# computational-cell-analytics/micro-sam

Hardware: AMD Instinct MI355X
Metric: 1024^2 tiles/s embed+AMG (vit_b bf16) (higher is better)
Workload: dtype bf16 image encoder (patch embedding + neck, 1.2 % of its flops, on hi+lo operand pairs of that type), fp16 mask decoder (16-bit MFMA operands, fp32 accumulation); 1 GPU; configs[1]: vit_b, 1024x1024 uint8 synthetic tiles, batched embedding precompute + AutomaticMaskGenerator (32x32 grid, multimask, default thresholds); encoder_batch=16, distinct_tiles_per_gpu=256, weights=seeded synthetic checkpoint (synthetic.py variant 'cells'), decode_lanes=3

## Files before the change

### include/msam_hip.h

```cpp
#ifndef MSAM_HIP_H
#define MSAM_HIP_H

#include <stdint.h>

#ifdef __cplusplus
extern "C" {
#endif

#define MSAM_MAX_BLOCKS 32
#define MSAM_F32 1
#define MSAM_BF16 2
#define MSAM_FP8 3
#define MSAM_F16 4
#define MSAM_U8 5
#define MSAM_U16 6
#define MSAM_ACT_NONE 0
#define MSAM_ACT_GELU 1
#define MSAM_ACT_RELU 2
#define MSAM_ACT_SIGMOID 3

const char* msam_last_error(void);
int msam_abi_version(void);


// ... 20 lines not shown
    const float* row_scale; const float* col_scale;
    int32_t split_k;
    const float* ln_add; void* ln_out_a; void* ln_out_b;
} msam_gemm_t;
int msam_gemm_bf16(const msam_gemm_t* p, void* stream);
#define MSAM_GEMM_GROUP_MAX 5
int msam_gemm_group_bf16(const msam_gemm_t* items, int32_t n, void* stream);

typedef struct {
    const void* A; const void* W; int32_t M, N, K;
    const float* bias;
    const float* table; int32_t table_rows, table_cols; int64_t table_ld;
    const void* resid; int32_t resid_rows; int64_t ldr;
    int32_t ln_mode; const float* ln_w; const float* ln_b; float ln_eps;
    void* out; int64_t ldc;
    int32_t kv_split; void* k_out; void* vT_out; int32_t tokens;
    int32_t head_major;
} msam_wsgemm_t;
int msam_wsgemm_bf16(const msam_wsgemm_t* p, void* stream);

typedef struct {
    const void* xin; const void* q_shared;
    const void* wq; const float* bq; const float* peq;
    const void* wo; const float* bo; const float* ln_w; const float* ln_b; float ln_eps;
    const void* ktok; const void* vtok; int32_t Nt;
    void* out; int32_t rows;
} msam_image_layer_t;
int msam_decoder_image_layer(const msam_image_layer_t* p, void* stream);

int64_t msam_t2i_fold_workspace_bytes(int32_t P);
int msam_t2i_fold_attention(const void* keys, int32_t kv_shared, const void* qtok, int32_t P, int32_t Nt, const void* wk,
                            const void* tabk, const void* wv, const float* bv, void* out, void* workspace,
                            int64_t workspace_bytes, void* stream);

int64_t msam_i2t_fold_workspace_bytes(int32_t P);
int msam_i2t_fold_layer(const void* xin, int32_t x_shared, const void* ktok, const void* vtok, int32_t P, int32_t Nt,
                        const void* wq, const void* tabq, const void* wo, const float* bo, const float* ln_w,
                        const float* ln_b, float ln_eps, void* out, void* workspace, int64_t workspace_bytes, void* stream);

int64_t msam_chain_tables_bytes(void);
int msam_chain_prepare_tables(const void* src, const void* q0, const void* tabk, const void* tabq1, void* tables, void* stream);
int64_t msam_i2t_fold_operand_bytes(int32_t P);
int msam_i2t_fold_operands(const void* ktok, const void* vtok, int32_t P, int32_t Nt, const void* wq, const void* wo,
                           const float* bo, int32_t with_kfold, void* operands, void* stream);
int64_t msam_i2t0_t2i_workspace_bytes(int32_t P);
int msam_i2t0_t2i_fused(const void* tables, const void* operands0, const float* ln0_w, const float* ln0_b, float ln_eps,
                        const void* qtok, int32_t P, int32_t Nt, const void* wk, const void* wv, const float* bv, void* out,
                        void* workspace, int64_t workspace_bytes, void* stream);
int64_t msam_chain_tables2_bytes(void);
int msam_chain_prepare_tables2(const void* src, const void* wv, const float* bv, const void* wk, const float* ln0_w,
                               const float* ln0_b, const void* wo0, const float* bo0, void* tables2, void* stream);
int64_t msam_chain_const2_bytes(void);
int msam_chain_prepare_const2(const void* wv, const float* bv, const void* wk, const float* ln0_w, const float* ln0_b,
                              const void* wo0, const float* bo0, void* const2, void* stream);
int msam_chain_prepare_tables2_c(const void* src, const void* const2, void* tables2, void* stream);
int64_t msam_t2i_fold_values_bytes(int32_t P);
int msam_t2i_fold_values(const void* vtok0, int32_t P, int32_t Nt, const void* tables2, void* mf, void* stream);
int msam_i2t_fold_operands_values(const void* ktok, const void* vtok, int32_t P, int32_t Nt, const void* wq, const void* wo,
                                  const float* bo, int32_t with_kfold, const void* tables2, void* operands, void* mf, void* stream);
int64_t msam_i2t0_t2i_v2_workspace_bytes(int32_t P);
int msam_i2t0_t2i_fused_v2(const void* tables, const void* tables2, const void* operands0, const void* mf, const float* ln0_w,
                           float ln_eps, const void* qtok, int32_t P, int32_t Nt, const void* wk, void* out, void* workspace,
                           int64_t workspace_bytes, void* stream);
int msam_i2t01_fused(const void* tables, const void* operands0, const float* ln0_w, const float* ln0_b, const void* operands1,
                     const float* ln1_w, const float* ln1_b, float ln_eps, int32_t P, int32_t Nt, void* out, void* stream);
int64_t msam_chain_handover_bytes(int32_t P);
int msam_i2t0_t2i_fused_v2_handover(const void* tables, const void* tables2, const void* operands0, const void* mf, const float* ln0_w,
                                    float ln_eps, const void* qtok, int32_t P, int32_t Nt, const void* wk, void* out, void* workspace,
                                    int64_t workspace_bytes, void* handover, void* stream);
int msam_i2t01_fused_handover(const void* tables, const void* operands0, const float* ln0_w, const float* ln0_b, const void* operands1,
                              const float* ln1_w, const float* ln1_b, float ln_eps, int32_t P, int32_t Nt, const void* handover,
                              void* out, void* stream);

int msam_upscale_fused(const void* keys, int32_t P, const void* w1, const float* b1, const float* ln_w, const float* ln_b,
                       float ln_eps, const void* w2, const float* b2, const float* hyper, int32_t hyper_ld, int32_t mask0,
                       int32_t nmask, float* low_res, void* stream);
int msam_upscale_fused_layout(const void* keys, int32_t keys_blocked, int32_t P, const void* w1, const float* b1,
                              const float* ln_w, const float* ln_b, float ln_eps, const void* w2, const float* b2,
                              const float* hyper, int32_t hyper_ld, int32_t mask0, int32_t nmask, float* low_res, void* stream);
int msam_upscale_fused_out(const void* keys, int32_t keys_blocked, int32_t P, const void* w1, const float* b1,
                           const float* ln_w, const float* ln_b, float ln_eps, const void* w2, const float* b2,
                           const float* hyper, int32_t hyper_ld, int32_t mask0, int32_t nmask, void* low_res,
                           int32_t low_res_dtype, void* stream);

int msam_upscale_set_prio(int32_t prio);
int msam_fold_attn_set_dma(int32_t on);
int msam_tune_set(const char* key, int32_t value);
int msam_debug_i2t_timing(int32_t enable, uint64_t* host_out);
int msam_gemm256_set_staging(int staging);
int msam_gemm_set_trace(void* device_words);
int msam_profile_enable(int on);
int msam_profile_collect(int32_t* launches, double* total_ms, double* total_flops);
#define MSAM_PROFILE_FAMILIES 8
int msam_profile_collect_family(int32_t* launches, double* ms, double* flops, double* bytes);

int msam_to_image(const void* in, int32_t in_dtype, int32_t H, int32_t W, int32_t C, uint8_t* out, void* workspace, void* stream);

int msam_mask_nms(const uint32_t* bits, const int32_t* order, const float* boxes, const int32_t* area, int32_t K, int32_t H,
                  int32_t W, float thresh, int32_t intersection_over_min, uint64_t* mask_scratch, int32_t* keep_flags,
                  void* stream);

int64_t msam_amg_generate_workspace_bytes(int32_t N, int32_t H, int32_t W);
int msam_amg_generate_labels(const float* iou, const float* stability, const int32_t* boxes, const int32_t* area,
                             const uint32_t* bits, int32_t N, int32_t H, int32_t W, const int32_t* crop_box,
                             float pred_iou_thresh, float stability_score_thresh, float box_nms_thresh,
                             int32_t min_object_size, int32_t with_background, int32_t* labels, int32_t* flag,
                             void* workspace, int64_t workspace_bytes, void* stream);

int64_t msam_labels_from_masks_workspace_bytes(int32_t H, int32_t W);
int msam_labels_from_masks(const uint32_t* bits, const int32_t* order, int32_t K, const int32_t* k_dev, int32_t H, int32_t W,
                           int32_t min_object_size, int32_t with_background, int32_t* labels, int32_t* flag,
                           void* workspace, int64_t workspace_bytes, void* stream);

int msam_layernorm_backward(const float* x, const float* weight, const float* dy, float eps, int64_t rows, int32_t dim,
                            float* dx, float* dweight, float* dbias, void* stream);
int msam_attention_forward(const float* q, const float* k, const float* v, int32_t BH, int32_t Nq, int32_t Nk, int32_t D,
                           float scale, float* out, float* lse, void* stream);
int msam_attention_backward(const float* q, const float* k, const float* v, const float* out, const float* dout,
                            const float* lse, int32_t BH, int32_t Nq, int32_t Nk, int32_t D, float scale, float* dq, float* dk,
                            float* dv, float* delta, void* stream);

int msam_relpos_attention_forward(const float* q, const float* k, const float* v, const float* bias_h, const float* bias_w,
                                  int32_t BH, int32_t Gh, int32_t Gw, int32_t D, float scale, float* out, float* lse,
                                  void* stream);
int msam_relpos_attention_backward(const float* q, const float* k, const float* v, const float* bias_h, const float* bias_w,
                                   const float* out, const float* dout, const float* lse, int32_t BH, int32_t Gh, int32_t Gw,
                                   int32_t D, float scale, float* dq, float* dk, float* dv, float* dbias_h, float* dbias_w,
                                   float* delta, void* stream);

int msam_cast_transpose(const void* x, int32_t x_dtype, int64_t M, int32_t K, int64_t ldx, void* out16, void* outT, float* colsum,
                        void* stream);

int msam_layernorm(const float* x, const float* weight, const float* bias, float eps, int64_t rows, int32_t dim,
                   void* out, int32_t out_dtype, int32_t gelu, int32_t out_nchw_hw, void* stream);

int msam_layernorm_fp8(const float* x, const float* weight, const float* bias, float eps, int64_t rows, int32_t dim,
                       void* out_fp8, float* row_scale, void* stream);
int msam_quant_rows_fp8(const void* x_bf16, int64_t rows, int32_t dim, void* out_fp8, float* row_scale, void* stream);
int msam_patchify(const float* img, int32_t B, void* out_bf16, void* stream);
int msam_patchify16(const float* img, int32_t B, int32_t dtype16, void* out16, void* stream);
int msam_patchify_u8(const uint8_t* img, int32_t B, int32_t h, int32_t w, void* out_bf16, void* stream);
int msam_patchify_u8_16(const uint8_t* img, int32_t B, int32_t h, int32_t w, int32_t dtype16, void* out16, void* stream);
int msam_im2col3x3(const void* x_bf16, int32_t B, int32_t C, void* out_bf16, void* stream);
int msam_cast_f32_to_bf16(const float* x, void* out_bf16, int64_t n, void* stream);
int msam_cast_f32_to_16(const float* x, int32_t dtype16, void* out16, int64_t n, void* stream);
int msam_resample_u8(const uint8_t* in, int32_t B, int32_t H, int32_t W, int32_t C, int32_t axis, int32_t n_out,
                     const int32_t* bounds, const int32_t* coefs, int32_t ksize, uint8_t* out, void* stream);
int msam_patchify_split16(const float* img, int32_t B, int32_t dtype16, void* out16, void* stream);
int msam_patchify_u8_split16(const uint8_t* img, int32_t B, int32_t h, int32_t w, int32_t dtype16, void* out16, void* stream);
int msam_im2col3x3_split16(const float* x_f32, int32_t B, int32_t C, int32_t dtype16, void* out16, void* stream);
int msam_cast_f32_split16(const float* x, int32_t dtype16, void* out16, int64_t rows, int32_t dim, void* stream);

int msam_window_attention(const void* q, const void* k, const void* v, const void* rel_h, const void* rel_w,
                          const float* qkv_bias, int32_t B, int32_t heads, int32_t head_dim, float scale, void* out,
                          void* stream);
int msam_window_attention16(const void* q, const void* k, const void* v, const void* rel_h, const void* rel_w,
                            const float* qkv_bias, int32_t B, int32_t heads, int32_t head_dim, float scale, int32_t dtype16,
                            void* out, void* stream);
int msam_global_attention(const void* q, const void* k, const void* v, const void* rel_h, const void* rel_w,
                          int32_t B, int32_t heads, int32_t head_dim, float scale, void* out, void* stream);
int msam_global_attention16(const void* q, const void* k, const void* v, const void* rel_h, const void* rel_w, int32_t B,
                            int32_t heads, int32_t head_dim, float scale, int32_t dtype16, void* out, void* stream);

typedef struct {
    int32_t embed_dim, depth, heads;
    int32_t is_global[MSAM_MAX_BLOCKS];
    const void* patch_w; const float* patch_b;
    const float* pos_embed;
    const float* ln1_w[MSAM_MAX_BLOCKS]; const float* ln1_b[MSAM_MAX_BLOCKS];
    const void* qkv_w[MSAM_MAX_BLOCKS]; const float* qkv_b[MSAM_MAX_BLOCKS];
    const void* rel_h[MSAM_MAX_BLOCKS]; const void* rel_w[MSAM_MAX_BLOCKS];
    const void* proj_w[MSAM_MAX_BLOCKS]; const float* proj_b[MSAM_MAX_BLOCKS];
    const float* ln2_w[MSAM_MAX_BLOCKS]; const float* ln2_b[MSAM_MAX_BLOCKS];
    const void* lin1_w[MSAM_MAX_BLOCKS]; const float* lin1_b[MSAM_MAX_BLOCKS];
    const void* lin2_w[MSAM_MAX_BLOCKS]; const float* lin2_b[MSAM_MAX_BLOCKS];
    const void* neck0_w;
    const float* neck1_w; const float* neck1_b;
    const void* neck2_w;
    const float* neck3_w; const float* neck3_b;
    int32_t use_glds;
    int32_t head_dim_stored;
    int32_t fp8;
    const void* qkv_w8[MSAM_MAX_BLOCKS]; const float* qkv_cs[MSAM_MAX_BLOCKS];
    const void* proj_w8[MSAM_MAX_BLOCKS]; const float* proj_cs[MSAM_MAX_BLOCKS];
    const void* lin1_w8[MSAM_MAX_BLOCKS]; const float* lin1_cs[MSAM_MAX_BLOCKS];
    const void* lin2_w8[MSAM_MAX_BLOCKS]; const float* lin2_cs[MSAM_MAX_BLOCKS];
    int32_t dtype16;
    int32_t split_io;
    const void* adapter_wd[MSAM_MAX_BLOCKS]; const float* adapter_bd[MSAM_MAX_BLOCKS];
    const void* adapter_wu[MSAM_MAX_BLOCKS]; const float* adapter_bu[MSAM_MAX_BLOCKS];
    const float* adapter_alpha[MSAM_MAX_BLOCKS];
    int32_t adapter_dim;
} msam_encoder_t;

int64_t msam_encoder_workspace_bytes(const msam_encoder_t* enc, int32_t B);
int msam_encoder_forward(const msam_encoder_t* enc, const float* img_f32, const uint8_t* img_u8, int32_t h, int32_t w,
                         int32_t B, float* out, void* workspace, int64_t workspace_bytes,
                         float* tap, int32_t tap_block, void* stream);

int msam_adapter_bf16(const void* y16, int64_t ldy, const void* wd16, const float* bd, const void* wu16, const float* bu,
                      const float* alpha, float* x, int64_t ldx, int32_t R, int32_t D, int32_t P, int32_t dtype16, void* stream);

typedef struct {
    const void* q_w; const float* q_b; const void* k_w; const float* k_b;
    const void* v_w; const float* v_b; const void* o_w; const float* o_b;
} msam_attn_w_t;
typedef struct {
    msam_attn_w_t self_attn, t2i, i2t;
    const float *n1_w, *n1_b, *n2_w, *n2_b, *n3_w, *n3_b, *n4_w, *n4_b;
    const void* mlp1_w; const float* mlp1_b; const void* mlp2_w; const float* mlp2_b;
    const void* mlp1_ws; const void* mlp2_ws;
} msam_twoway_layer_t;
typedef struct {
    const float* pe_gauss;
    const float* point_embed;
    const float* not_a_point;
    const float* no_mask;
    const float* out_tokens;
    msam_twoway_layer_t layer[2];
    msam_attn_w_t final_attn; const float *nf_w, *nf_b;
    const void* up1_w; const float* up1_b;
    const float* up_ln_w; const float* up_ln_b;
    const void* up2_w; const float* up2_b;
    const void* hyp_w[4][3]; const float* hyp_b[4][3];
    const void* iou_w[3]; const float* iou_b[3];
    int32_t use_glds;
    int32_t low_res_dtype;
    int32_t up1_centred;
} msam_decoder_t;

int msam_decoder_dtype(void);
int64_t msam_decoder_const_bytes(void);
int msam_decoder_prepare_const(const msam_decoder_t* dec, void* consts, void* stream);
int64_t msam_decoder_image_bytes(void);
int msam_decoder_prepare_image(const msam_decoder_t* dec, const void* consts, const float* embedding ,
                               void* image_state, void* workspace, int64_t workspace_bytes, void* stream);
int64_t msam_decoder_workspace_bytes(int32_t P);
int msam_decoder_forward(const msam_decoder_t* dec, const void* consts, const void* image_state,
                         const float* points, const int32_t* labels, int32_t Np, const float* boxes, int32_t P,
                         int32_t multimask, float* low_res, float* iou,
                         void* workspace, int64_t workspace_bytes, void* stream);

typedef struct {
    const float *c1_w, *c1_b, *ln1_w, *ln1_b, *c2_w, *c2_b, *ln2_w, *ln2_b, *c3_w, *c3_b;
    int32_t exact_gelu;
} msam_mask_prompt_t;
int msam_decoder_forward_masks(const msam_decoder_t* dec, const msam_mask_prompt_t* mask_w, const void* consts,
                               const void* image_state, const float* points, const int32_t* labels, int32_t Np,
                               const float* boxes, const float* mask_input, int32_t P, int32_t multimask, float* low_res,
                               float* iou, void* workspace, int64_t workspace_bytes, void* stream);

int msam_prompt_encode(const msam_decoder_t* dec, const msam_mask_prompt_t* mask_w, const float* points,
                       const int32_t* labels, int32_t Np, const float* boxes, const float* mask_input, int32_t P,
                       float* sparse, float* dense, void* stream);
int msam_decoder_forward_embeddings(const msam_decoder_t* dec, const void* consts, const void* image_state,
                                    const float* sparse, int32_t Ns, const float* dense, const float* embedding,
                                    int32_t P, int32_t multimask, float* low_res, float* iou, void* workspace,
                                    int64_t workspace_bytes, void* stream);

int msam_postprocess_masks(const float* low_res, int32_t N, int32_t in_h, int32_t in_w, int32_t out_h, int32_t out_w,
                           float thr, float off, int32_t* counts, int32_t* boxes, uint32_t* bits, float* logits,
                           void* stream);
int msam_postprocess_masks16(const void* low_res, int32_t low_res_dtype, int32_t N, int32_t in_h, int32_t in_w, int32_t out_h,
                             int32_t out_w, float thr, float off, int32_t* counts, int32_t* boxes, uint32_t* bits, float* logits,
                             void* stream);
int msam_uncrop_bits(const uint32_t* bits_crop, int32_t N, int32_t crop_h, int32_t crop_w, int32_t x0, int32_t y0,
                     int32_t out_h, int32_t out_w, uint32_t* bits_out, void* stream);

int msam_rle_run_counts(const uint32_t* bits, int32_t N, int32_t out_h, int32_t out_w, int32_t* n_runs, void* stream);
int msam_rle_encode(const uint32_t* bits, int32_t N, int32_t out_h, int32_t out_w, const int64_t* offsets,
                    int32_t* counts_out, void* stream);

int msam_box_nms(const float* boxes_sorted, int32_t K, float iou_threshold, uint64_t* mask_scratch, int32_t* keep_flags,
                 void* stream);

int msam_box_nms_valid(const float* boxes_sorted, const int32_t* valid_sorted, int32_t K, float iou_threshold,
                       uint64_t* mask_scratch, int32_t* keep_flags, void* stream);

int msam_paint_label_image(const uint32_t* bits, const int32_t* order, int32_t K, int32_t H, int32_t W, int32_t* label,
                           void* stream);
int msam_paint_label_image_dev(const uint32_t* bits, const int32_t* order, const int32_t* k_dev, int32_t H, int32_t W,
                               int32_t* label, void* stream);
int msam_label_components(const int32_t* seg, int32_t H, int32_t W, int32_t* roots, int32_t* changed_flag,
                          int32_t max_iters, int32_t* iters_done, void* stream);

int msam_component_sizes(const int32_t* roots, int32_t n, int32_t* sizes, int32_t* bg_count, void* stream);
int msam_label_components_async(const int32_t* seg, int32_t H, int32_t W, int32_t* roots, int32_t* changed_flag,
                                int32_t passes, void* stream);

#define MSAM_MATCH_MAX_THRESHOLDS 16
#define MSAM_MATCH_MAX_BATCH 65535
#define MSAM_MATCH_HEADER 4
#define MSAM_MATCH_ITEM 20
#define MSAM_MATCH_EDGE 6
int64_t msam_label_matching_workspace_bytes(int32_t B, int32_t capacity);
int msam_label_matching(const int32_t* pred, const int32_t* gt, int32_t B, int32_t G, int32_t H, int32_t W,
                        const double* thresholds, int32_t T, void* workspace, int64_t workspace_bytes, int32_t capacity,
                        int32_t* result, int32_t max_edges, void* stream);

int msam_slice_overlaps(const int32_t* labels, int32_t Z, int32_t H, int32_t W, uint64_t* table_keys, int32_t* table_counts,
                        int32_t capacity, int32_t* edges, int32_t max_edges, int32_t* n_edges, void* stream);

int msam_host_seeded_watershed(const float* image, const int32_t* markers, const uint8_t* mask, int32_t H, int32_t W, int32_t* out);

typedef struct {
    const float* A; int64_t lda;
    const float* A2; int64_t lda2; int64_t a2_rows;
    const float* W; int64_t ldw;
    int64_t M; int32_t N, K;
    const float* bias; int32_t act;
    const float* res; int64_t ldr; int64_t res_rows;
    float* out; int64_t ldc;
    const float* col_scale; const float* col_shift;
    int32_t conv_h, conv_w, conv_c;
    int32_t shuffle_h, shuffle_w, shuffle_c;
    int32_t a2_cols;
    int32_t split16;
    float a_scale, w_scale;
    const void* w_pairs;
} msam_sgemm_t;
int msam_strict_gemm(const msam_sgemm_t* p, void* stream);
int msam_strict_layernorm(const float* x, const float* weight, const float* bias, float eps, int64_t rows, int32_t dim, float* out,
                          int32_t gelu, int32_t out_nchw_hw, void* stream);
int msam_strict_relpos_attention(const float* qkv, const float* qkv_bias, const float* rel_h, const float* rel_w, int32_t B, int32_t heads,
                                 int32_t head_dim, int32_t grid, int32_t window, float scale, float* out, void* stream);
int msam_split16_relpos_attention(const float* qkv, const float* qkv_bias, const float* rel_h, const float* rel_w, int32_t B, int32_t heads,
                                  int32_t head_dim, int32_t grid, int32_t window, float scale, float* out, void* stream);
typedef struct msam_si2t {
    const float* keys; int64_t key_batch_stride;
    const float* pos;
    const float* wq; const float* bq;
    const float* tok_k; const float* tok_v; int64_t ld_tok, tok_batch_stride;
    const float* wo; const float* bo;
    const float* ln_weight; const float* ln_bias; float ln_eps; float denom;
    float* out;
    int32_t B, Tk;
    int32_t split16;
    float wq_scale, wo_scale;
    const void* wq_pairs; const void* wo_pairs;
} msam_si2t_t;
int msam_strict_i2t_block(const msam_si2t_t* p, void* stream);
int msam_strict_attention(const float* q, int64_t ldq, int64_t q_batch_stride, const float* k, int64_t ldk, int64_t k_batch_stride,
                          const float* v, int64_t ldv, int64_t v_batch_stride, int32_t B, int32_t H, int32_t Nq, int32_t Nk, int32_t D,
                          float denom, float* out, int64_t ldo, int64_t out_batch_stride, void* stream);
int msam_strict_patchify(const float* img, const uint8_t* img_u8, int32_t B, int32_t h, int32_t w, float* out, void* stream);
int msam_strict_im2col3x3(const float* x, int32_t B, int32_t C, float* out, void* stream);
int msam_strict_source(const float* embedding, const float* dense, int64_t dense_stride, int32_t P, float* src, void* stream);
int msam_strict_hyper_masks(const float* up, const float* hyper, int32_t hyper_ld, int32_t mask0, int32_t nmask, int64_t P, float* low_res,
// ... 107 lines not shown
```

### micro_sam_amd/_lib.py

```python
from __future__ import annotations

import ctypes as C
import os
from typing import Optional

import torch

from . import build as _build

MSAM_MAX_BLOCKS = 32
F32, BF16, FP8, F16, U8, U16 = 1, 2, 3, 4, 5, 6
ACT_NONE, ACT_GELU, ACT_RELU, ACT_SIGMOID = 0, 1, 2, 3

_vp, _i32, _i64, _f32 = C.c_void_p, C.c_int32, C.c_int64, C.c_float
PROFILE_FAMILIES = 8


class GemmParams(C.Structure):
    _fields_ = [
        ("A", _vp), ("lda", _i64), ("W", _vp), ("ldw", _i64), ("M", _i32), ("N", _i32), ("K", _i32),
        ("bias", _vp), ("table", _vp), ("table_rows", _i32), ("table_cols", _i32), ("table_ld", _i64),
        ("resid", _vp), ("resid_dtype", _i32), ("resid_rows", _i32), ("ldr", _i64), ("act", _i32),
        ("out", _vp), ("out_dtype", _i32), ("ldc", _i64), ("out_mode", _i32),
        ("q", _vp), ("k", _vp), ("v", _vp), ("heads", _i32), ("head_dim", _i32), ("tokens", _i32),
        ("use_glds", _i32), ("ln_mode", _i32), ("ln_w", _vp), ("ln_b", _vp), ("ln_eps", _f32),
        ("a_dtype", _i32), ("row_scale", _vp), ("col_scale", _vp), ("split_k", _i32),
        ("ln_add", _vp), ("ln_out_a", _vp), ("ln_out_b", _vp),
    ]


class WsGemmParams(C.Structure):
    _fields_ = [
        ("A", _vp), ("W", _vp), ("M", _i32), ("N", _i32), ("K", _i32), ("bias", _vp),
        ("table", _vp), ("table_rows", _i32), ("table_cols", _i32), ("table_ld", _i64),
        ("resid", _vp), ("resid_rows", _i32), ("ldr", _i64),
        ("ln_mode", _i32), ("ln_w", _vp), ("ln_b", _vp), ("ln_eps", _f32),
        ("out", _vp), ("ldc", _i64), ("kv_split", _i32), ("k_out", _vp), ("vT_out", _vp), ("tokens", _i32),
        ("head_major", _i32),
    ]


class ImageLayerParams(C.Structure):
    _fields_ = [
        ("xin", _vp), ("q_shared", _vp), ("wq", _vp), ("bq", _vp), ("peq", _vp),
        ("wo", _vp), ("bo", _vp), ("ln_w", _vp), ("ln_b", _vp), ("ln_eps", _f32),
        ("ktok", _vp), ("vtok", _vp), ("Nt", _i32), ("out", _vp), ("rows", _i32),
    ]


_blk = _vp * MSAM_MAX_BLOCKS


class EncoderParams(C.Structure):
    _fields_ = [
        ("embed_dim", _i32), ("depth", _i32), ("heads", _i32), ("is_global", _i32 * MSAM_MAX_BLOCKS),
        ("patch_w", _vp), ("patch_b", _vp), ("pos_embed", _vp),
        ("ln1_w", _blk), ("ln1_b", _blk), ("qkv_w", _blk), ("qkv_b", _blk), ("rel_h", _blk), ("rel_w", _blk),
        ("proj_w", _blk), ("proj_b", _blk), ("ln2_w", _blk), ("ln2_b", _blk),
        ("lin1_w", _blk), ("lin1_b", _blk), ("lin2_w", _blk), ("lin2_b", _blk),
        ("neck0_w", _vp), ("neck1_w", _vp), ("neck1_b", _vp), ("neck2_w", _vp), ("neck3_w", _vp), ("neck3_b", _vp),
        ("use_glds", _i32), ("head_dim_stored", _i32), ("fp8", _i32),
        ("qkv_w8", _blk), ("qkv_cs", _blk), ("proj_w8", _blk), ("proj_cs", _blk),
        ("lin1_w8", _blk), ("lin1_cs", _blk), ("lin2_w8", _blk), ("lin2_cs", _blk),
        ("dtype16", _i32), ("split_io", _i32),
        ("adapter_wd", _blk), ("adapter_bd", _blk), ("adapter_wu", _blk), ("adapter_bu", _blk), ("adapter_alpha", _blk),
        ("adapter_dim", _i32),
    ]


class AttnW(C.Structure):
    _fields_ = [("q_w", _vp), ("q_b", _vp), ("k_w", _vp), ("k_b", _vp), ("v_w", _vp), ("v_b", _vp),
                ("o_w", _vp), ("o_b", _vp)]


class TwoWayLayer(C.Structure):
    _fields_ = [("self_attn", AttnW), ("t2i", AttnW), ("i2t", AttnW),
                ("n1_w", _vp), ("n1_b", _vp), ("n2_w", _vp), ("n2_b", _vp), ("n3_w", _vp), ("n3_b", _vp),
                ("n4_w", _vp), ("n4_b", _vp),
                ("mlp1_w", _vp), ("mlp1_b", _vp), ("mlp2_w", _vp), ("mlp2_b", _vp), ("mlp1_ws", _vp), ("mlp2_ws", _vp)]


class DecoderParams(C.Structure):
    _fields_ = [
        ("pe_gauss", _vp), ("point_embed", _vp), ("not_a_point", _vp), ("no_mask", _vp), ("out_tokens", _vp),
        ("layer", TwoWayLayer * 2), ("final_attn", AttnW), ("nf_w", _vp), ("nf_b", _vp),
        ("up1_w", _vp), ("up1_b", _vp), ("up_ln_w", _vp), ("up_ln_b", _vp), ("up2_w", _vp), ("up2_b", _vp),
        ("hyp_w", (_vp * 3) * 4), ("hyp_b", (_vp * 3) * 4), ("iou_w", _vp * 3), ("iou_b", _vp * 3),
        ("use_glds", _i32), ("low_res_dtype", _i32), ("up1_centred", _i32),
    ]


class SGemmParams(C.Structure):
    _fields_ = [("A", _vp), ("lda", _i64), ("A2", _vp), ("lda2", _i64), ("a2_rows", _i64), ("W", _vp), ("ldw", _i64),
                ("M", _i64), ("N", _i32), ("K", _i32), ("bias", _vp), ("act", _i32), ("res", _vp), ("ldr", _i64), ("res_rows", _i64),
                ("out", _vp), ("ldc", _i64), ("col_scale", _vp), ("col_shift", _vp), ("conv_h", _i32), ("conv_w", _i32), ("conv_c", _i32),
                ("shuffle_h", _i32), ("shuffle_w", _i32), ("shuffle_c", _i32), ("a2_cols", _i32), ("split16", _i32), ("a_scale", _f32), ("w_scale", _f32), ("w_pairs", _vp)]


class SI2TParams(C.Structure):
    _fields_ = [("keys", _vp), ("key_batch_stride", _i64), ("pos", _vp), ("wq", _vp), ("bq", _vp), ("tok_k", _vp), ("tok_v", _vp),
                ("ld_tok", _i64), ("tok_batch_stride", _i64), ("wo", _vp), ("bo", _vp), ("ln_weight", _vp), ("ln_bias", _vp),
                ("ln_eps", _f32), ("denom", _f32), ("out", _vp), ("B", _i32), ("Tk", _i32), ("split16", _i32), ("wq_scale", _f32), ("wo_scale", _f32), ("wq_pairs", _vp), ("wo_pairs", _vp)]


class ST2IParams(C.Structure):
    _fields_ = [("keys", _vp), ("key_batch_stride", _i64), ("pos", _vp), ("q", _vp), ("ldq", _i64), ("wk", _vp), ("wv", _vp), ("bv", _vp),
                ("denom", _f32), ("out", _vp), ("ldo", _i64), ("B", _i32), ("Tk", _i32), ("workspace", _vp), ("workspace_bytes", _i64)]


class SUp2Params(C.Structure):
    _fields_ = [("u1", _vp), ("ln_weight", _vp), ("ln_bias", _vp), ("ln_eps", _f32), ("w2", _vp), ("b2", _vp), ("w_scale", _f32),
                ("hyper", _vp), ("hyper_ld", _i32), ("mask0", _i32), ("nmask", _i32), ("low_res", _vp), ("P", _i64)]


class MaskPromptParams(C.Structure):
    _fields_ = [(n, _vp) for n in ("c1_w", "c1_b", "ln1_w", "ln1_b", "c2_w", "c2_b", "ln2_w", "ln2_b", "c3_w", "c3_b")] + [("exact_gelu", _i32)]


_PROTOS = {
    "msam_last_error": (C.c_char_p, []),
    "msam_abi_version": (_i32, []),
    "msam_gemm_bf16": (_i32, [C.POINTER(GemmParams), _vp]),
    "msam_wsgemm_bf16": (_i32, [C.POINTER(WsGemmParams), _vp]),
    "msam_decoder_image_layer": (_i32, [C.POINTER(ImageLayerParams), _vp]),
    "msam_t2i_fold_workspace_bytes": (_i64, [_i32]),
    "msam_t2i_fold_attention": (_i32, [_vp, _i32, _vp, _i32, _i32, _vp, _vp, _vp, _vp, _vp, _vp, _i64, _vp]),
    "msam_upscale_fused": (_i32, [_vp, _i32, _vp, _vp, _vp, _vp, _f32, _vp, _vp, _vp, _i32, _i32, _i32, _vp, _vp]),
    "msam_uncrop_bits": (_i32, [_vp, _i32, _i32, _i32, _i32, _i32, _i32, _i32, _vp, _vp]),
    "msam_decoder_forward_masks": (_i32, [C.POINTER(DecoderParams), C.POINTER(MaskPromptParams), _vp, _vp, _vp, _vp, _i32, _vp, _vp,
                                          _i32, _i32, _vp, _vp, _vp, _i64, _vp]),
    "msam_i2t_fold_workspace_bytes": (_i64, [_i32]),
    "msam_i2t_fold_layer": (_i32, [_vp, _i32, _vp, _vp, _i32, _i32, _vp, _vp, _vp, _vp, _vp, _vp, _f32, _vp, _vp, _i64, _vp]),
    "msam_profile_enable": (_i32, [_i32]),
    "msam_profile_collect": (_i32, [C.POINTER(_i32), C.POINTER(C.c_double), C.POINTER(C.c_double)]),
    "msam_profile_collect_family": (_i32, [_i32 * PROFILE_FAMILIES, C.c_double * PROFILE_FAMILIES, C.c_double * PROFILE_FAMILIES,
                                          C.c_double * PROFILE_FAMILIES]),
    "msam_layernorm": (_i32, [_vp, _vp, _vp, _f32, _i64, _i32, _vp, _i32, _i32, _i32, _vp]),
    "msam_layernorm_backward": (_i32, [_vp, _vp, _vp, _f32, _i64, _i32, _vp, _vp, _vp, _vp]),
    "msam_attention_forward": (_i32, [_vp, _vp, _vp, _i32, _i32, _i32, _i32, _f32, _vp, _vp, _vp]),
    "msam_attention_backward": (_i32, [_vp, _vp, _vp, _vp, _vp, _vp, _i32, _i32, _i32, _i32, _f32, _vp, _vp, _vp, _vp, _vp]),
    "msam_relpos_attention_forward": (_i32, [_vp, _vp, _vp, _vp, _vp, _i32, _i32, _i32, _i32, _f32, _vp, _vp, _vp]),
    "msam_relpos_attention_backward": (_i32, [_vp, _vp, _vp, _vp, _vp, _vp, _vp, _vp, _i32, _i32, _i32, _i32, _f32, _vp, _vp, _vp,
                                              _vp, _vp, _vp, _vp]),
    "msam_amg_generate_workspace_bytes": (_i64, [_i32, _i32, _i32]),
    "msam_amg_generate_labels": (_i32, [_vp, _vp, _vp, _vp, _vp, _i32, _i32, _i32, C.POINTER(_i32), _f32, _f32, _f32, _i32, _i32,
                                        _vp, _vp, _vp, _i64, _vp]),
    "msam_to_image": (_i32, [_vp, _i32, _i32, _i32, _i32, _vp, _vp, _vp]),
    "msam_patchify": (_i32, [_vp, _i32, _vp, _vp]),
    "msam_patchify_u8": (_i32, [_vp, _i32, _i32, _i32, _vp, _vp]),
    "msam_im2col3x3": (_i32, [_vp, _i32, _i32, _vp, _vp]),
    "msam_cast_f32_to_bf16": (_i32, [_vp, _vp, _i64, _vp]),
    "msam_cast_transpose": (_i32, [_vp, _i32, _i64, _i32, _i64, _vp, _vp, _vp, _vp]),
    "msam_gemm256_set_staging": (_i32, [_i32]),
    "msam_gemm_set_trace": (_i32, [_vp]),
    "msam_gemm_group_bf16": (_i32, [_vp, _i32, _vp]),
    "msam_fold_attn_set_dma": (_i32, [_i32]),
    "msam_tune_set": (_i32, [C.c_char_p, _i32]),
    "msam_i2t_fold_operand_bytes": (_i64, [_i32]),
    "msam_i2t_fold_operands": (_i32, [_vp, _vp, _i32, _i32, _vp, _vp, _vp, _i32, _vp, _vp]),
    "msam_i2t0_t2i_workspace_bytes": (_i64, [_i32]),
    "msam_i2t0_t2i_fused": (_i32, [_vp, _vp, _vp, _vp, _f32, _vp, _i32, _i32, _vp, _vp, _vp, _vp, _vp, _i64, _vp]),
    "msam_i2t01_fused": (_i32, [_vp, _vp, _vp, _vp, _vp, _vp, _vp, _f32, _i32, _i32, _vp, _vp]),
    "msam_chain_tables2_bytes": (_i64, []),
    "msam_chain_prepare_tables2": (_i32, [_vp, _vp, _vp, _vp, _vp, _vp, _vp, _vp, _vp, _vp]),
    "msam_chain_const2_bytes": (_i64, []),
    "msam_chain_prepare_const2": (_i32, [_vp, _vp, _vp, _vp, _vp, _vp, _vp, _vp, _vp]),
    "msam_chain_prepare_tables2_c": (_i32, [_vp, _vp, _vp, _vp]),
    "msam_t2i_fold_values_bytes": (_i64, [_i32]),
    "msam_t2i_fold_values": (_i32, [_vp, _i32, _i32, _vp, _vp, _vp]),
    "msam_i2t_fold_operands_values": (_i32, [_vp, _vp, _i32, _i32, _vp, _vp, _vp, _i32, _vp, _vp, _vp, _vp]),
    "msam_i2t0_t2i_v2_workspace_bytes": (_i64, [_i32]),
    "msam_i2t0_t2i_fused_v2": (_i32, [_vp, _vp, _vp, _vp, _vp, _f32, _vp, _i32, _i32, _vp, _vp, _vp, _i64, _vp]),
    "msam_chain_handover_bytes": (_i64, [_i32]),
    "msam_i2t0_t2i_fused_v2_handover": (_i32, [_vp, _vp, _vp, _vp, _vp, _f32, _vp, _i32, _i32, _vp, _vp, _vp, _i64, _vp, _vp]),
    "msam_i2t01_fused_handover": (_i32, [_vp, _vp, _vp, _vp, _vp, _vp, _vp, _f32, _i32, _i32, _vp, _vp, _vp]),
    "msam_chain_tables_bytes": (_i64, []),
    "msam_chain_prepare_tables": (_i32, [_vp, _vp, _vp, _vp, _vp, _vp]),
    "msam_upscale_fused_layout": (_i32, [_vp, _i32, _i32, _vp, _vp, _vp, _vp, _f32, _vp, _vp, _vp, _i32, _i32, _i32, _vp, _vp]),
    "msam_upscale_fused_out": (_i32, [_vp, _i32, _i32, _vp, _vp, _vp, _vp, _f32, _vp, _vp, _vp, _i32, _i32, _i32, _vp, _i32, _vp]),
    "msam_upscale_set_prio": (_i32, [_i32]),
    "msam_layernorm_fp8": (_i32, [_vp, _vp, _vp, _f32, _i64, _i32, _vp, _vp, _vp]),
    "msam_quant_rows_fp8": (_i32, [_vp, _i64, _i32, _vp, _vp, _vp]),
    "msam_debug_i2t_timing": (_i32, [_i32, _vp]),
    "msam_window_attention": (_i32, [_vp, _vp, _vp, _vp, _vp, _vp, _i32, _i32, _i32, C.c_float, _vp, _vp]),
    "msam_global_attention": (_i32, [_vp, _vp, _vp, _vp, _vp, _i32, _i32, _i32, C.c_float, _vp, _vp]),
    "msam_window_attention16": (_i32, [_vp, _vp, _vp, _vp, _vp, _vp, _i32, _i32, _i32, C.c_float, _i32, _vp, _vp]),
    "msam_global_attention16": (_i32, [_vp, _vp, _vp, _vp, _vp, _i32, _i32, _i32, C.c_float, _i32, _vp, _vp]),
    "msam_patchify16": (_i32, [_vp, _i32, _i32, _vp, _vp]),
    "msam_patchify_u8_16": (_i32, [_vp, _i32, _i32, _i32, _i32, _vp, _vp]),
    "msam_cast_f32_to_16": (_i32, [_vp, _i32, _vp, _i64, _vp]),
    "msam_resample_u8": (_i32, [_vp, _i32, _i32, _i32, _i32, _i32, _i32, _vp, _vp, _i32, _vp, _vp]),
    "msam_patchify_split16": (_i32, [_vp, _i32, _i32, _vp, _vp]),
    "msam_patchify_u8_split16": (_i32, [_vp, _i32, _i32, _i32, _i32, _vp, _vp]),
    "msam_im2col3x3_split16": (_i32, [_vp, _i32, _i32, _i32, _vp, _vp]),
    "msam_cast_f32_split16": (_i32, [_vp, _i32, _vp, _i64, _i32, _vp]),
    "msam_encoder_workspace_bytes": (_i64, [C.POINTER(EncoderParams), _i32]),
    "msam_encoder_forward": (_i32, [C.POINTER(EncoderParams), _vp, _vp, _i32, _i32, _i32, _vp, _vp, _i64, _vp, _i32, _vp]),
    "msam_decoder_dtype": (_i32, []),
    "msam_decoder_const_bytes": (_i64, []),
    "msam_decoder_prepare_const": (_i32, [C.POINTER(DecoderParams), _vp, _vp]),
    "msam_decoder_image_bytes": (_i64, []),
    "msam_decoder_prepare_image": (_i32, [C.POINTER(DecoderParams), _vp, _vp, _vp, _vp, _i64, _vp]),
    "msam_decoder_workspace_bytes": (_i64, [_i32]),
    "msam_prompt_encode": (_i32, [C.POINTER(DecoderParams), C.POINTER(MaskPromptParams), _vp, _vp, _i32, _vp, _vp, _i32, _vp, _vp, _vp]),
    "msam_decoder_forward_embeddings": (_i32, [C.POINTER(DecoderParams), _vp, _vp, _vp, _i32, _vp, _vp, _i32, _i32, _vp, _vp, _vp,
                                               _i64, _vp]),
    "msam_decoder_forward": (_i32, [C.POINTER(DecoderParams), _vp, _vp, _vp, _vp, _i32, _vp, _i32, _i32, _vp, _vp, _vp,
                                    _i64, _vp]),
    "msam_postprocess_masks": (_i32, [_vp, _i32, _i32, _i32, _i32, _i32, _f32, _f32, _vp, _vp, _vp, _vp, _vp]),
    "msam_postprocess_masks16": (_i32, [_vp, _i32, _i32, _i32, _i32, _i32, _i32, _f32, _f32, _vp, _vp, _vp, _vp, _vp]),
    "msam_rle_run_counts": (_i32, [_vp, _i32, _i32, _i32, _vp, _vp]),
    "msam_rle_encode": (_i32, [_vp, _i32, _i32, _i32, _vp, _vp, _vp]),
    "msam_mask_nms": (_i32, [_vp, _vp, _vp, _vp, _i32, _i32, _i32, _f32, _i32, _vp, _vp, _vp]),
    "msam_box_nms": (_i32, [_vp, _i32, _f32, _vp, _vp, _vp]),
    "msam_box_nms_valid": (_i32, [_vp, _vp, _i32, _f32, _vp, _vp, _vp]),
    "msam_paint_label_image_dev": (_i32, [_vp, _vp, _vp, _i32, _i32, _vp, _vp]),
    "msam_label_components_async": (_i32, [_vp, _i32, _i32, _vp, _vp, _i32, _vp]),
    "msam_component_sizes": (_i32, [_vp, _i32, _vp, _vp, _vp]),
    "msam_labels_from_masks_workspace_bytes": (_i64, [_i32, _i32]),
    "msam_labels_from_masks": (_i32, [_vp, _vp, _i32, _vp, _i32, _i32, _i32, _i32, _vp, _vp, _vp, _i64, _vp]),
    "msam_host_seeded_watershed": (_i32, [_vp, _vp, _vp, _i32, _i32, _vp]),
    "msam_slice_overlaps": (_i32, [_vp, _i32, _i32, _i32, _vp, _vp, _i32, _vp, _i32, _vp, _vp]),
    "msam_paint_label_image": (_i32, [_vp, _vp, _i32, _i32, _i32, _vp, _vp]),
    "msam_label_components": (_i32, [_vp, _i32, _i32, _vp, _vp, _i32, C.POINTER(_i32), _vp]),
    "msam_strict_gemm": (_i32, [C.POINTER(SGemmParams), _vp]),
    "msam_strict_i2t_block": (_i32, [C.POINTER(SI2TParams), _vp]),
    "msam_strict_layernorm": (_i32, [_vp, _vp, _vp, _f32, _i64, _i32, _vp, _i32, _i32, _vp]),
    "msam_strict_relpos_attention": (_i32, [_vp, _vp, _vp, _vp, _i32, _i32, _i32, _i32, _i32, _f32, _vp, _vp]),
    "msam_split16_relpos_attention": (_i32, [_vp, _vp, _vp, _vp, _i32, _i32, _i32, _i32, _i32, _f32, _vp, _vp]),
    "msam_strict_attention": (_i32, [_vp, _i64, _i64, _vp, _i64, _i64, _vp, _i64, _i64, _i32, _i32, _i32, _i32, _i32, _f32, _vp, _i64,
                                     _i64, _vp]),
    "msam_strict_patchify": (_i32, [_vp, _vp, _i32, _i32, _i32, _vp, _vp]),
    "msam_strict_im2col3x3": (_i32, [_vp, _i32, _i32, _vp, _vp]),
    "msam_strict_source": (_i32, [_vp, _vp, _i64, _i32, _vp, _vp]),
    "msam_strict_hyper_masks": (_i32, [_vp, _vp, _i32, _i32, _i32, _i64, _vp, _vp]),
    "msam_strict_upscale2": (_i32, [C.POINTER(SUp2Params), _vp]),
    "msam_split16_t2i_attention": (_i32, [C.POINTER(ST2IParams), _vp]),
    "msam_split16_prepare_pairs": (_i32, [_vp, _i64, _i32, _f32, _i32, _vp, _vp]),
    "msam_split16_i2t_block": (_i32, [C.POINTER(SI2TParams), _vp, _i64, _vp]),
    "msam_strict_instance_norm": (_i32, [_vp, _i64, _i32, _i64, _i32, _f32, _vp, _vp, _i64, _vp]),
    "msam_strict_resize_bilinear": (_i32, [_vp, _i32, _i32, _i32, _i32, _i32, _i64, _i32, _i32, _i32, _f32, _f32, _i32, _vp, _vp]),
    "msam_objfeat_gather": (_i32, [_vp, _vp, _i32, _i32, _vp, _vp, _i32, _vp, _vp, _vp]),
    "msam_objfeat_accumulate": (_i32, [_vp, _vp, _i32, _vp, _vp, _vp, _vp, _vp, _vp, _vp, _i32, _i32, _i32, _vp, _vp]),
    "msam_objfeat_finish": (_i32, [_vp, _vp, _vp, _i32, _vp, _vp, _i32, _vp, _vp]),
    "msam_objfeat_project": (_i32, [_vp, _i64, _vp, _i32, _vp, _vp]),
    "msam_label_matching_workspace_bytes": (_i64, [_i32, _i32]),
    "msam_label_matching": (_i32, [_vp, _vp, _i32, _i32, _i32, _i32, C.POINTER(C.c_double), _i32, _vp, _i64, _i32, _vp, _i32, _vp]),
    "msam_edt_squared_workspace_bytes": (_i64, [_i32, _i32]),
    "msam_edt_squared": (_i32, [_vp, _i32, _i32, _i32, _vp, _vp, _i64, _vp]),
    "msam_label_props_workspace_bytes": (_i64, [_i32, _i32, _i32]),
    "msam_label_props": (_i32, [_vp, _i32, _i32, _vp, _i32, _vp, _vp, _vp, _vp, _vp, _i64, _vp]),
    "msam_distance_targets_workspace_bytes": (_i64, [_i32, _i32, _i32]),
    "msam_distance_targets": (_i32, [_vp, _i32, _i32, _i32, _i32, _f32, _vp, _vp, _vp, _vp, _vp, _i64, _vp]),
    "msam_mask_pack": (_i32, [_vp, _i32, _i32, _i32, _vp, _vp]),
    "msam_mask_iou_counts": (_i32, [_vp, _vp, _i32, _i32, _i32, C.c_double, _vp, _vp, _vp]),
    "msam_mask_box_prompts": (_i32, [_vp, _i32, _i32, _i32, C.c_double, _i32, _i32, _vp, _vp, _vp]),
    "msam_mask_logits": (_i32, [_vp, _i32, _i32, _i32, _vp, _vp]),
    "msam_paint_max": (_i32, [_vp, _vp, _vp, _i32, _i32, _i32, _vp, _vp]),
    "msam_pca_moments_workspace_bytes": (_i64, [_i32, _i32, _i32]),
    "msam_pca_moments": (_i32, [_vp, _i32, _i32, _i32, _vp, _vp, _vp, _i64, _vp]),
    "msam_pca_project": (_i32, [_vp, _vp, _vp, _i32, _i32, _i32, _i32, _vp, _vp, _vp]),
    "msam_pca_to_rgb": (_i32, [_vp, _vp, _i32, _i32, _vp, _vp]),
    "msam_semantic_loss_workspace_bytes": (_i64, [_i32, _i32, _i32]),
    "msam_semantic_loss_forward": (_i32, [_vp, _vp, _i32, _i32, _i32, _f32, _f32, _i32, C.c_double, _vp, _i64, _vp, _vp, _vp]),
    "msam_semantic_loss_backward": (_i32, [_vp, _vp, _i32, _i32, _i32, _f32, _f32, _i32, C.c_double, _vp, _vp, _vp, _vp]),
    "msam_depth_conv3_bf16": (_i32, [_vp, _i64, _vp, _vp, _vp, _i64, _i32, _i32, _i32, _i32, _i32, _vp]),
    "msam_conv3d_k3_bf16": (_i32, [_vp, _i64, _vp, _vp, _vp, _i64, _i32, _i32, _i32, _i32, _i32, _i32, _vp]),
    "msam_conv3d_k3_wgrad_workspace_bytes": (_i64, [_i32, _i32, _i32, _i32, _i32, _i32]),
    "msam_conv3d_k3_wgrad_bf16": (_i32, [_vp, _i64, _vp, _i64, _vp, _vp, _i64, _i32, _i32, _i32, _i32, _i32, _i32, _vp]),
    "msam_instance_norm_workspace_bytes": (_i64, [_i32, _i64, _i32]),
    "msam_instance_norm_stats": (_i32, [_vp, _i64, _i32, _i64, _i32, _vp, _vp, _i64, _vp]),
    "msam_instance_norm_apply": (_i32, [_vp, _i64, _vp, _vp, _i64, _vp, _i32, _i64, _i32, _f32, _f32, _i32, _vp, _i64, _vp, _i64, _vp]),
    "msam_instance_norm_backward": (_i32, [_vp, _i64, _vp, _i64, _vp, _vp, _i64, _vp, _i32, _i64, _i32, _f32, _f32, _i32, _vp, _i64, _vp, _i64,
                                           _vp, _vp, _i64, _vp]),
    "msam_column_sums_f32": (_i32, [_vp, _i64, _i64, _i32, _vp, _vp, _i64, _vp]),
    "msam_adapter_bf16": (_i32, [_vp, _i64, _vp, _vp, _vp, _vp, _vp, _vp, _i64, _i32, _i32, _i32, _i32, _vp]),
}
OPTIONAL = set()

_lib: Optional[C.CDLL] = None


def lib_path() -> str:
    return _build.variant_path(os.environ.get("MSAM_LIB_VARIANT", ""))


def load() -> C.CDLL:
    global _lib
    if _lib is not None:
        return _lib
    path = lib_path()
    if not os.path.exists(path):
        raise RuntimeError(
            f"micro_sam_amd: {path} is missing. Build it with `python -m micro_sam_amd.build` "
            "(hipcc --offload-arch=gfx950). There is no CPU / PyTorch fallback."
        )
    lib = C.CDLL(path)
    for name, (res, args) in _PROTOS.items():
        if not hasattr(lib, name):
            if name in OPTIONAL:
                continue
            raise RuntimeError(f"micro_sam_amd: {path} does not export {name}")
        fn = getattr(lib, name)
        fn.restype, fn.argtypes = res, args
    _lib = lib
    for item in filter(None, os.environ.get("MSAM_TUNE", "").split(",")):
        key, _, val = item.partition("=")
        if lib.msam_tune_set(key.strip().encode(), int(val)) != 0:
            raise RuntimeError(f"micro_sam_amd: MSAM_TUNE: unknown knob {key!r}")
    return lib


def decoder_dtype() -> torch.dtype:
    return torch.float16 if load().msam_decoder_dtype() == F16 else torch.bfloat16


def exported_symbols():
    return [n for n in _PROTOS if n not in OPTIONAL]


def check(status: int, what: str = "") -> None:
    if status == 0:
        return
    msg = load().msam_last_error().decode("utf-8", "replace")
    if status == 1:
        raise ValueError(f"{what}: {msg}")
    raise RuntimeError(f"{what}: {msg}")


def require_gpu(device=None) -> torch.device:
    if not torch.cuda.is_available():
        raise RuntimeError("micro_sam_amd needs an AMD GPU (gfx950); torch.cuda.is_available() is False. "
                           "There is no CPU fallback.")
    return torch.device("cuda", torch.cuda.current_device()) if device is None else torch.device(device)


def stream_ptr() -> int:
    return torch.cuda.current_stream().cuda_stream


def ptr(t: Optional[torch.Tensor]) -> Optional[int]:
    if t is None:
        return None
    assert t.is_cuda, "device tensor expected"
    return t.data_ptr()
```

### micro_sam_amd/csrc/decfold.hip

```cpp
#include "common.h"
#include "../../include/msam_hip.h"
#include <string>

void msam_set_error(const char* msg);
int msam_check_launch(const char* what);
void msam_profile_mark2(void* stream, int begin, double flops, double bytes, int family);

namespace {

constexpr int T = 4096, C = 256, CI = 128, TK = 32, NTHR = 256;
constexpr int SUBT = 1024 + 32;
constexpr int KEYS_BYTES = 16 * SUBT, TAB_BYTES = TK * CI * 2, BUF_BYTES = KEYS_BYTES + TAB_BYTES;
constexpr float NEG_BIG = -1.0e30f;
#ifndef FOLD_ATTN_DMA_DEFAULT
#define FOLD_ATTN_DMA_DEFAULT 0
#endif

typedef short s16x4_t __attribute__((ext_vector_type(4)));

MSAM_DEVINL uint2 lds_tr16(const unsigned char* p) {
    s16x4_t v = __builtin_amdgcn_ds_read_tr16_b64_v4i16((s16x4_t __attribute__((address_space(3)))*)p);
    return __builtin_bit_cast(uint2, v);
}

// ... 596 lines not shown
    if (g_fold_attn_dma && !a.blocked) {
        const int grid3 = a.nitems < 3 * cus ? a.nitems : 3 * cus;
        hipLaunchKernelGGL(fold_attn_kernel<true>, dim3(grid3), dim3(NTHR), 0, s, a);
    } else {
        hipLaunchKernelGGL(fold_attn_kernel<false>, dim3(grid), dim3(NTHR), 0, s, a);
    }
    msam_profile_mark2(stream, 0, flops, bytes, 3);
    if (int e = msam_check_launch("fold_attn")) return e;
    if (KS == 1) return 0;
    hipLaunchKernelGGL(fold_finish_kernel, dim3(P * 8), dim3(128), 0, s, opart, stats, KS, Nt, (const u16*)wv, bv, (u16*)out);
    return msam_check_launch("fold_finish");
}

int64_t msam_i2t_tok_workspace_bytes(int32_t P);
int msam_i2t_tok_layer(const void* xin, int32_t x_shared, const void* ktok, const void* vtok, int32_t P, int32_t Nt,
                       const void* wq, const void* tabq, const void* wo, const float* bo, const float* ln_w,
                       const float* ln_b, float ln_eps, void* out, void* workspace, int KS, void* stream);
extern int g_tune_i2t_variant;

extern "C" int64_t msam_i2t_fold_workspace_bytes(int32_t P) {
    const int64_t a = (int64_t)P * 64 * C * 2 * 2, b = msam_i2t_tok_workspace_bytes(P);
    return a > b ? a : b;
}

extern "C" int msam_i2t_fold_layer(const void* xin, int32_t x_shared, const void* ktok, const void* vtok, int32_t P,
                                   int32_t Nt, const void* wq, const void* tabq, const void* wo, const float* bo,
                                   const float* ln_w, const float* ln_b, float ln_eps, void* out, void* workspace,
                                   int64_t workspace_bytes, void* stream) {
    if (!xin || !ktok || !vtok || !wq || !tabq || !wo || !bo || !ln_w || !ln_b || !out || !workspace || P <= 0) {
        msam_set_error("msam_i2t_fold_layer: null argument");
        return 1;
    }
    if (Nt < 1 || Nt > 8) { msam_set_error("msam_i2t_fold_layer: 1 <= Nt <= 8 tokens per prompt"); return 1; }
    if (workspace_bytes < msam_i2t_fold_workspace_bytes(P)) { msam_set_error("msam_i2t_fold_layer: workspace too small"); return 1; }
    if (g_tune_i2t_variant == 1)
        return msam_i2t_tok_layer(xin, x_shared, ktok, vtok, P, Nt, wq, tabq, wo, bo, ln_w, ln_b, ln_eps, out, workspace,
                                  key_splits(P), stream);
    hipStream_t s = (hipStream_t)stream;
    u16* kfold = (u16*)workspace;
    u16* vfoldT = kfold + (long)P * 64 * C;
    hipLaunchKernelGGL(fold_q_kernel, dim3(P * 8), dim3(256), 0, s, (const u16*)ktok, (const u16*)wq, Nt, kfold);
    if (int e = msam_check_launch("fold_k")) return e;
    hipLaunchKernelGGL(fold_v_kernel, dim3(P), dim3(256), 0, s, (const u16*)vtok, (const u16*)wo, Nt, vfoldT);
    if (int e = msam_check_launch("fold_v")) return e;
    I2tArgs a{};
    a.xin = (const u16*)xin; a.x_shared = x_shared; a.kfold = kfold; a.vfoldT = vfoldT; a.ktok = (const u16*)ktok; a.Nt = Nt;
    a.tabq = (const u16*)tabq; a.bo = bo; a.ln_w = ln_w; a.ln_b = ln_b; a.eps = ln_eps;
    a.KS = key_splits(P); a.nitems = P * a.KS; a.out = (u16*)out;
    int dev = 0, cus = 256;
    (void)hipGetDevice(&dev);
    (void)hipDeviceGetAttribute(&cus, hipDeviceAttributeMultiprocessorCount, dev);
    const int grid = a.nitems < 2 * cus ? a.nitems : 2 * cus;
    const double flops = (double)P * T * (2.0 * 64 * C * 2 + 2.0 * 64 * 32);
    const double bytes = (double)(x_shared ? 1 : P) * T * C * 2 + (double)P * T * C * 2;
    msam_profile_mark2(stream, 1, flops, bytes, 2);
    if (g_i2t_timing) hipLaunchKernelGGL(fold_i2t_kernel<true>, dim3(grid), dim3(NTHR), 0, s, a);
    else hipLaunchKernelGGL(fold_i2t_kernel<false>, dim3(grid), dim3(NTHR), 0, s, a);
    msam_profile_mark2(stream, 0, flops, bytes, 2);
    return msam_check_launch("fold_i2t");
}

extern "C" int msam_debug_i2t_timing(int32_t enable, uint64_t* host_out) {
    g_i2t_timing = enable;
    if (host_out) {
        if (hipDeviceSynchronize() != hipSuccess ||
            hipMemcpyFromSymbol(host_out, HIP_SYMBOL(g_i2t_stamps), sizeof(unsigned long long) * 64 * 12) != hipSuccess) {
            msam_set_error("msam_debug_i2t_timing: copy failed");
            return 2;
        }
    }
    return 0;
}

extern "C" int msam_fold_attn_set_dma(int32_t on) { g_fold_attn_dma = on; return 0; }

extern int g_tune_i2t_wg_per_cu, g_tune_chain_variant, g_tune_chain_tmask, g_tune_up_gelu16, g_tune_up_ln_two_pass, g_tune_up_centred;
void msam_gemm_set_dbg(int v);
void msam_gemm_set_gw(int delay, int cls);
void msam_gemm_set_g3(int delay);
void msam_gemm_set_g3_epi(int v);
extern int g_tune_tok_fuse;
extern int g_tune_chain_handover, g_tune_chain_handover_ring;
extern int g_tune_mlp_split_fused;
extern int g_tune_sgemm_bufs, g_tune_srel_mfma, g_tune_sgemm_small_below, g_tune_si2t_dbg, g_tune_si2t_late_us, g_tune_sattn_allh;
int g_tune_dec_chain = 1, g_tune_dec_chain_min_p = 128;
extern "C" int msam_tune_set(const char* key, int32_t value) {
    const std::string k = key ? key : "";
    if (k == "i2t_variant") g_tune_i2t_variant = value;
    else if (k == "i2t_wg_per_cu") g_tune_i2t_wg_per_cu = value;
    else if (k == "dec_chain") g_tune_dec_chain = value;
    else if (k == "chain_variant") g_tune_chain_variant = value;
    else if (k == "chain_tmask") g_tune_chain_tmask = value;
    else if (k == "chain_handover") g_tune_chain_handover = value;
    else if (k == "chain_handover_ring") g_tune_chain_handover_ring = value;
    else if (k == "up_gelu16") g_tune_up_gelu16 = value;
    else if (k == "up_ln_two_pass") g_tune_up_ln_two_pass = value;
    else if (k == "up_centred") g_tune_up_centred = value;
    else if (k == "gemm_dbg") msam_gemm_set_dbg(value);
    else if (k == "gw_delay") msam_gemm_set_gw(value, -1);
    else if (k == "gw_class") msam_gemm_set_gw(-2, value);
    else if (k == "g3_delay") msam_gemm_set_g3(value);
    else if (k == "g3_epi") msam_gemm_set_g3_epi(value);
    else if (k == "tok_fuse") g_tune_tok_fuse = value;
    else if (k == "mlp_split_fused") g_tune_mlp_split_fused = value;
    else if (k == "dec_chain_min_p") g_tune_dec_chain_min_p = value;
    else if (k == "sgemm_bufs") g_tune_sgemm_bufs = value;
    else if (k == "srel_mfma") g_tune_srel_mfma = value;
    else if (k == "sattn_allh") g_tune_sattn_allh = value;
    else if (k == "sgemm_small_below") g_tune_sgemm_small_below = value;
    else if (k == "si2t_dbg") g_tune_si2t_dbg = value;
    else if (k == "si2t_late_us") g_tune_si2t_late_us = value;
    else { msam_set_error("msam_tune_set: unknown key"); return 1; }
    return 0;
}
```

### micro_sam_amd/csrc/decoder.hip

```cpp
#include <stdlib.h>
#include "common.h"
#include "../../include/msam_hip.h"

void msam_set_error(const char* msg);
int msam_check_launch(const char* what);

namespace {

constexpr int T = 4096;
constexpr int C = 256;
constexpr int CI = 128;
constexpr float NEG_BIG = -1.0e30f;
constexpr float TWO_PI = 6.283185307179586f;


MSAM_DEVINL void pe_encode(const float* __restrict__ G, float cx, float cy, int j, float& s, float& c) {
    const float x = 2.f * cx - 1.f, y = 2.f * cy - 1.f;
    const float v = TWO_PI * (x * G[j] + y * G[128 + j]);
    s = sinf(v); c = cosf(v);
}

__global__ __launch_bounds__(256) void dense_pe_kernel(const float* __restrict__ G, float* __restrict__ pos_f32,
                                                       u16* __restrict__ pos_bf16) {
    const int idx = blockIdx.x * 256 + threadIdx.x;
// ... 800 lines not shown
                CHECK(msam_cast_f32_split16(h32, MSAM_D16, h3, M, 2048, cx.s));
            }
            mlp_h = h3; mlp2_w = L.mlp2_ws; mlp2_k = 3 * 2048;
        } else {
        CHECK(gemm(cx, w.a, C, L.mlp1_w, M, 2048, C, L.mlp1_b, w.mlp_h, MSAM_D16, 2048, MSAM_ACT_RELU));
        }
        if (fuse_tok) {
            CHECK(gemm_ln_tok(cx, mlp_h, mlp2_k, mlp2_w, M, mlp2_k, L.mlp2_b, w.queries, L.n3_w, L.n3_b, w.queries, w.qpe, w.a, w.b));
        } else {
        CHECK(gemm(cx, mlp_h, mlp2_k, mlp2_w, M, C, mlp2_k, L.mlp2_b, w.tmp, MSAM_F32, C, 0, w.queries, MSAM_F32, C));
        LN(w.tmp, L.n3_w, L.n3_b, M, w.queries, MSAM_F32);
        ADD_CAST2(w.queries, w.qpe, w.a, w.b);
        }
        {
            const msam_gemm_t kv[2] = {mk_gemm(w.a, C, L.i2t.k_w, M, CI, C, L.i2t.k_b, w.ks, MSAM_D16, CI),
                                       mk_gemm(w.b, C, L.i2t.v_w, M, CI, C, L.i2t.v_b, w.vs, MSAM_D16, CI)};
            CHECK(msam_gemm_group_bf16(kv, 2, cx.s));
        }
        if (chain) {
            if (li == 0 && chain2)
                CHECK(msam_i2t_fold_operands_values(w.ks, w.vs, P, Nt, L.i2t.q_w, L.i2t.o_w, L.i2t.o_b, 0, tables2, oper0, mfrag, cx.s));
            else
                CHECK(msam_i2t_fold_operands(w.ks, w.vs, P, Nt, L.i2t.q_w, L.i2t.o_w, L.i2t.o_b, li, li == 0 ? oper0 : oper1, cx.s));
            if (li == 1) {
                const msam_twoway_layer_t& L0 = dec->layer[0];
                if (handover)
                    CHECK(msam_i2t01_fused_handover(tables, oper0, L0.n4_w, L0.n4_b, oper1, L.n4_w, L.n4_b, 1e-5f, P, Nt, w.hand, w.keys, cx.s));
                else
                    CHECK(msam_i2t01_fused(tables, oper0, L0.n4_w, L0.n4_b, oper1, L.n4_w, L.n4_b, 1e-5f, P, Nt, w.keys, cx.s));
            }
        } else if (Nt <= 8) {
            const bool shared = li == 0 && !own_src;
            CHECK(msam_i2t_fold_layer(shared ? (const void*)im.src_bf16 : (const void*)w.keys, shared, w.ks, w.vs, P, Nt,
                                      L.i2t.q_w, c.tab_q[li], L.i2t.o_w, L.i2t.o_b, L.n4_w, L.n4_b, 1e-5f, w.keys, w.qimg,
                                      (int64_t)((char*)w.up1 - (char*)w.qimg), cx.s));
        } else {
            msam_image_layer_t g{};
            g.wo = L.i2t.o_w; g.bo = L.i2t.o_b; g.ln_w = L.n4_w; g.ln_b = L.n4_b; g.ln_eps = 1e-5f;
            g.ktok = w.ks; g.vtok = w.vs; g.Nt = Nt; g.out = w.keys; g.rows = (int)R;
            if (li == 0 && !own_src) { g.xin = im.src_bf16; g.q_shared = im.q0; }
            else { g.xin = w.keys; g.wq = L.i2t.q_w; g.bq = L.i2t.q_b; g.peq = c.pe_q[li]; }
            CHECK(msam_decoder_image_layer(&g, cx.s));
        }
    }
    if (dbg) return 0;
    if (!fuse_tok) ADD_CAST(w.queries, w.qpe, w.a);
    CHECK(gemm(cx, w.a, C, dec->final_attn.q_w, M, CI, C, dec->final_attn.q_b, w.qs, MSAM_D16, CI));
    CHECK(t2i_stream(cx, w, c, 2, dec->final_attn, P, Nt, chain));
    if (fuse_tok) {
        CHECK(gemm_ln_tok(cx, w.attn_tok, CI, dec->final_attn.o_w, M, CI, dec->final_attn.o_b, w.queries, dec->nf_w, dec->nf_b, w.queries,
                          nullptr, w.a, nullptr));
    } else {
    CHECK(gemm(cx, w.attn_tok, CI, dec->final_attn.o_w, M, C, CI, dec->final_attn.o_b, w.tmp, MSAM_F32, C, 0, w.queries,
               MSAM_F32, C));
    LN(w.tmp, dec->nf_w, dec->nf_b, M, w.queries, MSAM_F32);

    ADD_CAST(w.queries, nullptr, w.a);
    }
    {
        msam_gemm_t h[5];
        const long PC = (long)P * C;
        for (int i = 0; i < 5; ++i) {
            const void* wt = i == 0 ? dec->iou_w[0] : dec->hyp_w[i - 1][0];
            const float* bs = i == 0 ? dec->iou_b[0] : dec->hyp_b[i - 1][0];
            h[i] = mk_gemm(w.a + (long)i * C, (long)Nt * C, wt, P, C, C, bs, w.hh0 + i * PC, MSAM_D16, C, MSAM_ACT_RELU);
        }
        CHECK(msam_gemm_group_bf16(h, 5, cx.s));
        for (int i = 0; i < 5; ++i) {
            const void* wt = i == 0 ? dec->iou_w[1] : dec->hyp_w[i - 1][1];
            const float* bs = i == 0 ? dec->iou_b[1] : dec->hyp_b[i - 1][1];
            h[i] = mk_gemm(w.hh0 + i * PC, C, wt, P, C, C, bs, w.hh1 + i * PC, MSAM_D16, C, MSAM_ACT_RELU);
        }
        CHECK(msam_gemm_group_bf16(h, 5, cx.s));
        h[0] = mk_gemm(w.hh1, C, dec->iou_w[2], P, 128, C, dec->iou_b[2], w.iou_full, MSAM_F32, 128);
        for (int i = 1; i < 5; ++i)
            h[i] = mk_gemm(w.hh1 + i * PC, C, dec->hyp_w[i - 1][2], P, 128, C, dec->hyp_b[i - 1][2], w.hyper + (long)(i - 1) * 128,
                           MSAM_F32, 4 * 128);
        CHECK(msam_gemm_group_bf16(h, 5, cx.s));
    }
    const int mask0 = multimask ? 1 : 0, nmask = multimask ? 3 : 1;
    hipLaunchKernelGGL(gather_iou_kernel, dim3((P * nmask + 255) / 256), dim3(256), 0, cx.s, w.iou_full, P, mask0, nmask, iou);
    CHECK(msam_check_launch("gather_iou"));

    CHECK(msam_upscale_fused_out(w.keys, (chain ? 1 : 0) | (dec->up1_centred ? 2 : 0), P, dec->up1_w, dec->up1_b, dec->up_ln_w, dec->up_ln_b, 1e-6f, dec->up2_w,
                                 dec->up2_b, w.hyper, 128, mask0, nmask, low_res, dec->low_res_dtype == MSAM_F16 ? MSAM_F16 : MSAM_F32,
                                 cx.s));
#undef CHECK
#undef ADD_CAST
#undef ADD_CAST2
#undef LN
    return 0;
}
}
```

### micro_sam_amd/csrc/postprocess.hip

```cpp
#include "common.h"
#include "../../include/msam_hip.h"

void msam_set_error(const char* msg);
int msam_check_launch(const char* what);

namespace {

struct Axis { int i0, i1; float w0, w1; };
struct lowh_t { unsigned short bits; };
MSAM_DEVINL float lowf(float v) { return v; }
MSAM_DEVINL float lowf(lowh_t v) { return h2f(v.bits); }

MSAM_DEVINL Axis axis_weights(int dst, float scale, int in_size) {
    float src = __fsub_rn(__fmul_rn(scale, __fadd_rn((float)dst, 0.5f)), 0.5f);
    if (src < 0.f) src = 0.f;
    Axis a;
    a.i0 = (int)src;
    a.i1 = a.i0 + (a.i0 < in_size - 1 ? 1 : 0);
    a.w1 = __fsub_rn(src, (float)a.i0);
    a.w0 = __fsub_rn(1.0f, a.w1);
    return a;
}

MSAM_DEVINL float lerp_torch(float w0, float p0, float w1, float p1) { return __fmaf_rn(w0, p0, __fmul_rn(w1, p1)); }

template <typename TL>
MSAM_DEVINL float stage1(const TL* __restrict__ low, int Y, int X) {
    const Axis ay = axis_weights(Y, 0.25f, 256), ax = axis_weights(X, 0.25f, 256);
    const TL* r0 = low + ay.i0 * 256; const TL* r1 = low + ay.i1 * 256;
    const float t0 = lerp_torch(ax.w0, lowf(r0[ax.i0]), ax.w1, lowf(r0[ax.i1]));
    const float t1 = lerp_torch(ax.w0, lowf(r1[ax.i0]), ax.w1, lowf(r1[ax.i1]));
    return lerp_torch(ay.w0, t0, ay.w1, t1);
}

__global__ void init_stats_kernel(int* __restrict__ counts, int* __restrict__ boxes, int N) {
    const int n = blockIdx.x * 256 + threadIdx.x;
    if (n >= N) return;
    counts[n * 3] = 0; counts[n * 3 + 1] = 0; counts[n * 3 + 2] = 0;
    boxes[n * 4] = 0x7fffffff; boxes[n * 4 + 1] = 0x7fffffff; boxes[n * 4 + 2] = -1; boxes[n * 4 + 3] = -1;
}

__global__ void finalize_boxes_kernel(int* __restrict__ boxes, int N) {
    const int n = blockIdx.x * 256 + threadIdx.x;
    if (n >= N) return;
    if (boxes[n * 4 + 2] < boxes[n * 4] || boxes[n * 4 + 3] < boxes[n * 4 + 1]) {
        boxes[n * 4] = 0; boxes[n * 4 + 1] = 0; boxes[n * 4 + 2] = 0; boxes[n * 4 + 3] = 0;
    }
}

template <bool TWO_STAGE, bool LOGITS, typename TL>
__global__ __launch_bounds__(256) void postprocess_kernel(const TL* __restrict__ low_res, int in_h, int in_w, int out_h,
                                                          int out_w, float thr, float off, int* __restrict__ counts,
                                                          int* __restrict__ boxes, uint32_t* __restrict__ bits,
                                                          float* __restrict__ logits) {
    __shared__ int red[4][7];
    __shared__ float tile[2][10 * 66];
    const int x = blockIdx.x * 256 + threadIdx.x, n = blockIdx.y;
    const int wpc = (out_h + 31) >> 5;
    const TL* low = low_res + (long)n * 65536;
    const float hi_t = thr + off, lo_t = thr - off;
    int c_hi = 0, c_lo = 0, c_m = 0, ymin = 0x7fffffff, ymax = -1;
    bool any = false;
    if (!TWO_STAGE) {
        const int cbase = max((int)blockIdx.x * 64 - 1, 0);
        int sr[3], sc[3];
#pragma unroll
        for (int k = 0; k < 3; ++k) {
            const int idx = threadIdx.x + k * 256;
            sr[k] = idx / 66; sc[k] = min(cbase + idx % 66, 255);
        }
        float nx[3] = {0.f, 0.f, 0.f};
#define PP_LOAD(yw_)                                                                               \
        _Pragma("unroll") for (int k = 0; k < 3; ++k)                                              \
            if (threadIdx.x + k * 256 < 660) nx[k] = lowf(low[min(max((yw_) * 8 - 1 + sr[k], 0), 255) * 256 + sc[k]]);
#define PP_STORE(buf_)                                                                             \
        _Pragma("unroll") for (int k = 0; k < 3; ++k)                                              \
            if (threadIdx.x + k * 256 < 660) tile[buf_][threadIdx.x + k * 256] = nx[k];
        PP_LOAD(0);
        PP_STORE(0);
        __syncthreads();
        const Axis ax = axis_weights(min(x, out_w - 1), 0.25f, 256);
        const int l0 = ax.i0 - cbase, l1 = ax.i1 - cbase;
        const float W1[4] = {0.625f, 0.875f, 0.125f, 0.375f};
        for (int yw = 0; yw < wpc; ++yw) {
            if (yw + 1 < wpc) { PP_LOAD(yw + 1); }
            const float* tl = tile[yw & 1];
            if (x < out_w) {
                float t[10];
#pragma unroll
                for (int k = 0; k < 10; ++k) t[k] = lerp_torch(ax.w0, tl[k * 66 + l0], ax.w1, tl[k * 66 + l1]);
                const int nb = min(32, out_h - yw * 32);
                uint32_t wm = 0, wh = 0, wl = 0;
                uint32_t word;
                if (nb == 32) {
                    int s_hi = 0, s_lo = 0;
                    bool decided = false;
                    if (!LOGITS) {
                        const float tmin = fminf(fminf(fminf(t[0], t[1]), fminf(t[2], t[3])), fminf(fminf(t[4], t[5]), fminf(fminf(t[6], t[7]), fminf(t[8], t[9]))));
                        const float tmax = fmaxf(fmaxf(fmaxf(t[0], t[1]), fmaxf(t[2], t[3])), fmaxf(fmaxf(t[4], t[5]), fmaxf(fmaxf(t[6], t[7]), fmaxf(t[8], t[9]))));
                        const bool one = tmin > hi_t + 0.01f && tmax < 8192.f, zero = tmax < lo_t - 0.01f && tmin > -8192.f;
                        if (__ballot(!(one || zero)) == 0) {
                            decided = true;
                            word = one ? 0xffffffffu : 0u;
                            s_hi = s_lo = 32 * __popcll(__ballot(one));
                        }
                    }
                    if (!decided) {
#pragma unroll
                        for (int b = 0; b < 32; ++b) {
                            float w1 = W1[b & 3];
                            if (b < 2 && yw == 0) w1 = 0.0f;
                            const float v = lerp_torch(1.0f - w1, t[(b + 2) / 4], w1, t[(b + 2) / 4 + 1]);
                            if (LOGITS) logits[((long)n * out_h + yw * 32 + b) * out_w + x] = v;
                            wm = __builtin_amdgcn_alignbit(wm, __float_as_uint(__fsub_rn(thr, v)), 31);
                            s_hi += __popcll(__ballot(v > hi_t));
                            s_lo += __popcll(__ballot(v > lo_t));
                        }
                        word = __brev(wm);
                    }
                    if ((threadIdx.x & 63) == __ffsll((long long)__ballot(1)) - 1) { c_hi += s_hi; c_lo += s_lo; }
                } else {
#pragma unroll
                    for (int b = 0; b < 32; ++b) {
                        float w1 = W1[b & 3];
                        if (b < 2 && yw == 0) w1 = 0.0f;
                        const float v = lerp_torch(1.0f - w1, t[(b + 2) / 4], w1, t[(b + 2) / 4 + 1]);
                        if (LOGITS) { if (b < nb) logits[((long)n * out_h + yw * 32 + b) * out_w + x] = v; }
                        wm = __builtin_amdgcn_alignbit(wm, __float_as_uint(__fsub_rn(thr, v)), 31);
                        wh = __builtin_amdgcn_alignbit(wh, __float_as_uint(__fsub_rn(hi_t, v)), 31);
                        wl = __builtin_amdgcn_alignbit(wl, __float_as_uint(__fsub_rn(lo_t, v)), 31);
                    }
                    const uint32_t valid = (1u << nb) - 1u;
                    word = __brev(wm) & valid;
                    c_hi += __popc(__brev(wh) & valid); c_lo += __popc(__brev(wl) & valid);
                }
                if (word) {
                    c_m += __popc(word); any = true;
                    ymin = min(ymin, yw * 32 + __ffs(word) - 1); ymax = yw * 32 + 31 - __clz(word);
                }
                bits[((long)n * wpc + yw) * out_w + x] = word;
            }
            if (yw + 1 < wpc) { PP_STORE((yw + 1) & 1); }
            __syncthreads();
        }
#undef PP_LOAD
#undef PP_STORE
    } else {
        const bool live = x < out_w;
        const int x = min((int)(blockIdx.x * 256 + threadIdx.x), out_w - 1);
        const float sx = (float)in_w / (float)out_w, sy = (float)in_h / (float)out_h;
        const Axis ax2 = axis_weights(x, sx, in_w);
        const Axis axa = axis_weights(ax2.i0, 0.25f, 256), axb = axis_weights(ax2.i1, 0.25f, 256);
        int lr[2] = {-1, -1};
        float la[2] = {0.f, 0.f}, lb[2] = {0.f, 0.f};
        int lnext = 0;
        auto low_row = [&](int r, float& va, float& vb) {
            if (r == lr[0]) { va = la[0]; vb = lb[0]; return; }
            if (r == lr[1]) { va = la[1]; vb = lb[1]; return; }
            const TL* row = low + r * 256;
            va = lerp_torch(axa.w0, lowf(row[axa.i0]), axa.w1, lowf(row[axa.i1]));
            vb = lerp_torch(axb.w0, lowf(row[axb.i0]), axb.w1, lowf(row[axb.i1]));
            lr[lnext] = r; la[lnext] = va; lb[lnext] = vb; lnext ^= 1;
        };
        int ir[2] = {-1, -1};
        float ia[2] = {0.f, 0.f}, ib[2] = {0.f, 0.f};
        int inext = 0;
        auto inter_row = [&](int Y, float& va, float& vb) {
            if (Y == ir[0]) { va = ia[0]; vb = ib[0]; return; }
            if (Y == ir[1]) { va = ia[1]; vb = ib[1]; return; }
            const Axis ay = axis_weights(Y, 0.25f, 256);
            float a0, b0, a1, b1;
            low_row(ay.i0, a0, b0);
            low_row(ay.i1, a1, b1);
            va = lerp_torch(ay.w0, a0, ay.w1, a1);
            vb = lerp_torch(ay.w0, b0, ay.w1, b1);
            ir[inext] = Y; ia[inext] = va; ib[inext] = vb; inext ^= 1;
        };
        int gclo, gchi;
        {
            const int xf = min((int)blockIdx.x * 256, out_w - 1), xl = min((int)blockIdx.x * 256 + 255, out_w - 1);
            const Axis f2 = axis_weights(xf, sx, in_w), l2 = axis_weights(xl, sx, in_w);
            gclo = axis_weights(f2.i0, 0.25f, 256).i0; gchi = axis_weights(l2.i1, 0.25f, 256).i1;
        }
        for (int yw = 0; yw < wpc; ++yw) {
            uint32_t word = 0;
            if (!LOGITS) {
                const int y0 = yw * 32, nb = min(32, out_h - y0);
                const int Ylo = axis_weights(y0, sy, in_h).i0, Yhi = axis_weights(y0 + nb - 1, sy, in_h).i1;
                const int rlo = axis_weights(Ylo, 0.25f, 256).i0, rhi = axis_weights(Yhi, 0.25f, 256).i1;
                float* cm = &tile[yw & 1][0];
                if ((int)threadIdx.x <= gchi - gclo) {
                    const int c = gclo + threadIdx.x;
                    float a = 3.0e38f, b = -3.0e38f;
                    for (int r = rlo; r <= rhi; ++r) { const float v = lowf(low[r * 256 + c]); a = fminf(a, v); b = fmaxf(b, v); }
                    cm[threadIdx.x] = a; cm[256 + threadIdx.x] = b;
                }
                __syncthreads();
                const int clo = min(axa.i0, axb.i0), chi = max(axa.i1, axb.i1);
                float mn = 3.0e38f, mx = -3.0e38f;
                for (int c = clo; c <= chi; ++c) { mn = fminf(mn, cm[c - gclo]); mx = fmaxf(mx, cm[256 + c - gclo]); }
                const bool one = mn > hi_t + 0.01f && mx < 8192.f, zero = mx < lo_t - 0.01f && mn > -8192.f;
                if (__ballot(!(one || zero)) == 0) {
                    if (!live) continue;
                    if (one) {
                        word = nb == 32 ? 0xffffffffu : (1u << nb) - 1u;
                        c_hi += nb; c_lo += nb; c_m += nb; any = true;
                        ymin = min(ymin, y0); ymax = y0 + nb - 1;
                    }
                    bits[((long)n * wpc + yw) * out_w + x] = word;
                    continue;
                }
            }
            for (int b = 0; b < 32; ++b) {
                const int y = yw * 32 + b;
                if (y >= out_h) break;
                const Axis ay2 = axis_weights(y, sy, in_h);
                float p00, p01, p10, p11;
                inter_row(ay2.i0, p00, p01);
                inter_row(ay2.i1, p10, p11);
                const float t0 = lerp_torch(ax2.w0, p00, ax2.w1, p01);
                const float t1 = lerp_torch(ax2.w0, p10, ax2.w1, p11);
                const float v = lerp_torch(ay2.w0, t0, ay2.w1, t1);
                if (!live) continue;
                if (LOGITS) logits[((long)n * out_h + y) * out_w + x] = v;
                c_hi += v > hi_t; c_lo += v > lo_t;
                if (v > thr) { word |= 1u << b; ++c_m; any = true; ymin = min(ymin, y); ymax = y; }
            }
            if (live) bits[((long)n * wpc + yw) * out_w + x] = word;
        }
    }
    int xmin = any ? x : 0x7fffffff, xmax = any ? x : -1;
#pragma unroll
    for (int s = 1; s < 64; s <<= 1) {
        c_hi += __shfl_xor(c_hi, s); c_lo += __shfl_xor(c_lo, s); c_m += __shfl_xor(c_m, s);
        ymin = min(ymin, __shfl_xor(ymin, s)); ymax = max(ymax, __shfl_xor(ymax, s));
        xmin = min(xmin, __shfl_xor(xmin, s)); xmax = max(xmax, __shfl_xor(xmax, s));
    }
    const int wave = threadIdx.x >> 6;
    if ((threadIdx.x & 63) == 0) {
        red[wave][0] = c_hi; red[wave][1] = c_lo; red[wave][2] = c_m; red[wave][3] = xmin; red[wave][4] = ymin;
        red[wave][5] = xmax; red[wave][6] = ymax;
    }
    __syncthreads();
    if (threadIdx.x == 0) {
        int hi = 0, lo = 0, m = 0, x0 = 0x7fffffff, y0 = 0x7fffffff, x1 = -1, y1 = -1;
        for (int w = 0; w < 4; ++w) {
            hi += red[w][0]; lo += red[w][1]; m += red[w][2];
            x0 = min(x0, red[w][3]); y0 = min(y0, red[w][4]); x1 = max(x1, red[w][5]); y1 = max(y1, red[w][6]);
        }
        if (hi) atomicAdd(&counts[n * 3], hi);
        if (lo) atomicAdd(&counts[n * 3 + 1], lo);
        if (m) {
            atomicAdd(&counts[n * 3 + 2], m);
            atomicMin(&boxes[n * 4], x0); atomicMin(&boxes[n * 4 + 1], y0);
            atomicMax(&boxes[n * 4 + 2], x1); atomicMax(&boxes[n * 4 + 3], y1);
        }
    }
}


MSAM_DEVINL uint32_t col_prev_bit(const uint32_t* __restrict__ bm, int wpc, int out_w, int out_h, int x) {
    if (x == 0) return 0u;
    const int y = out_h - 1;
    return (bm[(long)(y >> 5) * out_w + (x - 1)] >> (y & 31)) & 1u;
}

MSAM_DEVINL int col_transitions(const uint32_t* __restrict__ bm, int wpc, int out_w, int out_h, int x, uint32_t prev) {
    int cnt = 0;
    for (int yw = 0; yw < wpc; ++yw) {
        uint32_t w = bm[(long)yw * out_w + x];
        const int nb = min(32, out_h - yw * 32);
        uint32_t shifted = (w << 1) | prev;
        uint32_t diff = w ^ shifted;
        if (nb < 32) diff &= (1u << nb) - 1u;
        cnt += __popc(diff);
        prev = (w >> (nb - 1)) & 1u;
    }
    return cnt;
}

__global__ __launch_bounds__(256) void rle_count_kernel(const uint32_t* __restrict__ bits, int out_h, int out_w,
                                                        int* __restrict__ n_runs) {
    __shared__ int red[4];
    const int n = blockIdx.x, wpc = (out_h + 31) >> 5;
    const uint32_t* bm = bits + (long)n * wpc * out_w;
    int cnt = 0;
    for (int x = threadIdx.x; x < out_w; x += 256) cnt += col_transitions(bm, wpc, out_w, out_h, x, col_prev_bit(bm, wpc, out_w, out_h, x));
#pragma unroll
    for (int s = 1; s < 64; s <<= 1) cnt += __shfl_xor(cnt, s);
    if ((threadIdx.x & 63) == 0) red[threadIdx.x >> 6] = cnt;
    __syncthreads();
    if (threadIdx.x == 0) n_runs[n] = red[0] + red[1] + red[2] + red[3] + 1;
}

__global__ __launch_bounds__(256) void rle_encode_kernel(const uint32_t* __restrict__ bits, int out_h, int out_w,
                                                         const long* __restrict__ offsets, int* __restrict__ out) {
    __shared__ int scan[256];
    __shared__ int carry;
    const int n = blockIdx.x, wpc = (out_h + 31) >> 5, tid = threadIdx.x;
    const uint32_t* bm = bits + (long)n * wpc * out_w;
    int* dst = out + offsets[n];
    if (tid == 0) carry = 0;
    __syncthreads();
    for (int x0 = 0; x0 < out_w; x0 += 256) {
        const int x = x0 + tid;
        uint32_t prev = 0; int cnt = 0;
        if (x < out_w) { prev = col_prev_bit(bm, wpc, out_w, out_h, x); cnt = col_transitions(bm, wpc, out_w, out_h, x, prev); }
        scan[tid] = cnt;
        __syncthreads();
        for (int s = 1; s < 256; s <<= 1) {
            int v = tid >= s ? scan[tid - s] : 0;
            __syncthreads();
            scan[tid] += v;
            __syncthreads();
        }
        int k = carry + scan[tid] - cnt;
        if (x < out_w) {
            for (int yw = 0; yw < wpc; ++yw) {
                uint32_t w = bm[(long)yw * out_w + x];
                const int nb = min(32, out_h - yw * 32);
                uint32_t diff = w ^ ((w << 1) | prev);
                if (nb < 32) diff &= (1u << nb) - 1u;
                while (diff) {
                    const int b = __ffs(diff) - 1;
                    diff &= diff - 1;
                    dst[k++] = x * out_h + yw * 32 + b;
                }
                prev = (w >> (nb - 1)) & 1u;
            }
        }
        __syncthreads();
        if (tid == 255) carry += scan[255];
        __syncthreads();
    }
    const int ntrans = carry;
    const int L = out_w * out_h;
    const int nchunks = (ntrans + 1 + 255) / 256;
    for (int ch = nchunks - 1; ch >= 0; --ch) {
        const int k = ch * 256 + tid;
        int val = 0; bool ok = k <= ntrans;
        if (ok) {
            const int cur = k < ntrans ? dst[k] : L;
            const int prv = k > 0 ? dst[k - 1] : 0;
            val = cur - prv;
        }
        __syncthreads();
        if (ok) dst[k] = val;
        __syncthreads();
    }
}

}

extern "C" int msam_postprocess_masks16(const void* low_res, int32_t low_res_dtype, int32_t N, int32_t in_h, int32_t in_w, int32_t out_h,
                                        int32_t out_w, float thr, float off, int32_t* counts, int32_t* boxes, uint32_t* bits,
                                        float* logits, void* stream) {
    if (!low_res || !counts || !boxes || !bits || N <= 0) { msam_set_error("msam_postprocess_masks: null argument"); return 1; }
    if (low_res_dtype != MSAM_F32 && low_res_dtype != MSAM_F16) { msam_set_error("msam_postprocess_masks16: low_res_dtype is MSAM_F32 or MSAM_F16"); return 1; }
    if (in_h <= 0 || in_w <= 0 || in_h > 1024 || in_w > 1024 || out_h <= 0 || out_w <= 0) {
        msam_set_error("msam_postprocess_masks: bad sizes");
        return 1;
    }
    if (N > 65535) { msam_set_error("msam_postprocess_masks: at most 65535 masks per call"); return 1; }
    hipStream_t s = (hipStream_t)stream;
    hipLaunchKernelGGL(init_stats_kernel, dim3((N + 255) / 256), dim3(256), 0, s, counts, boxes, N);
    dim3 grid((out_w + 255) / 256, N);
#define PP_LAUNCH(TS_, LG_)                                                                                                              \
    do {                                                                                                                                 \
        if (low_res_dtype == MSAM_F16)                                                                                                   \
            hipLaunchKernelGGL((postprocess_kernel<TS_, LG_, lowh_t>), grid, dim3(256), 0, s, (const lowh_t*)low_res, in_h, in_w,        \
                               out_h, out_w, thr, off, counts, boxes, bits, logits);                                                     \
        else                                                                                                                             \
            hipLaunchKernelGGL((postprocess_kernel<TS_, LG_, float>), grid, dim3(256), 0, s, (const float*)low_res, in_h, in_w, out_h,   \
                               out_w, thr, off, counts, boxes, bits, logits);                                                            \
    } while (0)
    const bool direct = in_h == out_h && in_w == out_w;
    if (direct && !logits) PP_LAUNCH(false, false);
    else if (direct) PP_LAUNCH(false, true);
    else if (!logits) PP_LAUNCH(true, false);
    else PP_LAUNCH(true, true);
#undef PP_LAUNCH
    hipLaunchKernelGGL(finalize_boxes_kernel, dim3((N + 255) / 256), dim3(256), 0, s, boxes, N);
    return msam_check_launch("msam_postprocess_masks");
}

extern "C" int msam_postprocess_masks(const float* low_res, int32_t N, int32_t in_h, int32_t in_w, int32_t out_h,
                                      int32_t out_w, float thr, float off, int32_t* counts, int32_t* boxes, uint32_t* bits,
                                      float* logits, void* stream) {
    return msam_postprocess_masks16(low_res, MSAM_F32, N, in_h, in_w, out_h, out_w, thr, off, counts, boxes, bits, logits, stream);
}

__global__ __launch_bounds__(256) void uncrop_bits_kernel(const uint32_t* __restrict__ in, int ch, int cw, int x0, int y0,
                                                          int H, int W, uint32_t* __restrict__ out) {
    const int x = blockIdx.x * 256 + threadIdx.x, yw = blockIdx.y, n = blockIdx.z;
    if (x >= W) return;
    const int wpc_in = (ch + 31) >> 5, wpc_out = (H + 31) >> 5;
    uint32_t word = 0u;
    const int xs = x - x0;
    if (xs >= 0 && xs < cw) {
        const int base = yw * 32 - y0;
        const uint32_t* src = in + (long)n * wpc_in * cw + xs;
        if (base >= 0) {
            const int wl = base >> 5, sh = base & 31;
            if (wl < wpc_in) word = src[(long)wl * cw] >> sh;
            if (sh && wl + 1 < wpc_in) word |= src[(long)(wl + 1) * cw] << (32 - sh);
        } else if (base > -32) {
            word = src[0] << (-base);
        }
        const int rows = min(32, H - yw * 32);
        if (rows < 32) word &= (1u << rows) - 1u;
    }
    out[((long)n * wpc_out + yw) * W + x] = word;
}

extern "C" int msam_uncrop_bits(const uint32_t* bits_crop, int32_t N, int32_t crop_h, int32_t crop_w, int32_t x0, int32_t y0,
                                int32_t out_h, int32_t out_w, uint32_t* bits_out, void* stream) {
    if (!bits_crop || !bits_out || N <= 0 || crop_h <= 0 || crop_w <= 0 || out_h <= 0 || out_w <= 0 || x0 < 0 || y0 < 0 ||
        x0 + crop_w > out_w || y0 + crop_h > out_h) {
        msam_set_error("msam_uncrop_bits: bad arguments (the crop must lie inside the output image)");
        return 1;
    }
    if (N > 65535) { msam_set_error("msam_uncrop_bits: at most 65535 masks per call"); return 1; }
    dim3 grid((out_w + 255) / 256, (out_h + 31) / 32, N);
    hipLaunchKernelGGL(uncrop_bits_kernel, grid, dim3(256), 0, (hipStream_t)stream, bits_crop, crop_h, crop_w, x0, y0, out_h,
                       out_w, bits_out);
    return msam_check_launch("msam_uncrop_bits");
}

extern "C" int msam_rle_run_counts(const uint32_t* bits, int32_t N, int32_t out_h, int32_t out_w, int32_t* n_runs,
                                   void* stream) {
    if (!bits || !n_runs || N <= 0 || out_h <= 0 || out_w <= 0) { msam_set_error("msam_rle_run_counts: bad arguments"); return 1; }
    hipLaunchKernelGGL(rle_count_kernel, dim3(N), dim3(256), 0, (hipStream_t)stream, bits, out_h, out_w, n_runs);
    return msam_check_launch("msam_rle_run_counts");
}

extern "C" int msam_rle_encode(const uint32_t* bits, int32_t N, int32_t out_h, int32_t out_w, const int64_t* offsets,
                               int32_t* counts_out, void* stream) {
    if (!bits || !offsets || !counts_out || N <= 0) { msam_set_error("msam_rle_encode: bad arguments"); return 1; }
    hipLaunchKernelGGL(rle_encode_kernel, dim3(N), dim3(256), 0, (hipStream_t)stream, bits, out_h, out_w,
                       (const long*)offsets, counts_out);
    return msam_check_launch("msam_rle_encode");
}
```

### micro_sam_amd/csrc/upfused.hip

```cpp
#include "common.h"
#include "../../include/msam_hip.h"

void msam_set_error(const char* msg);
int msam_check_launch(const char* what);
void msam_profile_mark2(void* stream, int begin, double flops, double bytes, int family);

namespace {

constexpr int T = 4096, C = 256, TK = 16, NTHR = 256;
int g_uf_prio = 1;
}
int g_tune_up_gelu16 = 1;
int g_tune_up_centred = 1;
int g_tune_up_ln_two_pass = 0;
namespace {
constexpr int SUB_BYTES = TK * 64 + 64, XT_BYTES = 8 * SUB_BYTES;
constexpr int W2_BYTES = 128 * 128;
constexpr int PATCH = 3 * 4 * 64;

struct UpArgs {
    const u16* keys;
    const u16* w1; const float* b1;
    const float* lnw; const float* lnb; float eps;
    const u16* w2; const float* b2;
    const float* hyper; int hyper_ld, mask0, nmask;
    int nitems, KS;
    void* out;
    int out16;
    int blocked;
    int centred;
};

MSAM_DEVINL float wave_rows_sum(float v) {
    const auto a = __builtin_amdgcn_permlane16_swap(__float_as_uint(v), __float_as_uint(v), false, false);
    const float t = __uint_as_float(a[0]) + __uint_as_float(a[1]);
    const auto b = __builtin_amdgcn_permlane32_swap(__float_as_uint(t), __float_as_uint(t), false, false);
    return __uint_as_float(b[0]) + __uint_as_float(b[1]);
}
typedef _Float16 h16x2_t __attribute__((ext_vector_type(2)));
typedef unsigned short u16x2_t __attribute__((ext_vector_type(2)));
template <int EXPM>
MSAM_DEVINL uint32_t gelu_pk_h(float x0, float x1) {
    const f32x2_t xf = {x0, x1};
    const h16x2_t x = __builtin_convertvector(xf, h16x2_t);
    const h16x2_t zero = {(_Float16)0.f, (_Float16)0.f};
    const h16x2_t r = __builtin_elementwise_max(x, zero);
    const h16x2_t t = r * (_Float16)2.f - x;
    h16x2_t q = t * (_Float16)-0.0248758f + (_Float16)-0.49884797f;
    q = q * t + (_Float16)-1.12922424f;
    q = q * t + (_Float16)-1.00353579f;
    h16x2_t e;
    if constexpr (EXPM == 2) {
        e = q;
    } else if constexpr (EXPM == 3) {
        const h16x2_t lim = {(_Float16)-13.f, (_Float16)-13.f};
        const h16x2_t qc = __builtin_elementwise_max(q, lim);
        const h16x2_t sm = qc + (_Float16)1536.f;
        const h16x2_t rr = sm - (_Float16)1536.f;
        const h16x2_t f = qc - rr;
        h16x2_t pz = f * (_Float16)0.0555041f + (_Float16)0.2402265f;
        pz = pz * f + (_Float16)0.6931472f;
        pz = pz * f + (_Float16)1.0f;
        const u16x2_t sh = __builtin_bit_cast(u16x2_t, sm) << (unsigned short)10;
        e = __builtin_bit_cast(h16x2_t, (u16x2_t)(__builtin_bit_cast(u16x2_t, pz) + sh));
    } else {
        uint32_t ew_;
        asm("v_exp_f16_sdwa %0, %1 dst_sel:WORD_0 dst_unused:UNUSED_PRESERVE src0_sel:WORD_0\n\ts_nop 0\n\t"
            "v_exp_f16_sdwa %0, %1 dst_sel:WORD_1 dst_unused:UNUSED_PRESERVE src0_sel:WORD_1\n\ts_nop 0"
            : "=&v"(ew_) : "v"(__builtin_bit_cast(uint32_t, q)));
        e = __builtin_bit_cast(h16x2_t, ew_);
    }
    const h16x2_t g = r - t * e;
    return __builtin_bit_cast(uint32_t, g);
}

template <int EXPM>
MSAM_DEVINL void gelu_pk_h2(float x0, float x1, float x2, float x3, uint32_t& g01, uint32_t& g23) {
    if constexpr (EXPM != 1) {
        g01 = gelu_pk_h<EXPM == 0 ? 1 : EXPM>(x0, x1); g23 = gelu_pk_h<EXPM == 0 ? 1 : EXPM>(x2, x3);
        return;
    }
    const h16x2_t zero = {(_Float16)0.f, (_Float16)0.f};
    const h16x2_t xa = __builtin_convertvector(f32x2_t{x0, x1}, h16x2_t), xb = __builtin_convertvector(f32x2_t{x2, x3}, h16x2_t);
    const h16x2_t ra = __builtin_elementwise_max(xa, zero), rb = __builtin_elementwise_max(xb, zero);
    const h16x2_t ta = ra * (_Float16)2.f - xa, tb = rb * (_Float16)2.f - xb;
    h16x2_t qa = ta * (_Float16)-0.0248758f + (_Float16)-0.49884797f, qb = tb * (_Float16)-0.0248758f + (_Float16)-0.49884797f;
    qa = qa * ta + (_Float16)-1.12922424f; qb = qb * tb + (_Float16)-1.12922424f;
    qa = qa * ta + (_Float16)-1.00353579f; qb = qb * tb + (_Float16)-1.00353579f;
    uint32_t ea_, eb_;
    asm("v_exp_f16_sdwa %0, %2 dst_sel:WORD_0 dst_unused:UNUSED_PRESERVE src0_sel:WORD_0\n\t"
        "v_exp_f16_sdwa %1, %3 dst_sel:WORD_0 dst_unused:UNUSED_PRESERVE src0_sel:WORD_0\n\t"
        "v_exp_f16_sdwa %0, %2 dst_sel:WORD_1 dst_unused:UNUSED_PRESERVE src0_sel:WORD_1\n\t"
        "v_exp_f16_sdwa %1, %3 dst_sel:WORD_1 dst_unused:UNUSED_PRESERVE src0_sel:WORD_1\n\ts_nop 0"
        : "=&v"(ea_), "=&v"(eb_) : "v"(__builtin_bit_cast(uint32_t, qa)), "v"(__builtin_bit_cast(uint32_t, qb)));
    g01 = __builtin_bit_cast(uint32_t, (h16x2_t)(ra - ta * __builtin_bit_cast(h16x2_t, ea_)));
    g23 = __builtin_bit_cast(uint32_t, (h16x2_t)(rb - tb * __builtin_bit_cast(h16x2_t, eb_)));
}

template <int UF_PRIO, int G16, int LN2P = 0, int CEN = 0>
__global__ __launch_bounds__(NTHR, 2) void up_fused_kernel(UpArgs a) {
#define UF_LDS_AHEAD 1
#if defined(__HIP_DEVICE_COMPILE__) && UF_LDS_AHEAD
#define UF_R16(dst_, base_, imm_) asm volatile("ds_read_b128 %0, %1 offset:%2" : "=v"(dst_) : "v"(base_), "n"(imm_))
#define UF_LDS_ADDR(ptr_) ((uint32_t)(size_t)(ptr_))
#define UF_ARRIVED2(n_, x0_, tok_) asm volatile("s_waitcnt lgkmcnt(" #n_ ")" : "+v"(x0_), "+v"(tok_))
#define UF_ARRIVED4(n_, x0_, x1_, x2_, tok_) asm volatile("s_waitcnt lgkmcnt(" #n_ ")" : "+v"(x0_), "+v"(x1_), "+v"(x2_), "+v"(tok_))
#define UF_ARRIVED6(n_, x0_, x1_, x2_, x3_, x4_, tok_) asm volatile("s_waitcnt lgkmcnt(" #n_ ")" : "+v"(x0_), "+v"(x1_), "+v"(x2_), "+v"(x3_), "+v"(x4_), "+v"(tok_))
#else
#define UF_R16(dst_, base_, imm_) dst_ = *(const f32x4_t*)((base_) + (imm_))
#define UF_LDS_ADDR(ptr_) ((const unsigned char*)(ptr_))
#define UF_ARRIVED2(n_, x0_, tok_) (void)0
#define UF_ARRIVED4(n_, x0_, x1_, x2_, tok_) (void)0
#define UF_ARRIVED6(n_, x0_, x1_, x2_, x3_, x4_, tok_) (void)0
#endif
    __shared__ __attribute__((aligned(16))) unsigned char lds[2 * XT_BYTES + W2_BYTES];
    __shared__ __attribute__((aligned(16))) float patch[2][PATCH + 4 * 64];
    __shared__ __attribute__((aligned(16))) float prm[256 + 64 + 64 + 32];
#if UF_LDS_AHEAD
    __shared__ __attribute__((aligned(16))) uint4 hyp[4][2][64];
#endif
    unsigned char* const W2L = lds + 2 * XT_BYTES;
    const int tid = threadIdx.x, lane = tid & 63, w = __builtin_amdgcn_readfirstlane(tid >> 6), fr = lane & 15, fg = lane >> 4;
    const int sub = w;
    const int ks_sh = __builtin_ctz(a.KS), tpi_sh = 8 - ks_sh, TPI = 1 << tpi_sh;
    const int my_items = (a.nitems - (int)blockIdx.x + (int)gridDim.x - 1) / (int)gridDim.x;
    const int nq = my_items * TPI;
    if (nq <= 0) return;

    for (int i = tid; i < 416; i += NTHR) prm[i] = i < 256 ? a.b1[i] : i < 320 ? a.lnw[i - 256] : i < 384 ? a.lnb[i - 320] : a.b2[i - 384];
#pragma unroll
    for (int j = 0; j < 4; ++j) {
        const int id = j * NTHR + tid, row = id >> 3, ch = id & 7, kk = ch >> 2, g = ch & 3;
        const uint2 lo = *(const uint2*)(a.w2 + row * 64 + kk * 32 + g * 4);
        const uint2 hi = *(const uint2*)(a.w2 + row * 64 + kk * 32 + 16 + g * 4);
        *(uint4*)(W2L + row * 128 + ((ch ^ ((row >> 1) & 7)) << 4)) = make_uint4(lo.x, lo.y, hi.x, hi.y);
    }
    uint4 w1f[4][8];
#pragma unroll
    for (int rt = 0; rt < 4; ++rt)
#pragma unroll
        for (int ks = 0; ks < 8; ++ks)
            w1f[rt][ks] = *(const uint4*)(a.w1 + (long)(sub * 64 + rt * 16 + fr) * C + ks * 32 + fg * 8);
    wait_vmem_all();

    uint4 ra0, ra1, rb0, rb1;
    int kdst[2];
#pragma unroll
    for (int i = 0; i < 2; ++i) {
        const int id = i * NTHR + tid;
        const int row = a.blocked ? id & 15 : id >> 5, c = a.blocked ? (id >> 6) * 4 + ((id >> 4) & 3) : id & 31;
        kdst[i] = (c >> 2) * SUB_BYTES + row * 64 + (((c & 3) ^ ((row >> 2) & 3)) << 4);
    }
    auto tile_pos = [&](int q, int& p, int& key0) {
        const int item = (int)blockIdx.x + (q >> tpi_sh) * (int)gridDim.x;
        p = __builtin_amdgcn_readfirstlane(item >> ks_sh);
        key0 = __builtin_amdgcn_readfirstlane((item & (a.KS - 1)) * (T >> ks_sh) + (q & (TPI - 1)) * TK);
    };
    const int voff = tid * 16;
    int lq = 0, lsoff;
    const u16* lbase;
    {
        int p_, k0_;
        tile_pos(0, p_, k0_);
        lbase = a.keys + (long)p_ * T * C; lsoff = k0_ * C * 2;
    }
    auto load_advance = [&]() {
        if (lq < nq - 1) {
            ++lq;
            if ((lq & (TPI - 1)) == 0) {
                int p_, k0_;
                tile_pos(lq, p_, k0_);
                lbase = a.keys + (long)p_ * T * C; lsoff = k0_ * C * 2;
            } else {
                lsoff += TK * C * 2;
            }
        }
    };
#define UF_LOAD(r0_, r1_)                                                                          \
    do {                                                                                           \
        const rsrc_t rx_ = make_rsrc(lbase, T * C * 2);                                            \
        r0_ = buf_load16(rx_, voff, lsoff); r1_ = buf_load16(rx_, voff, lsoff + NTHR * 16);        \
        load_advance();                                                                            \
    } while (0)
#define UF_STORE(r0_, r1_, buf_)                                                                   \
    do {                                                                                           \
        unsigned char* b_ = lds + (buf_) * XT_BYTES;                                               \
        *(uint4*)(b_ + kdst[0]) = r0_; *(uint4*)(b_ + kdst[1]) = r1_;                              \
    } while (0)

    const int boff = fr * 64 + ((fg ^ ((fr >> 2) & 3)) << 4);
    const int w2off = fr * 128;
    const int w2sw = (fr >> 1) & 7;
    const float* const b1p = prm + sub * 64 + fg * 4;
#if !UF_LDS_AHEAD
    uint4 hh = make_uint4(0, 0, 0, 0), hl = hh;
    f32x4_t b2a, b2b;
    {
        const float4 ba = *(const float4*)(a.b2 + fg * 4), bb = *(const float4*)(a.b2 + 16 + fg * 4);
        b2a = f32x4_t{ba.x, ba.y, ba.z, ba.w}; b2b = f32x4_t{bb.x, bb.y, bb.z, bb.w};
    }
#endif
    wait_vmem_all();

    auto stage1 = [&](const unsigned char* B, f32x4_t (&u)[4]) {
#pragma unroll
        for (int rt = 0; rt < 4; ++rt) u[rt] = *(const f32x4_t*)(b1p + rt * 16);
#pragma unroll
        for (int ks = 0; ks < 8; ++ks) {
            const uint4 kf = *(const uint4*)(B + boff + ks * SUB_BYTES);
#pragma unroll
            for (int rt = 0; rt < 4; ++rt) u[rt] = mfma16d(w1f[rt][ks], kf, u[rt]);
        }
    };

    f32x4_t ua[4], ub[4];
    UF_LOAD(ra0, ra1);
    UF_LOAD(rb0, rb1);
    __syncthreads();
    UF_STORE(ra0, ra1, 0);
    UF_STORE(rb0, rb1, 1);
    UF_LOAD(ra0, ra1);
    __syncthreads();
    stage1(lds, ua);
    __syncthreads();
#if UF_LDS_AHEAD
    f32x4_t kfa, kfb;
#define UF_NEXT_TILE(B_, u_)                                                                       \
    do {                                                                                           \
        UF_R16(u_[0], b1a, 0); UF_R16(u_[1], b1a, 64); UF_R16(u_[2], b1a, 128); UF_R16(u_[3], b1a, 192); \
        const auto bn_ = UF_LDS_ADDR((B_) + boff);                                                 \
        UF_R16(kfa, bn_, 0); UF_R16(kfb, bn_, SUB_BYTES);                                          \
    } while (0)
    const auto b1a = UF_LDS_ADDR(b1p), prma = UF_LDS_ADDR(&prm[256 + fg * 4]);
    UF_NEXT_TILE(lds + XT_BYTES, ub);
#endif

    if ((int)blockIdx.x >= ((int)gridDim.x >> 1)) __builtin_amdgcn_s_sleep(11);
    const int oesz = a.out16 ? 1 : 2;
    const int ptoff = ((lane >> 4) * 4 + w) * 64 + (lane & 15) * 4;
    const int ovoff = ((((lane >> 4) * 256 + w) * 256) + (lane & 15) * 4) << oesz;
    float4 o4c = make_float4(0.f, 0.f, 0.f, 0.f);
    const char* obase_c = (const char*)a.out;
    uint32_t orange_c = 0;
    int osoff_c = 0;
    auto store_previous = [&]() {
        const int oso = __builtin_amdgcn_readfirstlane(osoff_c);
        const unsigned long long ob_ = (unsigned long long)obase_c;
        const char* obu = (const char*)(((unsigned long long)(uint32_t)__builtin_amdgcn_readfirstlane((int)(ob_ >> 32)) << 32) |
                                        (uint32_t)__builtin_amdgcn_readfirstlane((int)(uint32_t)ob_));
        const rsrc_t ro = make_rsrc(obu, (uint32_t)__builtin_amdgcn_readfirstlane((int)orange_c));
        if (__builtin_amdgcn_readfirstlane(oesz) == 1) buf_store8(make_uint2(pack2h(o4c.x, o4c.y), pack2h(o4c.z, o4c.w)), ro, ovoff, oso);
        else buf_store16(make_uint4(__float_as_uint(o4c.x), __float_as_uint(o4c.y), __float_as_uint(o4c.z), __float_as_uint(o4c.w)), ro, ovoff, oso);
    };
    int q = 0, p = 0, key0 = 0;
    const char* obase = (const char*)a.out;
    auto iteration = [&](uint4& p0, uint4& p1, uint4& f0, uint4& f1, f32x4_t (&uc)[4], f32x4_t (&un)[4]) {
        UF_LOAD(f0, f1);
        if ((q & (TPI - 1)) != 0) {
            key0 += TK;
        } else {
            tile_pos(q, p, key0);
            obase = (const char*)a.out + (((long)p * a.nmask) << (16 + oesz));
            float h8[8] = {0.f, 0.f, 0.f, 0.f, 0.f, 0.f, 0.f, 0.f};
            if (fr < a.nmask) {
                const float* hp = a.hyper + ((long)p * 4 + a.mask0 + fr) * a.hyper_ld;
                const float4 x0 = *(const float4*)(hp + fg * 4), x1 = *(const float4*)(hp + 16 + fg * 4);
                h8[0] = x0.x; h8[1] = x0.y; h8[2] = x0.z; h8[3] = x0.w; h8[4] = x1.x; h8[5] = x1.y; h8[6] = x1.z; h8[7] = x1.w;
            }
            wait_vmem_all();
#if UF_LDS_AHEAD
            uint4 hh, hl;
#endif
            hh = make_uint4(pack2h(h8[0], h8[1]), pack2h(h8[2], h8[3]), pack2h(h8[4], h8[5]), pack2h(h8[6], h8[7]));
            const uint32_t hw_[4] = {hh.x, hh.y, hh.z, hh.w};
            float l8[8];
#pragma unroll
            for (int i = 0; i < 4; ++i) { l8[2 * i] = h8[2 * i] - h2f(hw_[i] & 0xffff); l8[2 * i + 1] = h8[2 * i + 1] - h2f(hw_[i] >> 16); }
            hl = make_uint4(pack2h(l8[0], l8[1]), pack2h(l8[2], l8[3]), pack2h(l8[4], l8[5]), pack2h(l8[6], l8[7]));
#if UF_LDS_AHEAD
            hyp[w][0][lane] = hh; hyp[w][1][lane] = hl;
#endif
        }
        const unsigned char* Bn = lds + ((q + 1) & 1) * XT_BYTES;
#if UF_LDS_AHEAD
        const auto bna = UF_LDS_ADDR(Bn + boff);
#endif
#if !UF_LDS_AHEAD
#pragma unroll
        for (int rt = 0; rt < 4; ++rt) un[rt] = *(const f32x4_t*)(b1p + rt * 16);
#endif
#if UF_LDS_AHEAD
#define UF_MF_(ks_, between_)                                                                      \
        do {                                                                                       \
            f32x4_t& kf_ = ((ks_) & 1) ? kfb : kfa;                                                \
            const uint4 kw_ = make_uint4(__float_as_uint(kf_[0]), __float_as_uint(kf_[1]), __float_as_uint(kf_[2]), __float_as_uint(kf_[3])); \
            _Pragma("unroll") for (int rt_ = 0; rt_ < 4; ++rt_) un[rt_] = mfma16d(w1f[rt_][ks_], kw_, un[rt_]); \
            between_;                                                                              \
            if ((ks_) + 2 < 8) UF_R16(kf_, bna, (((ks_) + 2) & 7) * SUB_BYTES);                    \
        } while (0)
#define UF_MF(ks_) UF_MF_(ks_, (void)0)
#define UF_S1(ks_, tok_, n_)                                                                       \
        do {                                                                                       \
            if ((ks_) & 1) UF_ARRIVED2(n_, kfb, tok_); else UF_ARRIVED2(n_, kfa, tok_);            \
            UF_MF(ks_);                                                                            \
        } while (0)
#else
#define UF_MF(ks_) (void)0
#define UF_S1(ks_, tok_, n_) UF_S1_(ks_, tok_)
#define UF_S1_(ks_, tok_)                                                                          \
        do {                                                                                       \
            uint4 kf_ = *(const uint4*)(Bn + boff + (ks_) * SUB_BYTES);                            \
            asm volatile("" : "+v"(kf_.x), "+v"(tok_));                                            \
            _Pragma("unroll") for (int rt_ = 0; rt_ < 4; ++rt_) un[rt_] = mfma16d(w1f[rt_][ks_], kf_, un[rt_]); \
        } while (0)
#endif
#if UF_LDS_AHEAD
        { int first_ = 0; UF_ARRIVED6(1, un[0], un[1], un[2], un[3], kfa, first_); }
        UF_MF_(0, store_previous());
        f32x4_t gq[2], bq[2];
        UF_R16(gq[0], prma, 0); UF_R16(bq[0], prma, 256);
#else
        { int first_ = 0; UF_S1(0, first_, 0); }
        store_previous();
#endif
        float s = 0.f, ss = 0.f;
#pragma unroll
        for (int rt = 0; rt < 4; ++rt) {
            if constexpr (!CEN) s += (uc[rt][0] + uc[rt][1]) + (uc[rt][2] + uc[rt][3]);
#pragma unroll
            for (int r = 0; r < 4; ++r) ss += uc[rt][r] * uc[rt][r];
        }
        if constexpr (!CEN) s = wave_rows_sum(s);
        ss = wave_rows_sum(ss);
        float mean = s * (1.f / 64.f);
        __builtin_amdgcn_sched_barrier(0);
        if constexpr (CEN) UF_S1(1, ss, 3); else UF_S1(1, mean, 3);
        if constexpr (!CEN) {
#pragma unroll
            for (int rt = 0; rt < 4; ++rt)
#pragma unroll
                for (int r = 0; r < 4; ++r) uc[rt][r] -= mean;
        }
        __builtin_amdgcn_sched_barrier(0);
        if constexpr (LN2P) {
            float s2 = 0.f;
#pragma unroll
            for (int rt = 0; rt < 4; ++rt)
#pragma unroll
                for (int r = 0; r < 4; ++r) s2 += uc[rt][r] * uc[rt][r];
            ss = wave_rows_sum(s2);
        }
        UF_S1(2, ss, 3);
        float rstd = (LN2P || CEN) ? rsqrtf(ss * (1.f / 64.f) + a.eps) : rsqrtf(fmaxf(ss * (1.f / 64.f) - mean * mean, 0.f) + a.eps);
        __builtin_amdgcn_sched_barrier(0);
        uint32_t g1w[4][2];
#pragma unroll
        for (int rt = 0; rt < 4; ++rt) {
#if UF_LDS_AHEAD
            f32x4_t& kfr = (rt & 1) ? kfa : kfb;
            if (rt == 0) UF_ARRIVED4(1, gq[0], bq[0], kfr, rstd); else UF_ARRIVED4(1, gq[rt & 1], bq[rt & 1], kfr, g1w[rt - 1][1]);
            const float4 g4 = make_float4(gq[rt & 1][0], gq[rt & 1][1], gq[rt & 1][2], gq[rt & 1][3]);
            const float4 b4 = make_float4(bq[rt & 1][0], bq[rt & 1][1], bq[rt & 1][2], bq[rt & 1][3]);
            if (rt < 3) { UF_R16(gq[(rt + 1) & 1], prma, ((rt + 1) & 3) * 64); UF_R16(bq[(rt + 1) & 1], prma, 256 + ((rt + 1) & 3) * 64); }
            UF_MF(3 + rt);
#else
            if (rt == 0) UF_S1(3, rstd, 0); else UF_S1(3 + rt, g1w[rt - 1][1], 0);
            const float4 g4 = *(const float4*)&prm[256 + rt * 16 + fg * 4], b4 = *(const float4*)&prm[320 + rt * 16 + fg * 4];
#endif
            if (G16) {
                gelu_pk_h2<G16>(uc[rt][0] * rstd * g4.x + b4.x, uc[rt][1] * rstd * g4.y + b4.y, uc[rt][2] * rstd * g4.z + b4.z,
                                uc[rt][3] * rstd * g4.w + b4.w, g1w[rt][0], g1w[rt][1]);
            } else {
                const f32x2_t g01 = gelu_erf2(f32x2_t{uc[rt][0] * rstd * g4.x + b4.x, uc[rt][1] * rstd * g4.y + b4.y});
                const f32x2_t g23 = gelu_erf2(f32x2_t{uc[rt][2] * rstd * g4.z + b4.z, uc[rt][3] * rstd * g4.w + b4.w});
                g1w[rt][0] = pack2d(g01.x, g01.y); g1w[rt][1] = pack2d(g23.x, g23.y);
            }
            __builtin_amdgcn_sched_barrier(0);
        }
        UF_S1(7, g1w[3][1], 0);
#undef UF_S1
#undef UF_MF
        uint4 g1[2];
#pragma unroll
        for (int kk = 0; kk < 2; ++kk) g1[kk] = make_uint4(g1w[2 * kk][0], g1w[2 * kk][1], g1w[2 * kk + 1][0], g1w[2 * kk + 1][1]);
        float* pt = patch[q & 1];
        f32x4_t ya[4], yb[4], ov[4];
        uint4 gh[4];
#if UF_LDS_AHEAD
        const f32x4_t b2a = *(const f32x4_t*)&prm[384 + fg * 4], b2b = *(const f32x4_t*)&prm[400 + fg * 4];
        const uint4 hh = hyp[w][0][lane], hl = hyp[w][1][lane];
#endif
        auto stage2 = [&](int s2) {
            f32x4_t xa = b2a, xb = b2b;
#pragma unroll
            for (int kk = 0; kk < 2; ++kk) {
                const uint4 wa = *(const uint4*)(W2L + (s2 * 2) * 2048 + w2off + (((kk * 4 + fg) ^ w2sw) << 4));
                const uint4 wb = *(const uint4*)(W2L + (s2 * 2 + 1) * 2048 + w2off + (((kk * 4 + fg) ^ w2sw) << 4));
                xa = mfma16d(wa, g1[kk], xa);
                xb = mfma16d(wb, g1[kk], xb);
            }
            ya[s2] = xa; yb[s2] = xb;
        };
        auto act2 = [&](int s2) {
            if (G16) {
                gelu_pk_h2<G16>(ya[s2][0], ya[s2][1], ya[s2][2], ya[s2][3], gh[s2].x, gh[s2].y);
                gelu_pk_h2<G16>(yb[s2][0], yb[s2][1], yb[s2][2], yb[s2][3], gh[s2].z, gh[s2].w);
                return;
            }
            const f32x2_t a01 = gelu_erf2(f32x2_t{ya[s2][0], ya[s2][1]}), a23 = gelu_erf2(f32x2_t{ya[s2][2], ya[s2][3]});
            const f32x2_t b01 = gelu_erf2(f32x2_t{yb[s2][0], yb[s2][1]}), b23 = gelu_erf2(f32x2_t{yb[s2][2], yb[s2][3]});
            gh[s2] = make_uint4(pack2h(a01.x, a01.y), pack2h(a23.x, a23.y), pack2h(b01.x, b01.y), pack2h(b23.x, b23.y));
        };
        auto stage3 = [&](int s2) {
            f32x4_t o = {0.f, 0.f, 0.f, 0.f};
            o = mfma16h(hh, gh[s2], o);
            o = mfma16h(hl, gh[s2], o);
            ov[s2] = o;
        };
        stage2(0); stage2(1);
        act2(0);
        stage2(2);
        act2(1);
        stage3(0); stage2(3);
        act2(2);
        stage3(1);
        act2(3);
        stage3(2); stage3(3);
        if (fg == 0) {
#pragma unroll
            for (int sub2 = 0; sub2 < 4; ++sub2) {
                const int yl = (sub >> 1) * 2 + (sub2 >> 1), xl = fr * 4 + (sub & 1) * 2 + (sub2 & 1);
                pt[(0 * 4 + yl) * 64 + xl] = ov[sub2][0];
                pt[(1 * 4 + yl) * 64 + xl] = ov[sub2][1];
                pt[(2 * 4 + yl) * 64 + xl] = ov[sub2][2];
            }
        }
        UF_STORE(p0, p1, q & 1);
        __syncthreads();
#if UF_LDS_AHEAD
        UF_NEXT_TILE(lds + (q & 1) * XT_BYTES, uc);
#endif
        o4c = *(const float4*)&pt[ptoff];
        obase_c = obase; orange_c = (uint32_t)a.nmask << (16 + oesz);
        osoff_c = (((key0 >> 6) << 10) + ((key0 & 63) << 2)) << oesz;
    };
    while (true) {
        iteration(ra0, ra1, rb0, rb1, ua, ub);
        if (++q >= nq) break;
        iteration(rb0, rb1, ra0, ra1, ub, ua);
        if (++q >= nq) break;
    }
    store_previous();
#undef UF_LOAD
#undef UF_STORE
}

}

extern "C" int msam_upscale_fused_out(const void* keys, int32_t keys_blocked, int32_t P, const void* w1, const float* b1,
                                      const float* ln_w, const float* ln_b, float ln_eps, const void* w2, const float* b2,
                                      const float* hyper, int32_t hyper_ld, int32_t mask0, int32_t nmask, void* low_res,
                                      int32_t low_res_dtype, void* stream);
extern "C" int msam_upscale_fused_layout(const void* keys, int32_t keys_blocked, int32_t P, const void* w1, const float* b1,
                                         const float* ln_w, const float* ln_b, float ln_eps, const void* w2, const float* b2,
                                         const float* hyper, int32_t hyper_ld, int32_t mask0, int32_t nmask, float* low_res,
                                         void* stream) {
    return msam_upscale_fused_out(keys, keys_blocked, P, w1, b1, ln_w, ln_b, ln_eps, w2, b2, hyper, hyper_ld, mask0, nmask, low_res,
                                  MSAM_F32, stream);
}
extern "C" int msam_upscale_fused(const void* keys, int32_t P, const void* w1, const float* b1, const float* ln_w,
                                  const float* ln_b, float ln_eps, const void* w2, const float* b2, const float* hyper,
                                  int32_t hyper_ld, int32_t mask0, int32_t nmask, float* low_res, void* stream) {
    return msam_upscale_fused_layout(keys, 0, P, w1, b1, ln_w, ln_b, ln_eps, w2, b2, hyper, hyper_ld, mask0, nmask, low_res, stream);
}

extern "C" int msam_upscale_fused_out(const void* keys, int32_t keys_blocked, int32_t P, const void* w1, const float* b1,
                                      const float* ln_w, const float* ln_b, float ln_eps, const void* w2, const float* b2,
                                      const float* hyper, int32_t hyper_ld, int32_t mask0, int32_t nmask, void* low_res,
                                      int32_t low_res_dtype, void* stream) {
    if (low_res_dtype != MSAM_F32 && low_res_dtype != MSAM_F16) {
        msam_set_error("msam_upscale_fused_out: low_res_dtype is MSAM_F32 or MSAM_F16");
        return 1;
    }
    if (!keys || !w1 || !b1 || !ln_w || !ln_b || !w2 || !b2 || !hyper || !low_res || P <= 0) {
        msam_set_error("msam_upscale_fused: null argument");
        return 1;
    }
    if (nmask < 1 || nmask > 3 || mask0 < 0 || mask0 + nmask > 4 || hyper_ld < 32 || hyper_ld % 4) {
        msam_set_error("msam_upscale_fused: 1 <= nmask <= 3 masks out of 4, hyper_ld >= 32 and a multiple of 4");
        return 1;
    }
    UpArgs a{};
    a.keys = (const u16*)keys; a.w1 = (const u16*)w1; a.b1 = b1; a.lnw = ln_w; a.lnb = ln_b; a.eps = ln_eps;
    a.w2 = (const u16*)w2; a.b2 = b2; a.hyper = hyper; a.hyper_ld = hyper_ld; a.mask0 = mask0; a.nmask = nmask;
    int dev = 0, cus = 256;
    (void)hipGetDevice(&dev);
    (void)hipDeviceGetAttribute(&cus, hipDeviceAttributeMultiprocessorCount, dev);
    int ks = 1;
    while (P * ks < 2 * cus && ks < 16) ks *= 2;
    a.KS = ks; a.nitems = P * ks; a.out = low_res; a.out16 = low_res_dtype == MSAM_F16; a.blocked = keys_blocked & 1; a.centred = (keys_blocked >> 1) & 1;
    const int grid = a.nitems < 2 * cus ? a.nitems : 2 * cus;
    const double rows = (double)P * T;
    const double flops = rows * (2.0 * 256 * 256 + 4 * 2.0 * 128 * 64 + 16 * 3 * 2.0 * 16 * 32);
    const double bytes = rows * C * 2 + (double)P * nmask * 256 * 256 * (low_res_dtype == MSAM_F16 ? 2 : 4);
    msam_profile_mark2(stream, 1, flops, bytes, 4);
#if MSAM_DEC_F16
    if (g_tune_up_gelu16 == 2) hipLaunchKernelGGL((up_fused_kernel<1, 2>), dim3(grid), dim3(NTHR), 0, (hipStream_t)stream, a);
    else if (g_tune_up_gelu16 == 3) hipLaunchKernelGGL((up_fused_kernel<1, 3>), dim3(grid), dim3(NTHR), 0, (hipStream_t)stream, a);
    else if (g_tune_up_gelu16) {
        if (g_tune_up_ln_two_pass) hipLaunchKernelGGL((up_fused_kernel<1, 1, 1>), dim3(grid), dim3(NTHR), 0, (hipStream_t)stream, a);
        else if (g_uf_prio && a.centred && g_tune_up_centred) hipLaunchKernelGGL((up_fused_kernel<1, 1, 0, 1>), dim3(grid), dim3(NTHR), 0, (hipStream_t)stream, a);
        else if (g_uf_prio) hipLaunchKernelGGL((up_fused_kernel<1, 1>), dim3(grid), dim3(NTHR), 0, (hipStream_t)stream, a);
        else hipLaunchKernelGGL((up_fused_kernel<0, 1>), dim3(grid), dim3(NTHR), 0, (hipStream_t)stream, a);
    } else
#endif
    if (g_tune_up_ln_two_pass) hipLaunchKernelGGL((up_fused_kernel<1, 0, 1>), dim3(grid), dim3(NTHR), 0, (hipStream_t)stream, a);
    else if (g_uf_prio && a.centred && g_tune_up_centred) hipLaunchKernelGGL((up_fused_kernel<1, 0, 0, 1>), dim3(grid), dim3(NTHR), 0, (hipStream_t)stream, a);
    else if (g_uf_prio) hipLaunchKernelGGL((up_fused_kernel<1, 0>), dim3(grid), dim3(NTHR), 0, (hipStream_t)stream, a);
    else hipLaunchKernelGGL((up_fused_kernel<0, 0>), dim3(grid), dim3(NTHR), 0, (hipStream_t)stream, a);
    msam_profile_mark2(stream, 0, flops, bytes, 4);
    return msam_check_launch("up_fused");
}

extern "C" int msam_upscale_set_prio(int32_t prio) { g_uf_prio = prio; return 0; }
```

### micro_sam_amd/modeling.py

```python
from __future__ import annotations

import ctypes as C
import os
from typing import List, Optional, Tuple

import torch
import torch.nn as nn
import torch.nn.functional as F

from . import _lib

VIT_CONFIGS = {
    "vit_b": dict(embed_dim=768, depth=12, num_heads=12, global_attn_indexes=(2, 5, 8, 11)),
    "vit_l": dict(embed_dim=1024, depth=24, num_heads=16, global_attn_indexes=(5, 11, 17, 23)),
    "vit_h": dict(embed_dim=1280, depth=32, num_heads=16, global_attn_indexes=(7, 15, 23, 31)),
}
IMG_SIZE, PATCH, GRID, WINDOW, PROMPT_DIM = 1024, 16, 64, 14, 256


def _bf16(t: torch.Tensor) -> torch.Tensor:
    return t.detach().to(torch.bfloat16).contiguous()


def _d16(t: torch.Tensor) -> torch.Tensor:
    return t.detach().to(_lib.decoder_dtype()).contiguous()


class _ParamWatch:

    def __init__(self, *modules) -> None:
        self._modules = modules
        self._slots = None

    def reset(self) -> None:
        self._slots = None

    def key(self) -> int:
        if self._slots is None:
            self._slots = [(m._parameters, name) for root in self._modules for m in root.modules() for name in m._parameters]
        acc = []
        for d, name in self._slots:
            q = d.get(name)
            if q is not None:
                acc.append((id(q), q._version, q.data_ptr(), q.device.index))
        return hash(tuple(acc))


def _split16(w: torch.Tensor) -> torch.Tensor:
    w = w.detach().to(torch.float32)
    hi = w.to(_lib.decoder_dtype())
    lo = (w - hi.to(torch.float32)).to(_lib.decoder_dtype())
    return torch.cat([hi, hi, lo], dim=1).contiguous()


def _f32(t: torch.Tensor) -> torch.Tensor:
    return t.detach().to(torch.float32).contiguous()


class LayerNorm2d(nn.Module):
    def __init__(self, num_channels: int, eps: float = 1e-6) -> None:
        super().__init__()
        self.weight = nn.Parameter(torch.ones(num_channels))
        self.bias = nn.Parameter(torch.zeros(num_channels))
        self.eps = eps


class MLPBlock(nn.Module):
    def __init__(self, dim: int, mlp_dim: int, act=nn.GELU) -> None:
        super().__init__()
        self.lin1 = nn.Linear(dim, mlp_dim)
        self.lin2 = nn.Linear(mlp_dim, dim)
        self.act = act()


class _ViTAttention(nn.Module):
    def __init__(self, dim: int, num_heads: int, input_size: int) -> None:
        super().__init__()
        self.num_heads = num_heads
        head_dim = dim // num_heads
        self.scale = head_dim ** -0.5
        self.qkv = nn.Linear(dim, dim * 3, bias=True)
        self.proj = nn.Linear(dim, dim)
        self.use_rel_pos = True
        self.rel_pos_h = nn.Parameter(torch.zeros(2 * input_size - 1, head_dim))
        self.rel_pos_w = nn.Parameter(torch.zeros(2 * input_size - 1, head_dim))


# ... 514 lines not shown
        state = torch.empty(lib.msam_decoder_image_bytes(), dtype=torch.uint8, device=self.device)
        _lib.check(lib.msam_decoder_prepare_image(C.byref(p), consts.data_ptr(), feats.data_ptr(), state.data_ptr(),
                                                  None, 0, _lib.stream_ptr()), "msam_decoder_prepare_image")
        self._img_state = (key, state, feats, features)
        return state

    def _workspace(self, P: int) -> torch.Tensor:
        need = _lib.load().msam_decoder_workspace_bytes(P)
        if self._dec_ws is None or self._dec_ws.numel() < need or self._dec_ws.device != self.device:
            self._dec_ws = None
            self._dec_ws = torch.empty(need, dtype=torch.uint8, device=self.device)
        return self._dec_ws

    @torch.no_grad()
    def _prompt_encode(self, points, boxes, masks):
        p, _, _ = self._prepare_decoder()
        dev = self.device
        pts = lbl = bx = msk = None
        if points is not None:
            pts = points[0].to(device=dev, dtype=torch.float32).contiguous()
            lbl = points[1].to(device=dev, dtype=torch.int32).contiguous()
            B, Np = pts.shape[0], pts.shape[1]
        else:
            Np = 0
            B = boxes.shape[0] if boxes is not None else (masks.shape[0] if masks is not None else 1)
        if boxes is not None:
            bx = boxes.to(device=dev, dtype=torch.float32).reshape(-1, 4).contiguous()
        if masks is not None:
            msk = masks.to(device=dev, dtype=torch.float32).reshape(-1, 4 * GRID, 4 * GRID).contiguous()
            if msk.shape[0] != B:
                raise ValueError(f"masks holds {msk.shape[0]} masks for {B} prompts")
        Ns = Np + (2 if boxes is not None else (1 if Np > 0 else 0))
        sparse = torch.empty((B, Ns, PROMPT_DIM), dtype=torch.float32, device=dev)
        dense = torch.empty((B, PROMPT_DIM, GRID, GRID), dtype=torch.float32, device=dev) if msk is not None else None
        if Ns > 0 or msk is not None:
            self._mask_params.exact_gelu = 1 if self.reference_formulation else 0
            _lib.check(_lib.load().msam_prompt_encode(
                C.byref(p), C.byref(self._mask_params), _lib.ptr(pts), _lib.ptr(lbl), Np, _lib.ptr(bx), _lib.ptr(msk), B,
                _lib.ptr(sparse) if Ns > 0 else None, _lib.ptr(dense), _lib.stream_ptr()), "msam_prompt_encode")
        if dense is None:
            dense = self.prompt_encoder.no_mask_embed.weight.detach().to(dev).reshape(1, -1, 1, 1).expand(B, -1, GRID, GRID)
        return sparse, dense

    @torch.no_grad()
    def _decode_embeddings(self, image_embeddings, image_pe, sparse, dense, multimask_output: bool):
        if image_embeddings.numel() != PROMPT_DIM * GRID * GRID:
            raise NotImplementedError("micro_sam_amd: mask_decoder takes ONE image embedding [1,256,64,64] per call "
                                      f"(got {tuple(image_embeddings.shape)})")
        p, _, consts = self._prepare_decoder()
        dev = self.device
        if self.reference_formulation:
            nm = self.prompt_encoder.no_mask_embed.weight.detach().to(dev).reshape(1, -1, 1, 1)
            dn = dense.to(device=dev, dtype=torch.float32)
            no_mask = (dn.stride(-1) == 0 and dn.stride(-2) == 0 and torch.equal(dn[:, :, :1, :1], nm.expand(dn.shape[0], -1, 1, 1))) \
                or bool(torch.equal(dn, nm.expand_as(dn)))
            return self._decode_strict(image_embeddings, sparse.to(device=dev, dtype=torch.float32), None if no_mask else dn,
                                       multimask_output)
        own_pe = self._dense_pe()
        if image_pe is not None and (tuple(image_pe.shape) != tuple(own_pe.shape) or
                                     not torch.allclose(image_pe.to(device=dev, dtype=torch.float32), own_pe, atol=1e-5)):
            raise NotImplementedError("micro_sam_amd: mask_decoder needs image_pe == prompt_encoder.get_dense_pe() "
                                      "(the positional projections are precomputed tables)")
        state = self._image_state(image_embeddings)
        sp = sparse.to(device=dev, dtype=torch.float32).contiguous()
        P, Ns = sp.shape[0], sp.shape[1]
        if Ns > 11:
            raise ValueError(f"at most 11 sparse prompt tokens per prompt, got {Ns}")
        nm = self.prompt_encoder.no_mask_embed.weight.detach().to(dev).reshape(1, -1, 1, 1)
        dn = dense.to(device=dev, dtype=torch.float32)
        is_no_mask = (dn.stride(-1) == 0 and dn.stride(-2) == 0 and torch.equal(dn[:, :, :1, :1], nm.expand(dn.shape[0], -1, 1, 1))) \
            or bool(torch.equal(dn, nm.expand_as(dn)))
        dptr = eptr = None
        if not is_no_mask:
            if dn.shape[0] != P:
                raise ValueError(f"dense_prompt_embeddings holds {dn.shape[0]} entries for {P} prompts")
            dn = dn.contiguous()
            emb = image_embeddings.to(device=dev, dtype=torch.float32).reshape(PROMPT_DIM, GRID * GRID).contiguous()
            dptr, eptr = dn.data_ptr(), emb.data_ptr()
        nc = 3 if multimask_output else 1
        low = torch.empty((P, nc, 256, 256), dtype=torch.float32, device=dev)
        iou = torch.empty((P, nc), dtype=torch.float32, device=dev)
        ws = self._workspace(P)
        p.low_res_dtype = _lib.F32
        _lib.check(_lib.load().msam_decoder_forward_embeddings(
            C.byref(p), consts.data_ptr(), state.data_ptr(), sp.data_ptr() if Ns > 0 else None, Ns, dptr, eptr, P,
            1 if multimask_output else 0, low.data_ptr(), iou.data_ptr(), ws.data_ptr(), ws.numel(), _lib.stream_ptr()),
            "msam_decoder_forward_embeddings")
        return low, iou

    @torch.no_grad()
    def decode(self, features: torch.Tensor, point_coords: Optional[torch.Tensor], point_labels: Optional[torch.Tensor],
               boxes: Optional[torch.Tensor] = None, mask_input: Optional[torch.Tensor] = None,
               multimask_output: bool = True, low_res_dtype: torch.dtype = torch.float32) -> Tuple[torch.Tensor, torch.Tensor]:
        if low_res_dtype not in (torch.float32, torch.float16):
            raise ValueError("low_res_dtype is torch.float32 or torch.float16")
        if features.numel() != PROMPT_DIM * GRID * GRID:
            raise ValueError(f"expected one image embedding [1,256,64,64], got {tuple(features.shape)}")
        if self.reference_formulation:
            if point_coords is None and boxes is None and mask_input is None:
                raise ValueError("micro_sam_amd: a prompt needs points, a box and / or a mask input")
            pts = None if point_coords is None else (point_coords, point_labels)
            msk = None if mask_input is None else mask_input.reshape(-1, 1, 4 * GRID, 4 * GRID)
            sparse, dense = self._prompt_encode(pts, None if boxes is None else boxes.reshape(-1, 4), msk)
            low, iou = self._decode_strict(features, sparse, dense if mask_input is not None else None, multimask_output)
            return (low if low_res_dtype == torch.float32 else low.to(low_res_dtype)), iou
        prepared = self._prepare_decoder()
        p, _, consts = prepared
        state = self._image_state(features, prepared)
        lib = _lib.load()
        dev = self.device
        if point_coords is not None:
            pts = point_coords.to(device=dev, dtype=torch.float32).contiguous()
            lbl = point_labels.to(device=dev, dtype=torch.int32).contiguous()
            P, Np = pts.shape[0], pts.shape[1]
        else:
            if boxes is None and mask_input is None:
                raise ValueError("micro_sam_amd: a prompt needs points, a box and / or a mask input")
            pts = lbl = None
            P, Np = (boxes.shape[0] if boxes is not None else mask_input.reshape(-1, 4 * GRID, 4 * GRID).shape[0]), 0
        bx = None if boxes is None else boxes.to(device=dev, dtype=torch.float32).reshape(-1, 4).contiguous()
        nc = 3 if multimask_output else 1
        low = torch.empty((P, nc, 256, 256), dtype=low_res_dtype, device=dev)
        iou = torch.empty((P, nc), dtype=torch.float32, device=dev)
        p.low_res_dtype = _lib.F16 if low_res_dtype == torch.float16 else _lib.F32
        need = lib.msam_decoder_workspace_bytes(P)
        if self._dec_ws is None or self._dec_ws.numel() < need or self._dec_ws.device != dev:
            self._dec_ws = None
            self._dec_ws = torch.empty(need, dtype=torch.uint8, device=dev)
        msk = None
        if mask_input is not None:
            msk = mask_input.to(device=dev, dtype=torch.float32).reshape(-1, 4 * GRID, 4 * GRID).contiguous()
            if msk.shape[0] != P:
                raise ValueError(f"mask_input holds {msk.shape[0]} masks for {P} prompts")
        _lib.check(lib.msam_decoder_forward_masks(
            C.byref(p), C.byref(self._mask_params), consts.data_ptr(), state.data_ptr(), _lib.ptr(pts), _lib.ptr(lbl), Np,
            _lib.ptr(bx), _lib.ptr(msk), P, 1 if multimask_output else 0, low.data_ptr(), iou.data_ptr(),
            self._dec_ws.data_ptr(), self._dec_ws.numel(), _lib.stream_ptr()), "msam_decoder_forward")
        return low, iou


def build_sam(model_type: str = "vit_b", num_multimask_outputs: int = 3) -> Sam:
    key = model_type[:5]
    if key == "vit_t":
        from .models.tiny_vit import TinyViT
        sam = Sam(TinyViT(), PromptEncoder(), MaskDecoder(num_multimask_outputs))
        sam.eval()
        return sam
    if key not in VIT_CONFIGS:
        raise ValueError(f"Invalid model_type: {model_type}. Expect one of {tuple(VIT_CONFIGS) + ('vit_t',)}")
    cfg = VIT_CONFIGS[key]
    sam = Sam(ImageEncoderViT(cfg["embed_dim"], cfg["depth"], cfg["num_heads"], cfg["global_attn_indexes"]),
              PromptEncoder(), MaskDecoder(num_multimask_outputs))
    sam.eval()
    return sam


sam_model_registry = {
    "vit_b": lambda **kw: build_sam("vit_b", **kw),
    "vit_l": lambda **kw: build_sam("vit_l", **kw),
    "vit_h": lambda **kw: build_sam("vit_h", **kw),
    "vit_t": lambda **kw: build_sam("vit_t", **kw),
}
```

### micro_sam_amd/ops.py

```python
from __future__ import annotations

import ctypes as C
from typing import Any, Dict, List, Optional, Tuple

import numpy as np
import torch

from . import _lib
from ._lib import ACT_GELU, ACT_NONE, ACT_RELU, BF16, F16, F32


_CODE16 = {torch.float32: F32, torch.bfloat16: BF16, torch.float16: F16}
_F32, _I32, _I64, _U8 = torch.float32, torch.int32, torch.int64, torch.uint8
_BITS = (torch.int32, torch.uint32)


def _code(name: str, dtype: torch.dtype) -> int:
    try:
        return _CODE16[dtype]
    except KeyError:
        raise TypeError(f"micro_sam_amd: {name} must be float32, bfloat16 or float16, got {dtype}") from None


def _home(name: str, t) -> torch.device:
# ... 253 lines not shown
        out = torch.empty((B, H, neww, Cc), dtype=torch.uint8, device=x.device)
        _lib.check(lib.msam_resample_u8(x.data_ptr(), B, H, W, Cc, 1, neww, b.data_ptr(), c.data_ptr(), int(c.shape[1]), out.data_ptr(),
                                        _lib.stream_ptr()), "msam_resample_u8")
        x, W = out, neww
    if newh != H:
        b, c = tables(H, newh)
        out = torch.empty((B, newh, W, Cc), dtype=torch.uint8, device=x.device)
        _lib.check(lib.msam_resample_u8(x.data_ptr(), B, H, W, Cc, 0, newh, b.data_ptr(), c.data_ptr(), int(c.shape[1]), out.data_ptr(),
                                        _lib.stream_ptr()), "msam_resample_u8")
        x = out
    return x


def patchify(img: torch.Tensor) -> torch.Tensor:
    _t("img", img, _F32, (None, 3, 1024, 1024), _home("img", img))
    B = img.shape[0]
    out = torch.empty((B * 4096, 768), dtype=torch.bfloat16, device=img.device)
    _lib.check(_lib.load().msam_patchify(img.data_ptr(), B, out.data_ptr(), _lib.stream_ptr()), "msam_patchify")
    return out


def patchify_u8(img: torch.Tensor) -> torch.Tensor:
    _t("img", img, _U8, (None, None, None, 3), _home("img", img))
    B, h, w = img.shape[:3]
    _need(1 <= h <= 1024 and 1 <= w <= 1024, f"img must be [B, h <= 1024, w <= 1024, 3], got {list(img.shape)}")
    out = torch.empty((B * 4096, 768), dtype=torch.bfloat16, device=img.device)
    _lib.check(_lib.load().msam_patchify_u8(img.data_ptr(), B, h, w, out.data_ptr(), _lib.stream_ptr()), "msam_patchify_u8")
    return out


def im2col3x3(x: torch.Tensor) -> torch.Tensor:
    _t("x", x, torch.bfloat16, (None, 64, 64, None), _home("x", x))
    B, _, _, Cc = x.shape
    _need(Cc % 8 == 0, f"x must have C % 8 == 0 channels, got {list(x.shape)}")
    out = torch.empty((B * 4096, 9 * Cc), dtype=torch.bfloat16, device=x.device)
    _lib.check(_lib.load().msam_im2col3x3(x.data_ptr(), B, Cc, out.data_ptr(), _lib.stream_ptr()), "msam_im2col3x3")
    return out


def _enc16(*tensors) -> int:
    dts = {t.dtype for t in tensors}
    if dts == {torch.bfloat16}:
        return _lib.BF16
    if dts == {torch.float16}:
        return _lib.F16
    raise ValueError(f"expected all-bfloat16 or all-float16 operands, got {sorted(str(d) for d in dts)}")


def _attention_operands(q, k, v, rel_h, rel_w, rel_rows: int) -> int:
    dev = _home("q", q)
    _t("q", q, (torch.bfloat16, torch.float16), (None, None, 4096, None), dev)
    _need(q.shape[3] in (64, 96), f"q must have a stored head_dim of 64 or 96, got {list(q.shape)}")
    for name, t in (("k", k), ("v", v)):
        _t(name, t, q.dtype, tuple(q.shape), dev)
    for name, t in (("rel_h", rel_h), ("rel_w", rel_w)):
        _t(name, t, q.dtype, (rel_rows, q.shape[3]), dev)
    return _enc16(q, k, v, rel_h, rel_w)


def window_attention(q, k, v, rel_h, rel_w, qkv_bias, scale: Optional[float] = None) -> torch.Tensor:
    dt = _attention_operands(q, k, v, rel_h, rel_w, 27)
    B, heads, _, hd = q.shape
    _t("qkv_bias", qkv_bias, _F32, (3 * heads * hd,), q.device)
    out = torch.empty((B * 4096, heads * hd), dtype=q.dtype, device=q.device)
    _lib.check(_lib.load().msam_window_attention16(q.data_ptr(), k.data_ptr(), v.data_ptr(), rel_h.data_ptr(), rel_w.data_ptr(),
                                                   qkv_bias.data_ptr(), B, heads, hd, float(hd ** -0.5 if scale is None else scale),
                                                   dt, out.data_ptr(), _lib.stream_ptr()),
               "msam_window_attention")
    return out


def global_attention(q, k, v, rel_h, rel_w, scale: Optional[float] = None) -> torch.Tensor:
    dt = _attention_operands(q, k, v, rel_h, rel_w, 127)
    B, heads, _, hd = q.shape
    out = torch.empty((B * 4096, heads * hd), dtype=q.dtype, device=q.device)
    _lib.check(_lib.load().msam_global_attention16(q.data_ptr(), k.data_ptr(), v.data_ptr(), rel_h.data_ptr(), rel_w.data_ptr(),
                                                   B, heads, hd, float(hd ** -0.5 if scale is None else scale), dt, out.data_ptr(),
                                                   _lib.stream_ptr()), "msam_global_attention")
    return out


def postprocess_masks(low_res: torch.Tensor, input_size: Tuple[int, int], original_size: Tuple[int, int],
                      mask_threshold: float = 0.0, stability_offset: float = 1.0,
                      want_logits: bool = False) -> Dict[str, torch.Tensor]:
    _home("low_res", low_res)
    _need(low_res.dim() == 3 and tuple(low_res.shape[1:]) == (256, 256), f"low_res must be [N,256,256], got {list(low_res.shape)}")
    low_res = low_res.contiguous() if low_res.dtype == torch.float16 else low_res.to(torch.float32).contiguous()
    low_dt = _lib.F16 if low_res.dtype == torch.float16 else _lib.F32
    N = low_res.shape[0]
    H, W = int(original_size[0]), int(original_size[1])
    dev = low_res.device
    counts = torch.empty((N, 3), dtype=torch.int32, device=dev)
    boxes = torch.empty((N, 4), dtype=torch.int32, device=dev)
    bits = torch.empty((N, (H + 31) // 32, W), dtype=torch.int32, device=dev)
    logits = torch.empty((N, H, W), dtype=torch.float32, device=dev) if want_logits else None
    lib = _lib.load()
    step = 65535
    for s in range(0, N, step):
        n = min(step, N - s)
        _lib.check(lib.msam_postprocess_masks16(
            low_res[s:].data_ptr(), low_dt, n, int(input_size[0]), int(input_size[1]), H, W, float(mask_threshold),
            float(stability_offset), counts[s:].data_ptr(), boxes[s:].data_ptr(), bits[s:].data_ptr(),
            None if logits is None else logits[s:].data_ptr(), _lib.stream_ptr()), "msam_postprocess_masks")
    out = {"counts": counts, "boxes": boxes, "bits": bits}
    if want_logits:
        out["logits"] = logits
    return out


def rle_encode(bits: torch.Tensor, height: int, width: int) -> Tuple[torch.Tensor, torch.Tensor]:
    _t("bits", bits, _BITS, (None, (height + 31) // 32, width), _home("bits", bits))
    N = bits.shape[0]
    lib = _lib.load()
    n_runs = torch.empty((N,), dtype=torch.int32, device=bits.device)
    _lib.check(lib.msam_rle_run_counts(bits.data_ptr(), N, height, width, n_runs.data_ptr(), _lib.stream_ptr()),
               "msam_rle_run_counts")
    offsets = torch.zeros((N + 1,), dtype=torch.int64, device=bits.device)
    torch.cumsum(n_runs, 0, out=offsets[1:])
    total = int(offsets[-1].item())
    counts = torch.empty((total,), dtype=torch.int32, device=bits.device)
    _lib.check(lib.msam_rle_encode(bits.data_ptr(), N, height, width, offsets.data_ptr(), counts.data_ptr(),
                                   _lib.stream_ptr()), "msam_rle_encode")
    return counts, offsets


def rles_to_list(counts: torch.Tensor, offsets: torch.Tensor, height: int, width: int,
                 as_list: bool = True) -> List[Dict[str, Any]]:
    c = counts.cpu().numpy()
    o = offsets.cpu().numpy()
    if as_list:
        return [{"size": [height, width], "counts": c[o[i]:o[i + 1]].tolist()} for i in range(len(o) - 1)]
    return [{"size": [height, width], "counts": c[o[i]:o[i + 1]]} for i in range(len(o) - 1)]


def unpack_bits(bits: torch.Tensor, height: int) -> torch.Tensor:
    N, wpc, W = bits.shape
    sh = torch.arange(32, device=bits.device, dtype=torch.int32).view(1, 1, 32, 1)
    m = ((bits.unsqueeze(2) >> sh) & 1).to(torch.bool).reshape(N, wpc * 32, W)
    return m[:, :height]


def paint_label_image(bits: torch.Tensor, order: torch.Tensor, height: int, width: int) -> torch.Tensor:
    _t("bits", bits, _BITS, (None, (height + 31) // 32, width), _home("bits", bits))
    _need(isinstance(order, torch.Tensor) and order.dim() == 1, "order must be a 1-d tensor of mask indices")
    label = torch.empty((height, width), dtype=torch.int32, device=bits.device)
    order = order.to(device=bits.device, dtype=torch.int32).contiguous()
    _lib.check(_lib.load().msam_paint_label_image(bits.data_ptr() if order.numel() else None,
                                                  order.data_ptr() if order.numel() else None, order.numel(), height, width,
                                                  label.data_ptr(), _lib.stream_ptr()), "msam_paint_label_image")
    return label


def _seg2d(seg) -> torch.Tensor:
    _home("seg", seg)
    if seg.dtype != torch.int32:
        raise TypeError(f"micro_sam_amd: seg must be int32, got {seg.dtype}")
    _need(seg.dim() == 2, f"seg must be [H,W], got {list(seg.shape)}")
    return seg.contiguous()


def label_components(seg: torch.Tensor) -> torch.Tensor:
    seg = _seg2d(seg)
    h, w = seg.shape
    roots = torch.empty((h * w,), dtype=torch.int32, device=seg.device)
    flag = torch.zeros((1,), dtype=torch.int32, device=seg.device)
    iters = C.c_int32(0)
    _lib.check(_lib.load().msam_label_components(seg.data_ptr(), h, w, roots.data_ptr(), flag.data_ptr(), 16, C.byref(iters),
                                                 _lib.stream_ptr()), "msam_label_components")
    return roots


def _boxes_scores(boxes, scores, valid=None) -> None:
    dev = _home("boxes", boxes)
    _need(boxes.dim() == 2 and boxes.shape[1] == 4, f"boxes must be [K,4], got {list(boxes.shape)}")
    k = boxes.shape[0]
    _need(isinstance(scores, torch.Tensor) and tuple(scores.shape) == (k,), f"scores must be [{k}] like boxes")
    _need(scores.device == dev, f"scores lives on {scores.device}, boxes on {dev}")
    if valid is not None:
        _need(isinstance(valid, torch.Tensor) and tuple(valid.shape) == (k,), f"valid must be [{k}] like boxes")
        if valid.dtype != torch.bool:
            raise TypeError(f"micro_sam_amd: valid must be bool, got {valid.dtype}")
        _need(valid.device == dev, f"valid lives on {valid.device}, boxes on {dev}")
# ... 644 lines not shown
```

### micro_sam_amd/predictor.py

```python
from __future__ import annotations

from typing import Optional, Tuple

import numpy as np
import torch

from .modeling import Sam
from .transforms import ResizeLongestSide


class SamPredictor:
    def __init__(self, sam_model: Sam) -> None:
        self.model = sam_model
        self.transform = ResizeLongestSide(sam_model.image_encoder.img_size)
        self.reset_image()

    @property
    def device(self) -> torch.device:
        return self.model.device

    def set_precision(self, mode: str) -> None:
        self.model.set_precision(mode)

    def reset_image(self) -> None:
        self.model._img_state = None
        self.is_image_set = False
        self.features = None
        self.orig_h = self.orig_w = self.input_h = self.input_w = None
        self.original_size = None
        self.input_size = None

    def set_image(self, image: np.ndarray, image_format: str = "RGB") -> None:
        assert image_format in ["RGB", "BGR"], f"image_format must be in ['RGB', 'BGR'], is {image_format}."
        if image_format != self.model.image_format:
            image = image[..., ::-1]
        input_image = self.transform.apply_image(image)
        self.reset_image()
        self.original_size = tuple(image.shape[:2])
        self.input_size = tuple(input_image.shape[:2])
        u8 = torch.as_tensor(np.ascontiguousarray(input_image), device=self.device)[None]
        self.features = self.model.image_encoder.forward_u8(u8)
        self.is_image_set = True

    @torch.no_grad()
    def set_torch_image(self, transformed_image: torch.Tensor, original_image_size: Tuple[int, ...]) -> None:
        assert (len(transformed_image.shape) == 4 and transformed_image.shape[1] == 3
                and max(*transformed_image.shape[2:]) == self.model.image_encoder.img_size), \
            f"set_torch_image input must be BCHW with long side {self.model.image_encoder.img_size}."
        self.reset_image()
        self.original_size = tuple(original_image_size)
        self.input_size = tuple(transformed_image.shape[-2:])
        input_image = self.model.preprocess(transformed_image.to(self.device).float())
        self.features = self.model.image_encoder(input_image)
        self.is_image_set = True

    def get_image_embedding(self) -> torch.Tensor:
        if not self.is_image_set:
            raise RuntimeError("An image must be set with .set_image(...) to generate an embedding.")
        assert self.features is not None, "Features must exist if an image has been set."
        return self.features

    def predict(self, point_coords: Optional[np.ndarray] = None, point_labels: Optional[np.ndarray] = None,
                box: Optional[np.ndarray] = None, mask_input: Optional[np.ndarray] = None,
                multimask_output: bool = True, return_logits: bool = False):
        if not self.is_image_set:
            raise RuntimeError("An image must be set with .set_image(...) before mask prediction.")
        coords_torch = labels_torch = box_torch = mask_input_torch = None
        if point_coords is not None:
            assert point_labels is not None, "point_labels must be supplied if point_coords is supplied."
            point_coords = self.transform.apply_coords(point_coords, self.original_size)
            coords_torch = torch.as_tensor(point_coords, dtype=torch.float, device=self.device)[None, :, :]
            labels_torch = torch.as_tensor(point_labels, dtype=torch.int, device=self.device)[None, :]
        if box is not None:
            box = self.transform.apply_boxes(box, self.original_size)
            box_torch = torch.as_tensor(box, dtype=torch.float, device=self.device)[None, :]
        if mask_input is not None:
            mask_input_torch = torch.as_tensor(mask_input, dtype=torch.float, device=self.device)[None, :, :, :]
        masks, iou, low = self.predict_torch(coords_torch, labels_torch, box_torch, mask_input_torch, multimask_output,
                                             return_logits=return_logits)
        return masks[0].detach().cpu().numpy(), iou[0].detach().cpu().numpy(), low[0].detach().cpu().numpy()

    @torch.no_grad()
    def predict_torch(self, point_coords: Optional[torch.Tensor], point_labels: Optional[torch.Tensor],
                      boxes: Optional[torch.Tensor] = None, mask_input: Optional[torch.Tensor] = None,
                      multimask_output: bool = True, return_logits: bool = False):
        if not self.is_image_set:
            raise RuntimeError("An image must be set with .set_image(...) before mask prediction.")
        low, iou = self.model.decode(self.features, point_coords, point_labels, boxes, mask_input, multimask_output)
        from .ops import postprocess_masks, unpack_bits
        b, c = low.shape[:2]
        res = postprocess_masks(low.reshape(b * c, 256, 256), self.input_size, self.original_size,
                                self.model.mask_threshold, 1.0, want_logits=return_logits)
        if return_logits:
            masks = res["logits"].reshape(b, c, *self.original_size)
        else:
            masks = unpack_bits(res["bits"], self.original_size[0]).reshape(b, c, *self.original_size)
        return masks, iou, low

    @torch.no_grad()
    def predict_masks_device(self, point_coords, point_labels, boxes=None, multimask_output: bool = True,
                             stability_score_offset: float = 1.0):
        if not self.is_image_set:
            raise RuntimeError("An image must be set with .set_image(...) before mask prediction.")
        low, iou = self.model.decode(self.features, point_coords, point_labels, boxes, None, multimask_output,
                                     low_res_dtype=self.model.amg_low_res_dtype)
        from .ops import postprocess_masks
        b, c = low.shape[:2]
        res = postprocess_masks(low.reshape(b * c, 256, 256), self.input_size, self.original_size,
                                self.model.mask_threshold, stability_score_offset, want_logits=False)
        return iou, res
```

Before: 180.8 tiles/s.

## Emit per-band logit range map from upscale kernel to shortcut AMG postprocess

Adds a range-emitting variant of the fused upscale kernel. It writes min/max logits per column band of each low-res mask into a small [N,256,4,2] map. A new postprocess entry point reads this map so it can decide whole 32-row bit words as all-ones or all-zeros without running the per-pixel interpolation and threshold work. The path is only used for float32 low-res output at 1024x1024 and is gated by a tune key. The cost is extra global writes for the map and a second kernel template instantiation. It also shares the x4 bit-word logic between the old and new postprocess kernels through helper functions.

New measurement: 185.4 tiles/s, median of 6. 1.03x the previous value.

```diff
diff --git a/include/msam_hip.h b/include/msam_hip.h
--- a/include/msam_hip.h
+++ b/include/msam_hip.h
@@ -126,10 +126,15 @@
                            const float* ln_w, const float* ln_b, float ln_eps, const void* w2, const float* b2,
                            const float* hyper, int32_t hyper_ld, int32_t mask0, int32_t nmask, void* low_res,
                            int32_t low_res_dtype, void* stream);
+int msam_upscale_fused_range(const void* keys, int32_t keys_blocked, int32_t P, const void* w1, const float* b1,
+                             const float* ln_w, const float* ln_b, float ln_eps, const void* w2, const float* b2,
+                             const float* hyper, int32_t hyper_ld, int32_t mask0, int32_t nmask, void* low_res,
+                             int32_t low_res_dtype, float* range, void* stream);
 
 int msam_upscale_set_prio(int32_t prio);
 int msam_fold_attn_set_dma(int32_t on);
 int msam_tune_set(const char* key, int32_t value);
+int msam_tune_get(const char* key, int32_t* value);
 int msam_debug_i2t_timing(int32_t enable, uint64_t* host_out);
 int msam_gemm256_set_staging(int staging);
 int msam_gemm_set_trace(void* device_words);
@@ -271,6 +276,7 @@
     int32_t use_glds;
     int32_t low_res_dtype;
     int32_t up1_centred;
+    float* low_res_range;
 } msam_decoder_t;
 
 int msam_decoder_dtype(void);
@@ -308,6 +314,9 @@
 int msam_postprocess_masks16(const void* low_res, int32_t low_res_dtype, int32_t N, int32_t in_h, int32_t in_w, int32_t out_h,
                              int32_t out_w, float thr, float off, int32_t* counts, int32_t* boxes, uint32_t* bits, float* logits,
                              void* stream);
+int msam_postprocess_masks_range(const float* low_res, const float* range, int32_t N, int32_t in_h, int32_t in_w, int32_t out_h,
+                                 int32_t out_w, float thr, float off, int32_t* counts, int32_t* boxes, uint32_t* bits,
+                                 void* stream);
 int msam_uncrop_bits(const uint32_t* bits_crop, int32_t N, int32_t crop_h, int32_t crop_w, int32_t x0, int32_t y0,
                      int32_t out_h, int32_t out_w, uint32_t* bits_out, void* stream);
 
diff --git a/micro_sam_amd/_lib.py b/micro_sam_amd/_lib.py
--- a/micro_sam_amd/_lib.py
+++ b/micro_sam_amd/_lib.py
@@ -86,7 +86,7 @@
         ("layer", TwoWayLayer * 2), ("final_attn", AttnW), ("nf_w", _vp), ("nf_b", _vp),
         ("up1_w", _vp), ("up1_b", _vp), ("up_ln_w", _vp), ("up_ln_b", _vp), ("up2_w", _vp), ("up2_b", _vp),
         ("hyp_w", (_vp * 3) * 4), ("hyp_b", (_vp * 3) * 4), ("iou_w", _vp * 3), ("iou_b", _vp * 3),
-        ("use_glds", _i32), ("low_res_dtype", _i32), ("up1_centred", _i32),
+        ("use_glds", _i32), ("low_res_dtype", _i32), ("up1_centred", _i32), ("low_res_range", _vp),
     ]
 
 
@@ -156,6 +156,7 @@
     "msam_gemm_group_bf16": (_i32, [_vp, _i32, _vp]),
     "msam_fold_attn_set_dma": (_i32, [_i32]),
     "msam_tune_set": (_i32, [C.c_char_p, _i32]),
+    "msam_tune_get": (_i32, [C.c_char_p, C.POINTER(_i32)]),
     "msam_i2t_fold_operand_bytes": (_i64, [_i32]),
     "msam_i2t_fold_operands": (_i32, [_vp, _vp, _i32, _i32, _vp, _vp, _vp, _i32, _vp, _vp]),
     "msam_i2t0_t2i_workspace_bytes": (_i64, [_i32]),
@@ -178,6 +179,7 @@
     "msam_chain_prepare_tables": (_i32, [_vp, _vp, _vp, _vp, _vp, _vp]),
     "msam_upscale_fused_layout": (_i32, [_vp, _i32, _i32, _vp, _vp, _vp, _vp, _f32, _vp, _vp, _vp, _i32, _i32, _i32, _vp, _vp]),
     "msam_upscale_fused_out": (_i32, [_vp, _i32, _i32, _vp, _vp, _vp, _vp, _f32, _vp, _vp, _vp, _i32, _i32, _i32, _vp, _i32, _vp]),
+    "msam_upscale_fused_range": (_i32, [_vp, _i32, _i32, _vp, _vp, _vp, _vp, _f32, _vp, _vp, _vp, _i32, _i32, _i32, _vp, _i32, _vp, _vp]),
     "msam_upscale_set_prio": (_i32, [_i32]),
     "msam_layernorm_fp8": (_i32, [_vp, _vp, _vp, _f32, _i64, _i32, _vp, _vp, _vp]),
     "msam_quant_rows_fp8": (_i32, [_vp, _i64, _i32, _vp, _vp, _vp]),
@@ -209,6 +211,7 @@
                                     _i64, _vp]),
     "msam_postprocess_masks": (_i32, [_vp, _i32, _i32, _i32, _i32, _i32, _f32, _f32, _vp, _vp, _vp, _vp, _vp]),
     "msam_postprocess_masks16": (_i32, [_vp, _i32, _i32, _i32, _i32, _i32, _i32, _f32, _f32, _vp, _vp, _vp, _vp, _vp]),
+    "msam_postprocess_masks_range": (_i32, [_vp, _vp, _i32, _i32, _i32, _i32, _i32, _f32, _f32, _vp, _vp, _vp, _vp]),
     "msam_rle_run_counts": (_i32, [_vp, _i32, _i32, _i32, _vp, _vp]),
     "msam_rle_encode": (_i32, [_vp, _i32, _i32, _i32, _vp, _vp, _vp]),
     "msam_mask_nms": (_i32, [_vp, _vp, _vp, _vp, _i32, _i32, _i32, _f32, _i32, _vp, _vp, _vp]),
@@ -311,6 +314,12 @@
     return lib
 
 
+def tune_get(key: str) -> int:
+    v = _i32(0)
+    check(load().msam_tune_get(key.encode(), C.byref(v)), "msam_tune_get")
+    return int(v.value)
+
+
 def decoder_dtype() -> torch.dtype:
     return torch.float16 if load().msam_decoder_dtype() == F16 else torch.bfloat16
 
diff --git a/micro_sam_amd/csrc/decfold.hip b/micro_sam_amd/csrc/decfold.hip
--- a/micro_sam_amd/csrc/decfold.hip
+++ b/micro_sam_amd/csrc/decfold.hip
@@ -702,6 +702,7 @@
 extern int g_tune_tok_fuse;
 extern int g_tune_chain_handover, g_tune_chain_handover_ring;
 extern int g_tune_mlp_split_fused;
+extern int g_tune_amg_range_map;
 extern int g_tune_sgemm_bufs, g_tune_srel_mfma, g_tune_sgemm_small_below, g_tune_si2t_dbg, g_tune_si2t_late_us, g_tune_sattn_allh;
 int g_tune_dec_chain = 1, g_tune_dec_chain_min_p = 128;
 extern "C" int msam_tune_set(const char* key, int32_t value) {
@@ -716,6 +717,7 @@
     else if (k == "up_gelu16") g_tune_up_gelu16 = value;
     else if (k == "up_ln_two_pass") g_tune_up_ln_two_pass = value;
     else if (k == "up_centred") g_tune_up_centred = value;
+    else if (k == "amg_range_map") g_tune_amg_range_map = value;
     else if (k == "gemm_dbg") msam_gemm_set_dbg(value);
     else if (k == "gw_delay") msam_gemm_set_gw(value, -1);
     else if (k == "gw_class") msam_gemm_set_gw(-2, value);
@@ -733,3 +735,9 @@
     else { msam_set_error("msam_tune_set: unknown key"); return 1; }
     return 0;
 }
+extern "C" int msam_tune_get(const char* key, int32_t* value) {
+    const std::string k = key ? key : "";
+    if (!value || k != "amg_range_map") { msam_set_error("msam_tune_get: unknown key"); return 1; }
+    *value = g_tune_amg_range_map;
+    return 0;
+}
diff --git a/micro_sam_amd/csrc/decoder.hip b/micro_sam_amd/csrc/decoder.hip
--- a/micro_sam_amd/csrc/decoder.hip
+++ b/micro_sam_amd/csrc/decoder.hip
@@ -906,9 +906,9 @@
     hipLaunchKernelGGL(gather_iou_kernel, dim3((P * nmask + 255) / 256), dim3(256), 0, cx.s, w.iou_full, P, mask0, nmask, iou);
     CHECK(msam_check_launch("gather_iou"));
 
-    CHECK(msam_upscale_fused_out(w.keys, (chain ? 1 : 0) | (dec->up1_centred ? 2 : 0), P, dec->up1_w, dec->up1_b, dec->up_ln_w, dec->up_ln_b, 1e-6f, dec->up2_w,
-                                 dec->up2_b, w.hyper, 128, mask0, nmask, low_res, dec->low_res_dtype == MSAM_F16 ? MSAM_F16 : MSAM_F32,
-                                 cx.s));
+    CHECK(msam_upscale_fused_range(w.keys, (chain ? 1 : 0) | (dec->up1_centred ? 2 : 0), P, dec->up1_w, dec->up1_b, dec->up_ln_w, dec->up_ln_b, 1e-6f, dec->up2_w,
+                                   dec->up2_b, w.hyper, 128, mask0, nmask, low_res, dec->low_res_dtype == MSAM_F16 ? MSAM_F16 : MSAM_F32,
+                                   dec->low_res_range, cx.s));
 #undef CHECK
 #undef ADD_CAST
 #undef ADD_CAST2
diff --git a/micro_sam_amd/csrc/postprocess.hip b/micro_sam_amd/csrc/postprocess.hip
--- a/micro_sam_amd/csrc/postprocess.hip
+++ b/micro_sam_amd/csrc/postprocess.hip
@@ -45,6 +45,118 @@
     if (n >= N) return;
     if (boxes[n * 4 + 2] < boxes[n * 4] || boxes[n * 4 + 3] < boxes[n * 4 + 1]) {
         boxes[n * 4] = 0; boxes[n * 4 + 1] = 0; boxes[n * 4 + 2] = 0; boxes[n * 4 + 3] = 0;
+    }
+}
+
+struct X4Stage { int sr[3], sc[3]; float nx[3]; };
+MSAM_DEVINL void x4_stage_init(X4Stage& st, int cbase) {
+#pragma unroll
+    for (int k = 0; k < 3; ++k) {
+        const int idx = threadIdx.x + k * 256;
+        st.sr[k] = idx / 66; st.sc[k] = min(cbase + idx % 66, 255);
+        st.nx[k] = 0.f;
+    }
+}
+template <typename TL>
+MSAM_DEVINL void x4_patch_load(X4Stage& st, const TL* __restrict__ low, int yw) {
+#pragma unroll
+    for (int k = 0; k < 3; ++k)
+        if (threadIdx.x + k * 256 < 660) st.nx[k] = lowf(low[min(max(yw * 8 - 1 + st.sr[k], 0), 255) * 256 + st.sc[k]]);
+}
+MSAM_DEVINL void x4_patch_store(const X4Stage& st, float* tile) {
+#pragma unroll
+    for (int k = 0; k < 3; ++k)
+        if (threadIdx.x + k * 256 < 660) tile[threadIdx.x + k * 256] = st.nx[k];
+}
+struct X4Acc { int c_hi, c_lo, c_m, ymin, ymax; bool any; };
+
+template <bool LOGITS>
+MSAM_DEVINL void x4_word(const float* tl, const Axis& ax, int l0, int l1, int n, int x, int yw, int wpc, int out_h, int out_w, float thr, float hi_t,
+                         float lo_t, uint32_t* __restrict__ bits, float* __restrict__ logits, X4Acc& acc) {
+    const float W1[4] = {0.625f, 0.875f, 0.125f, 0.375f};
+    float t[10];
+#pragma unroll
+    for (int k = 0; k < 10; ++k) t[k] = lerp_torch(ax.w0, tl[k * 66 + l0], ax.w1, tl[k * 66 + l1]);
+    const int nb = min(32, out_h - yw * 32);
+    uint32_t wm = 0, wh = 0, wl = 0;
+    uint32_t word;
+    if (nb == 32) {
+        int s_hi = 0, s_lo = 0;
+        bool decided = false;
+        if (!LOGITS) {
+            const float tmin = fminf(fminf(fminf(t[0], t[1]), fminf(t[2], t[3])), fminf(fminf(t[4], t[5]), fminf(fminf(t[6], t[7]), fminf(t[8], t[9]))));
+            const float tmax = fmaxf(fmaxf(fmaxf(t[0], t[1]), fmaxf(t[2], t[3])), fmaxf(fmaxf(t[4], t[5]), fmaxf(fmaxf(t[6], t[7]), fmaxf(t[8], t[9]))));
+            const bool one = tmin > hi_t + 0.01f && tmax < 8192.f, zero = tmax < lo_t - 0.01f && tmin > -8192.f;
+            if (__ballot(!(one || zero)) == 0) {
+                decided = true;
+                word = one ? 0xffffffffu : 0u;
+                s_hi = s_lo = 32 * __popcll(__ballot(one));
+            }
+        }
+        if (!decided) {
+#pragma unroll
+            for (int b = 0; b < 32; ++b) {
+                float w1 = W1[b & 3];
+                if (b < 2 && yw == 0) w1 = 0.0f;
+                const float v = lerp_torch(1.0f - w1, t[(b + 2) / 4], w1, t[(b + 2) / 4 + 1]);
+                if (LOGITS) logits[((long)n * out_h + yw * 32 + b) * out_w + x] = v;
+                wm = __builtin_amdgcn_alignbit(wm, __float_as_uint(__fsub_rn(thr, v)), 31);
+                s_hi += __popcll(__ballot(v > hi_t));
+                s_lo += __popcll(__ballot(v > lo_t));
+            }
+            word = __brev(wm);
+        }
+        if ((threadIdx.x & 63) == __ffsll((long long)__ballot(1)) - 1) { acc.c_hi += s_hi; acc.c_lo += s_lo; }
+    } else {
+#pragma unroll
+        for (int b = 0; b < 32; ++b) {
+            float w1 = W1[b & 3];
+            if (b < 2 && yw == 0) w1 = 0.0f;
+            const float v = lerp_torch(1.0f - w1, t[(b + 2) / 4], w1, t[(b + 2) / 4 + 1]);
+            if (LOGITS) { if (b < nb) logits[((long)n * out_h + yw * 32 + b) * out_w + x] = v; }
+            wm = __builtin_amdgcn_alignbit(wm, __float_as_uint(__fsub_rn(thr, v)), 31);
+            wh = __builtin_amdgcn_alignbit(wh, __float_as_uint(__fsub_rn(hi_t, v)), 31);
+            wl = __builtin_amdgcn_alignbit(wl, __float_as_uint(__fsub_rn(lo_t, v)), 31);
+        }
+        const uint32_t valid = (1u << nb) - 1u;
+        word = __brev(wm) & valid;
+        acc.c_hi += __popc(__brev(wh) & valid); acc.c_lo += __popc(__brev(wl) & valid);
+    }
+    if (word) {
+        acc.c_m += __popc(word); acc.any = true;
+        acc.ymin = min(acc.ymin, yw * 32 + __ffs(word) - 1); acc.ymax = yw * 32 + 31 - __clz(word);
+    }
+    bits[((long)n * wpc + yw) * out_w + x] = word;
+}
+
+MSAM_DEVINL void stats_reduce(int (*red)[7], int n, int x, int c_hi, int c_lo, int c_m, int ymin, int ymax, bool any, int* __restrict__ counts,
+                              int* __restrict__ boxes) {
+    int xmin = any ? x : 0x7fffffff, xmax = any ? x : -1;
+#pragma unroll
+    for (int s = 1; s < 64; s <<= 1) {
+        c_hi += __shfl_xor(c_hi, s); c_lo += __shfl_xor(c_lo, s); c_m += __shfl_xor(c_m, s);
+        ymin = min(ymin, __shfl_xor(ymin, s)); ymax = max(ymax, __shfl_xor(ymax, s));
+        xmin = min(xmin, __shfl_xor(xmin, s)); xmax = max(xmax, __shfl_xor(xmax, s));
+    }
+    const int wave = threadIdx.x >> 6;
+    if ((threadIdx.x & 63) == 0) {
+        red[wave][0] = c_hi; red[wave][1] = c_lo; red[wave][2] = c_m; red[wave][3] = xmin; red[wave][4] = ymin;
+        red[wave][5] = xmax; red[wave][6] = ymax;
+    }
+    __syncthreads();
+    if (threadIdx.x == 0) {
+        int hi = 0, lo = 0, m = 0, x0 = 0x7fffffff, y0 = 0x7fffffff, x1 = -1, y1 = -1;
+        for (int w = 0; w < 4; ++w) {
+            hi += red[w][0]; lo += red[w][1]; m += red[w][2];
+            x0 = min(x0, red[w][3]); y0 = min(y0, red[w][4]); x1 = max(x1, red[w][5]); y1 = max(y1, red[w][6]);
+        }
+        if (hi) atomicAdd(&counts[n * 3], hi);
+        if (lo) atomicAdd(&counts[n * 3 + 1], lo);
+        if (m) {
+            atomicAdd(&counts[n * 3 + 2], m);
+            atomicMin(&boxes[n * 4], x0); atomicMin(&boxes[n * 4 + 1], y0);
+            atomicMax(&boxes[n * 4 + 2], x1); atomicMax(&boxes[n * 4 + 3], y1);
+        }
     }
 }
 
@@ -63,88 +175,21 @@
     bool any = false;
     if (!TWO_STAGE) {
         const int cbase = max((int)blockIdx.x * 64 - 1, 0);
-        int sr[3], sc[3];
-#pragma unroll
-        for (int k = 0; k < 3; ++k) {
-            const int idx = threadIdx.x + k * 256;
-            sr[k] = idx / 66; sc[k] = min(cbase + idx % 66, 255);
-        }
-        float nx[3] = {0.f, 0.f, 0.f};
-#define PP_LOAD(yw_)                                                                               \
-        _Pragma("unroll") for (int k = 0; k < 3; ++k)                                              \
-            if (threadIdx.x + k * 256 < 660) nx[k] = lowf(low[min(max((yw_) * 8 - 1 + sr[k], 0), 255) * 256 + sc[k]]);
-#define PP_STORE(buf_)                                                                             \
-        _Pragma("unroll") for (int k = 0; k < 3; ++k)                                              \
-            if (threadIdx.x + k * 256 < 660) tile[buf_][threadIdx.x + k * 256] = nx[k];
-        PP_LOAD(0);
-        PP_STORE(0);
+        X4Stage st;
+        x4_stage_init(st, cbase);
+        x4_patch_load(st, low, 0);
+        x4_patch_store(st, tile[0]);
         __syncthreads();
         const Axis ax = axis_weights(min(x, out_w - 1), 0.25f, 256);
         const int l0 = ax.i0 - cbase, l1 = ax.i1 - cbase;
-        const float W1[4] = {0.625f, 0.875f, 0.125f, 0.375f};
+        X4Acc acc = {0, 0, 0, 0x7fffffff, -1, false};
         for (int yw = 0; yw < wpc; ++yw) {
-            if (yw + 1 < wpc) { PP_LOAD(yw + 1); }
-            const float* tl = tile[yw & 1];
-            if (x < out_w) {
-                float t[10];
-#pragma unroll
-                for (int k = 0; k < 10; ++k) t[k] = lerp_torch(ax.w0, tl[k * 66 + l0], ax.w1, tl[k * 66 + l1]);
-                const int nb = min(32, out_h - yw * 32);
-                uint32_t wm = 0, wh = 0, wl = 0;
-                uint32_t word;
-                if (nb == 32) {
-                    int s_hi = 0, s_lo = 0;
-                    bool decided = false;
-                    if (!LOGITS) {
-                        const float tmin = fminf(fminf(fminf(t[0], t[1]), fminf(t[2], t[3])), fminf(fminf(t[4], t[5]), fminf(fminf(t[6], t[7]), fminf(t[8], t[9]))));
-                        const float tmax = fmaxf(fmaxf(fmaxf(t[0], t[1]), fmaxf(t[2], t[3])), fmaxf(fmaxf(t[4], t[5]), fmaxf(fmaxf(t[6], t[7]), fmaxf(t[8], t[9]))));
-                        const bool one = tmin > hi_t + 0.01f && tmax < 8192.f, zero = tmax < lo_t - 0.01f && tmin > -8192.f;
-                        if (__ballot(!(one || zero)) == 0) {
-                            decided = true;
-                            word = one ? 0xffffffffu : 0u;
-                            s_hi = s_lo = 32 * __popcll(__ballot(one));
-                        }
-                    }
-                    if (!decided) {
-#pragma unroll
-                        for (int b = 0; b < 32; ++b) {
-                            float w1 = W1[b & 3];
-                            if (b < 2 && yw == 0) w1 = 0.0f;
-                            const float v = lerp_torch(1.0f - w1, t[(b + 2) / 4], w1, t[(b + 2) / 4 + 1]);
-                            if (LOGITS) logits[((long)n * out_h + yw * 32 + b) * out_w + x] = v;
-                            wm = __builtin_amdgcn_alignbit(wm, __float_as_uint(__fsub_rn(thr, v)), 31);
-                            s_hi += __popcll(__ballot(v > hi_t));
-                            s_lo += __popcll(__ballot(v > lo_t));
-                        }
-                        word = __brev(wm);
-                    }
-                    if ((threadIdx.x & 63) == __ffsll((long long)__ballot(1)) - 1) { c_hi += s_hi; c_lo += s_lo; }
-                } else {
-#pragma unroll
-                    for (int b = 0; b < 32; ++b) {
-                        float w1 = W1[b & 3];
-                        if (b < 2 && yw == 0) w1 = 0.0f;
-                        const float v = lerp_torch(1.0f - w1, t[(b + 2) / 4], w1, t[(b + 2) / 4 + 1]);
-                        if (LOGITS) { if (b < nb) logits[((long)n * out_h + yw * 32 + b) * out_w + x] = v; }
-                        wm = __builtin_amdgcn_alignbit(wm, __float_as_uint(__fsub_rn(thr, v)), 31);
-                        wh = __builtin_amdgcn_alignbit(wh, __float_as_uint(__fsub_rn(hi_t, v)), 31);
-                        wl = __builtin_amdgcn_alignbit(wl, __float_as_uint(__fsub_rn(lo_t, v)), 31);
-                    }
-                    const uint32_t valid = (1u << nb) - 1u;
-                    word = __brev(wm) & valid;
-                    c_hi += __popc(__brev(wh) & valid); c_lo += __popc(__brev(wl) & valid);
-                }
-                if (word) {
-                    c_m += __popc(word); any = true;
-                    ymin = min(ymin, yw * 32 + __ffs(word) - 1); ymax = yw * 32 + 31 - __clz(word);
-                }
-                bits[((long)n * wpc + yw) * out_w + x] = word;
-            }
-            if (yw + 1 < wpc) { PP_STORE((yw + 1) & 1); }
+            if (yw + 1 < wpc) x4_patch_load(st, low, yw + 1);
+            if (x < out_w) x4_word<LOGITS>(tile[yw & 1], ax, l0, l1, n, x, yw, wpc, out_h, out_w, thr, hi_t, lo_t, bits, logits, acc);
+            if (yw + 1 < wpc) x4_patch_store(st, tile[(yw + 1) & 1]);
             __syncthreads();
         }
-#undef PP_LOAD
-#undef PP_STORE
+        c_hi = acc.c_hi; c_lo = acc.c_lo; c_m = acc.c_m; ymin = acc.ymin; ymax = acc.ymax; any = acc.any;
     } else {
         const bool live = x < out_w;
         const int x = min((int)(blockIdx.x * 256 + threadIdx.x), out_w - 1);
@@ -229,33 +274,75 @@
             if (live) bits[((long)n * wpc + yw) * out_w + x] = word;
         }
     }
-    int xmin = any ? x : 0x7fffffff, xmax = any ? x : -1;
-#pragma unroll
-    for (int s = 1; s < 64; s <<= 1) {
-        c_hi += __shfl_xor(c_hi, s); c_lo += __shfl_xor(c_lo, s); c_m += __shfl_xor(c_m, s);
-        ymin = min(ymin, __shfl_xor(ymin, s)); ymax = max(ymax, __shfl_xor(ymax, s));
-        xmin = min(xmin, __shfl_xor(xmin, s)); xmax = max(xmax, __shfl_xor(xmax, s));
-    }
-    const int wave = threadIdx.x >> 6;
-    if ((threadIdx.x & 63) == 0) {
-        red[wave][0] = c_hi; red[wave][1] = c_lo; red[wave][2] = c_m; red[wave][3] = xmin; red[wave][4] = ymin;
-        red[wave][5] = xmax; red[wave][6] = ymax;
+    stats_reduce(red, n, x, c_hi, c_lo, c_m, ymin, ymax, any, counts, boxes);
+}
+
+__global__ __launch_bounds__(256) void postprocess_range_kernel(const float* __restrict__ low_res, const float* __restrict__ range, float thr,
+                                                                float off, int* __restrict__ counts, int* __restrict__ boxes,
+                                                                uint32_t* __restrict__ bits) {
+    __shared__ int red[4][7];
+    __shared__ float tile[2][10 * 66];
+    __shared__ float rmin[256], rmax[256];
+    __shared__ uint32_t settled[2];
+    const int bx = blockIdx.x, x = bx * 256 + threadIdx.x, n = blockIdx.y;
+    const float* low = low_res + (long)n * 65536;
+    const float hi_t = thr + off, lo_t = thr - off;
+    {
+        const float* rr = range + ((long)n * 256 + threadIdx.x) * 8;
+        float a = 3.0e38f, b = -3.0e38f;
+        bool nan = false;
+        for (int s = max(bx - 1, 0); s <= min(bx + 1, 3); ++s) {
+            const float lo = rr[2 * s], hi = rr[2 * s + 1];
+            nan = nan || lo != lo || hi != hi;
+            a = fminf(a, lo); b = fmaxf(b, hi);
+        }
+        rmin[threadIdx.x] = nan ? -3.0e38f : a; rmax[threadIdx.x] = nan ? 3.0e38f : b;
     }
     __syncthreads();
-    if (threadIdx.x == 0) {
-        int hi = 0, lo = 0, m = 0, x0 = 0x7fffffff, y0 = 0x7fffffff, x1 = -1, y1 = -1;
-        for (int w = 0; w < 4; ++w) {
-            hi += red[w][0]; lo += red[w][1]; m += red[w][2];
-            x0 = min(x0, red[w][3]); y0 = min(y0, red[w][4]); x1 = max(x1, red[w][5]); y1 = max(y1, red[w][6]);
-        }
-        if (hi) atomicAdd(&counts[n * 3], hi);
-        if (lo) atomicAdd(&counts[n * 3 + 1], lo);
-        if (m) {
-            atomicAdd(&counts[n * 3 + 2], m);
-            atomicMin(&boxes[n * 4], x0); atomicMin(&boxes[n * 4 + 1], y0);
-            atomicMax(&boxes[n * 4 + 2], x1); atomicMax(&boxes[n * 4 + 3], y1);
-        }
-    }
+    if (threadIdx.x < 64) {
+        const int yw = threadIdx.x & 31;
+        float a = 3.0e38f, b = -3.0e38f;
+        for (int r = max(8 * yw - 1, 0); r <= min(8 * yw + 8, 255); ++r) { a = fminf(a, rmin[r]); b = fmaxf(b, rmax[r]); }
+        const bool lane = threadIdx.x < 32;
+        const bool one = lane && a > hi_t + 0.01f && b < 8192.f, zero = lane && b < lo_t - 0.01f && a > -8192.f;
+        const uint32_t m1 = (uint32_t)__ballot(one), m0 = (uint32_t)__ballot(zero);
+        if (threadIdx.x == 0) { settled[0] = m0; settled[1] = m1; }
+    }
+    __syncthreads();
+#if defined(__HIP_DEVICE_COMPILE__)
+    const uint32_t ones = (uint32_t)__builtin_amdgcn_readfirstlane((int)settled[1]), done = (uint32_t)__builtin_amdgcn_readfirstlane((int)settled[0]) | ones;
+#else
+    const uint32_t ones = settled[1], done = settled[0] | ones;
+#endif
+    const int cbase = max(bx * 64 - 1, 0);
+    X4Stage st;
+    x4_stage_init(st, cbase);
+    if (!(done & 1u)) {
+        x4_patch_load(st, low, 0);
+        x4_patch_store(st, tile[0]);
+        __syncthreads();
+    }
+    const Axis ax = axis_weights(x, 0.25f, 256);
+    const int l0 = ax.i0 - cbase, l1 = ax.i1 - cbase;
+    X4Acc acc = {0, 0, 0, 0x7fffffff, -1, false};
+    for (int yw = 0; yw < 32; ++yw) {
+        const bool here = !((done >> yw) & 1u), next = yw + 1 < 32 && !((done >> (yw + 1)) & 1u);
+        if (next) x4_patch_load(st, low, yw + 1);
+        if (here) {
+            x4_word<false>(tile[yw & 1], ax, l0, l1, n, x, yw, 32, 1024, 1024, thr, hi_t, lo_t, bits, nullptr, acc);
+        } else {
+            uint32_t word = 0u;
+            if ((ones >> yw) & 1u) {
+                word = 0xffffffffu;
+                acc.c_hi += 32; acc.c_lo += 32; acc.c_m += 32; acc.any = true;
+                acc.ymin = min(acc.ymin, yw * 32); acc.ymax = yw * 32 + 31;
+            }
+            bits[((long)n * 32 + yw) * 1024 + x] = word;
+        }
+        if (next) x4_patch_store(st, tile[(yw + 1) & 1]);
+        if (here || next) __syncthreads();
+    }
+    stats_reduce(red, n, x, acc.c_hi, acc.c_lo, acc.c_m, acc.ymin, acc.ymax, acc.any, counts, boxes);
 }
 
 
@@ -384,6 +471,22 @@
     return msam_check_launch("msam_postprocess_masks");
 }
 
+int g_tune_amg_range_map = 1;
+
+extern "C" int msam_postprocess_masks_range(const float* low_res, const float* range, int32_t N, int32_t in_h, int32_t in_w, int32_t out_h,
+                                            int32_t out_w, float thr, float off, int32_t* counts, int32_t* boxes, uint32_t* bits,
+                                            void* stream) {
+    if (!range || in_h != 1024 || in_w != 1024 || out_h != 1024 || out_w != 1024)
+        return msam_postprocess_masks16(low_res, MSAM_F32, N, in_h, in_w, out_h, out_w, thr, off, counts, boxes, bits, nullptr, stream);
+    if (!low_res || !counts || !boxes || !bits || N <= 0) { msam_set_error("msam_postprocess_masks_range: null argument"); return 1; }
+    if (N > 65535) { msam_set_error("msam_postprocess_masks_range: at most 65535 masks per call"); return 1; }
+    hipStream_t s = (hipStream_t)stream;
+    hipLaunchKernelGGL(init_stats_kernel, dim3((N + 255) / 256), dim3(256), 0, s, counts, boxes, N);
+    hipLaunchKernelGGL(postprocess_range_kernel, dim3(4, N), dim3(256), 0, s, low_res, range, thr, off, counts, boxes, bits);
+    hipLaunchKernelGGL(finalize_boxes_kernel, dim3((N + 255) / 256), dim3(256), 0, s, boxes, N);
+    return msam_check_launch("msam_postprocess_masks_range");
+}
+
 extern "C" int msam_postprocess_masks(const float* low_res, int32_t N, int32_t in_h, int32_t in_w, int32_t out_h,
                                       int32_t out_w, float thr, float off, int32_t* counts, int32_t* boxes, uint32_t* bits,
                                       float* logits, void* stream) {
diff --git a/micro_sam_amd/csrc/upfused.hip b/micro_sam_amd/csrc/upfused.hip
--- a/micro_sam_amd/csrc/upfused.hip
+++ b/micro_sam_amd/csrc/upfused.hip
@@ -29,7 +29,26 @@
     int out16;
     int blocked;
     int centred;
+    float* range;
 };
+
+MSAM_DEVINL int fkey(int i) { return i ^ ((i >> 31) & 0x7fffffff); }
+template <int CTRL, int XOR>
+MSAM_DEVINL int row_xchg(int v) {
+#if defined(__HIP_DEVICE_COMPILE__)
+    return __builtin_amdgcn_update_dpp(v, v, CTRL, 0xf, 0xf, true);
+#else
+    return __shfl_xor(v, XOR);
+#endif
+}
+MSAM_DEVINL void row16_minmax(float& mnf, float& mxf) {
+    int mn = fkey((int)__float_as_uint(mnf)), mx = fkey((int)__float_as_uint(mxf));
+    mn = min(mn, row_xchg<0xB1, 1>(mn)); mx = max(mx, row_xchg<0xB1, 1>(mx));
+    mn = min(mn, row_xchg<0x4E, 2>(mn)); mx = max(mx, row_xchg<0x4E, 2>(mx));
+    mn = min(mn, row_xchg<0x141, 7>(mn)); mx = max(mx, row_xchg<0x141, 7>(mx));
+    mn = min(mn, row_xchg<0x140, 15>(mn)); mx = max(mx, row_xchg<0x140, 15>(mx));
+    mnf = __uint_as_float((uint32_t)fkey(mn)); mxf = __uint_as_float((uint32_t)fkey(mx));
+}
 
 MSAM_DEVINL float wave_rows_sum(float v) {
     const auto a = __builtin_amdgcn_permlane16_swap(__float_as_uint(v), __float_as_uint(v), false, false);
@@ -99,6 +118,7 @@
 
 template <int UF_PRIO, int G16, int LN2P = 0, int CEN = 0>
 __global__ __launch_bounds__(NTHR, 2) void up_fused_kernel(UpArgs a) {
+    constexpr bool CENW = (CEN & 1) != 0, RNG = (CEN & 2) != 0;
 #define UF_LDS_AHEAD 1
 #if defined(__HIP_DEVICE_COMPILE__) && UF_LDS_AHEAD
 #define UF_R16(dst_, base_, imm_) asm volatile("ds_read_b128 %0, %1 offset:%2" : "=v"(dst_) : "v"(base_), "n"(imm_))
@@ -239,6 +259,7 @@
     const int oesz = a.out16 ? 1 : 2;
     const int ptoff = ((lane >> 4) * 4 + w) * 64 + (lane & 15) * 4;
     const int ovoff = ((((lane >> 4) * 256 + w) * 256) + (lane & 15) * 4) << oesz;
+    const int rvoff = (lane & 15) == 0 ? ((lane >> 4) * 256 + w) * 32 : 0x40000000;
     float4 o4c = make_float4(0.f, 0.f, 0.f, 0.f);
     const char* obase_c = (const char*)a.out;
     uint32_t orange_c = 0;
@@ -251,6 +272,12 @@
         const rsrc_t ro = make_rsrc(obu, (uint32_t)__builtin_amdgcn_readfirstlane((int)orange_c));
         if (__builtin_amdgcn_readfirstlane(oesz) == 1) buf_store8(make_uint2(pack2h(o4c.x, o4c.y), pack2h(o4c.z, o4c.w)), ro, ovoff, oso);
         else buf_store16(make_uint4(__float_as_uint(o4c.x), __float_as_uint(o4c.y), __float_as_uint(o4c.z), __float_as_uint(o4c.w)), ro, ovoff, oso);
+        if constexpr (RNG) {
+            float mn = fminf(fminf(o4c.x, o4c.y), fminf(o4c.z, o4c.w)), mx = fmaxf(fmaxf(o4c.x, o4c.y), fmaxf(o4c.z, o4c.w));
+            row16_minmax(mn, mx);
+            const rsrc_t rr = make_rsrc((const char*)a.range + ((obu - (const char*)a.out) >> 5), (uint32_t)__builtin_amdgcn_readfirstlane((int)orange_c) >> 5);
+            buf_store8(make_uint2(__float_as_uint(mn), __float_as_uint(mx)), rr, rvoff, oso >> 5);
+        }
     };
     int q = 0, p = 0, key0 = 0;
     const char* obase = (const char*)a.out;
@@ -326,16 +353,16 @@
         float s = 0.f, ss = 0.f;
 #pragma unroll
         for (int rt = 0; rt < 4; ++rt) {
-            if constexpr (!CEN) s += (uc[rt][0] + uc[rt][1]) + (uc[rt][2] + uc[rt][3]);
+            if constexpr (!CENW) s += (uc[rt][0] + uc[rt][1]) + (uc[rt][2] + uc[rt][3]);
 #pragma unroll
             for (int r = 0; r < 4; ++r) ss += uc[rt][r] * uc[rt][r];
         }
-        if constexpr (!CEN) s = wave_rows_sum(s);
+        if constexpr (!CENW) s = wave_rows_sum(s);
         ss = wave_rows_sum(ss);
         float mean = s * (1.f / 64.f);
         __builtin_amdgcn_sched_barrier(0);
-        if constexpr (CEN) UF_S1(1, ss, 3); else UF_S1(1, mean, 3);
-        if constexpr (!CEN) {
+        if constexpr (CENW) UF_S1(1, ss, 3); else UF_S1(1, mean, 3);
+        if constexpr (!CENW) {
 #pragma unroll
             for (int rt = 0; rt < 4; ++rt)
 #pragma unroll
@@ -351,7 +378,7 @@
             ss = wave_rows_sum(s2);
         }
         UF_S1(2, ss, 3);
-        float rstd = (LN2P || CEN) ? rsqrtf(ss * (1.f / 64.f) + a.eps) : rsqrtf(fmaxf(ss * (1.f / 64.f) - mean * mean, 0.f) + a.eps);
+        float rstd = (LN2P || CENW) ? rsqrtf(ss * (1.f / 64.f) + a.eps) : rsqrtf(fmaxf(ss * (1.f / 64.f) - mean * mean, 0.f) + a.eps);
         __builtin_amdgcn_sched_barrier(0);
         uint32_t g1w[4][2];
 #pragma unroll
@@ -478,8 +505,16 @@
                                       const float* ln_w, const float* ln_b, float ln_eps, const void* w2, const float* b2,
                                       const float* hyper, int32_t hyper_ld, int32_t mask0, int32_t nmask, void* low_res,
                                       int32_t low_res_dtype, void* stream) {
+    return msam_upscale_fused_range(keys, keys_blocked, P, w1, b1, ln_w, ln_b, ln_eps, w2, b2, hyper, hyper_ld, mask0, nmask, low_res, low_res_dtype,
+                                    nullptr, stream);
+}
+
+extern "C" int msam_upscale_fused_range(const void* keys, int32_t keys_blocked, int32_t P, const void* w1, const float* b1,
+                                        const float* ln_w, const float* ln_b, float ln_eps, const void* w2, const float* b2,
+                                        const float* hyper, int32_t hyper_ld, int32_t mask0, int32_t nmask, void* low_res,
+                                        int32_t low_res_dtype, float* range, void* stream) {
     if (low_res_dtype != MSAM_F32 && low_res_dtype != MSAM_F16) {
-        msam_set_error("msam_upscale_fused_out: low_res_dtype is MSAM_F32 or MSAM_F16");
+        msam_set_error("msam_upscale_fused_out / _range: low_res_dtype is MSAM_F32 or MSAM_F16");
         return 1;
     }
     if (!keys || !w1 || !b1 || !ln_w || !ln_b || !w2 || !b2 || !hyper || !low_res || P <= 0) {
@@ -488,6 +523,11 @@
     }
     if (nmask < 1 || nmask > 3 || mask0 < 0 || mask0 + nmask > 4 || hyper_ld < 32 || hyper_ld % 4) {
         msam_set_error("msam_upscale_fused: 1 <= nmask <= 3 masks out of 4, hyper_ld >= 32 and a multiple of 4");
+        return 1;
+    }
+    if (range && low_res_dtype != MSAM_F32) { msam_set_error("msam_upscale_fused_range: the range map goes with fp32 low-res logits only"); return 1; }
+    if (range && (!g_uf_prio || g_tune_up_ln_two_pass || (MSAM_DEC_F16 && g_tune_up_gelu16 > 1))) {
+        msam_set_error("msam_upscale_fused_range: no range map with the up_ln_two_pass / up_gelu16 > 1 / priority 0 kernels");
         return 1;
     }
     UpArgs a{};
@@ -499,11 +539,23 @@
     int ks = 1;
     while (P * ks < 2 * cus && ks < 16) ks *= 2;
     a.KS = ks; a.nitems = P * ks; a.out = low_res; a.out16 = low_res_dtype == MSAM_F16; a.blocked = keys_blocked & 1; a.centred = (keys_blocked >> 1) & 1;
+    a.range = range;
     const int grid = a.nitems < 2 * cus ? a.nitems : 2 * cus;
     const double rows = (double)P * T;
     const double flops = rows * (2.0 * 256 * 256 + 4 * 2.0 * 128 * 64 + 16 * 3 * 2.0 * 16 * 32);
-    const double bytes = rows * C * 2 + (double)P * nmask * 256 * 256 * (low_res_dtype == MSAM_F16 ? 2 : 4);
+    const double bytes = rows * C * 2 + (double)P * nmask * 256 * 256 * (low_res_dtype == MSAM_F16 ? 2 : 4) + (range ? (double)P * nmask * 256 * 4 * 8 : 0.0);
     msam_profile_mark2(stream, 1, flops, bytes, 4);
+    const bool cen = a.centred && g_tune_up_centred;
+#if MSAM_DEC_F16
+    if (range && g_tune_up_gelu16) {
+        if (cen) hipLaunchKernelGGL((up_fused_kernel<1, 1, 0, 3>), dim3(grid), dim3(NTHR), 0, (hipStream_t)stream, a);
+        else hipLaunchKernelGGL((up_fused_kernel<1, 1, 0, 2>), dim3(grid), dim3(NTHR), 0, (hipStream_t)stream, a);
+    } else
+#endif
+    if (range) {
+        if (cen) hipLaunchKernelGGL((up_fused_kernel<1, 0, 0, 3>), dim3(grid), dim3(NTHR), 0, (hipStream_t)stream, a);
+        else hipLaunchKernelGGL((up_fused_kernel<1, 0, 0, 2>), dim3(grid), dim3(NTHR), 0, (hipStream_t)stream, a);
+    } else
 #if MSAM_DEC_F16
     if (g_tune_up_gelu16 == 2) hipLaunchKernelGGL((up_fused_kernel<1, 2>), dim3(grid), dim3(NTHR), 0, (hipStream_t)stream, a);
     else if (g_tune_up_gelu16 == 3) hipLaunchKernelGGL((up_fused_kernel<1, 3>), dim3(grid), dim3(NTHR), 0, (hipStream_t)stream, a);
diff --git a/micro_sam_amd/modeling.py b/micro_sam_amd/modeling.py
--- a/micro_sam_amd/modeling.py
+++ b/micro_sam_amd/modeling.py
@@ -2,7 +2,7 @@
 
 import ctypes as C
 import os
-from typing import List, Optional, Tuple
+from typing import List, Optional, Tuple, Union
 
 import torch
 import torch.nn as nn
@@ -683,6 +683,7 @@
         iou = torch.empty((P, nc), dtype=torch.float32, device=dev)
         ws = self._workspace(P)
         p.low_res_dtype = _lib.F32
+        p.low_res_range = None
         _lib.check(_lib.load().msam_decoder_forward_embeddings(
             C.byref(p), consts.data_ptr(), state.data_ptr(), sp.data_ptr() if Ns > 0 else None, Ns, dptr, eptr, P,
             1 if multimask_output else 0, low.data_ptr(), iou.data_ptr(), ws.data_ptr(), ws.numel(), _lib.stream_ptr()),
@@ -692,7 +693,11 @@
     @torch.no_grad()
     def decode(self, features: torch.Tensor, point_coords: Optional[torch.Tensor], point_labels: Optional[torch.Tensor],
                boxes: Optional[torch.Tensor] = None, mask_input: Optional[torch.Tensor] = None,
-               multimask_output: bool = True, low_res_dtype: torch.dtype = torch.float32) -> Tuple[torch.Tensor, torch.Tensor]:
+               multimask_output: bool = True, low_res_dtype: torch.dtype = torch.float32,
+               range_map: Union[bool, torch.Tensor] = False) -> Tuple[torch.Tensor, ...]:
+        want_range = range_map is not False and range_map is not None
+        if want_range and (low_res_dtype != torch.float32 or self.reference_formulation or mask_input is not None):
+            raise ValueError("range_map goes with float32 low-res logits of the kernel path, without a mask prompt")
         if low_res_dtype not in (torch.float32, torch.float16):
             raise ValueError("low_res_dtype is torch.float32 or torch.float16")
         if features.numel() != PROMPT_DIM * GRID * GRID:
@@ -724,6 +729,12 @@
         low = torch.empty((P, nc, 256, 256), dtype=low_res_dtype, device=dev)
         iou = torch.empty((P, nc), dtype=torch.float32, device=dev)
         p.low_res_dtype = _lib.F16 if low_res_dtype == torch.float16 else _lib.F32
+        rng = None
+        if want_range:
+            rng = range_map if isinstance(range_map, torch.Tensor) else torch.empty((P, nc, 256, 4, 2), dtype=torch.float32, device=dev)
+            if rng.dtype != torch.float32 or tuple(rng.shape) != (P, nc, 256, 4, 2) or not rng.is_contiguous() or rng.device != low.device:
+                raise ValueError(f"range_map must be a contiguous float32 tensor [{P},{nc},256,4,2] on {low.device}")
+        p.low_res_range = _lib.ptr(rng)
         need = lib.msam_decoder_workspace_bytes(P)
         if self._dec_ws is None or self._dec_ws.numel() < need or self._dec_ws.device != dev:
             self._dec_ws = None
@@ -737,6 +748,8 @@
             C.byref(p), C.byref(self._mask_params), consts.data_ptr(), state.data_ptr(), _lib.ptr(pts), _lib.ptr(lbl), Np,
             _lib.ptr(bx), _lib.ptr(msk), P, 1 if multimask_output else 0, low.data_ptr(), iou.data_ptr(),
             self._dec_ws.data_ptr(), self._dec_ws.numel(), _lib.stream_ptr()), "msam_decoder_forward")
+        if want_range:
+            return low, iou, rng
         return low, iou
 
 
diff --git a/micro_sam_amd/ops.py b/micro_sam_amd/ops.py
--- a/micro_sam_amd/ops.py
+++ b/micro_sam_amd/ops.py
@@ -359,7 +359,7 @@
 
 def postprocess_masks(low_res: torch.Tensor, input_size: Tuple[int, int], original_size: Tuple[int, int],
                       mask_threshold: float = 0.0, stability_offset: float = 1.0,
-                      want_logits: bool = False) -> Dict[str, torch.Tensor]:
+                      want_logits: bool = False, range_map: Optional[torch.Tensor] = None) -> Dict[str, torch.Tensor]:
     _home("low_res", low_res)
     _need(low_res.dim() == 3 and tuple(low_res.shape[1:]) == (256, 256), f"low_res must be [N,256,256], got {list(low_res.shape)}")
     low_res = low_res.contiguous() if low_res.dtype == torch.float16 else low_res.to(torch.float32).contiguous()
@@ -371,10 +371,19 @@
     boxes = torch.empty((N, 4), dtype=torch.int32, device=dev)
     bits = torch.empty((N, (H + 31) // 32, W), dtype=torch.int32, device=dev)
     logits = torch.empty((N, H, W), dtype=torch.float32, device=dev) if want_logits else None
+    if range_map is not None:
+        _need(low_res.dtype == torch.float32 and not want_logits, "range_map goes with float32 low_res and want_logits=False")
+        _t("range_map", range_map, _F32, (N, 256, 4, 2), dev)
     lib = _lib.load()
     step = 65535
     for s in range(0, N, step):
         n = min(step, N - s)
+        if range_map is not None:
+            _lib.check(lib.msam_postprocess_masks_range(
+                low_res[s:].data_ptr(), range_map[s:].data_ptr(), n, int(input_size[0]), int(input_size[1]), H, W, float(mask_threshold),
+                float(stability_offset), counts[s:].data_ptr(), boxes[s:].data_ptr(), bits[s:].data_ptr(), _lib.stream_ptr()),
+                "msam_postprocess_masks_range")
+            continue
         _lib.check(lib.msam_postprocess_masks16(
             low_res[s:].data_ptr(), low_dt, n, int(input_size[0]), int(input_size[1]), H, W, float(mask_threshold),
             float(stability_offset), counts[s:].data_ptr(), boxes[s:].data_ptr(), bits[s:].data_ptr(),
diff --git a/micro_sam_amd/predictor.py b/micro_sam_amd/predictor.py
--- a/micro_sam_amd/predictor.py
+++ b/micro_sam_amd/predictor.py
@@ -102,10 +102,17 @@
                              stability_score_offset: float = 1.0):
         if not self.is_image_set:
             raise RuntimeError("An image must be set with .set_image(...) before mask prediction.")
-        low, iou = self.model.decode(self.features, point_coords, point_labels, boxes, None, multimask_output,
-                                     low_res_dtype=self.model.amg_low_res_dtype)
+        from . import _lib
+        dt = self.model.amg_low_res_dtype
+        with_map = (dt == torch.float32 and not self.model.reference_formulation
+                    and tuple(int(v) for v in self.input_size) == (1024, 1024)
+                    and tuple(int(v) for v in self.original_size) == (1024, 1024) and _lib.tune_get("amg_range_map") == 1)
+        out = self.model.decode(self.features, point_coords, point_labels, boxes, None, multimask_output, low_res_dtype=dt,
+                                range_map=with_map)
+        low, iou = out[0], out[1]
         from .ops import postprocess_masks
         b, c = low.shape[:2]
         res = postprocess_masks(low.reshape(b * c, 256, 256), self.input_size, self.original_size,
-                                self.model.mask_threshold, stability_score_offset, want_logits=False)
+                                self.model.mask_threshold, stability_score_offset, want_logits=False,
+                                range_map=out[2].reshape(b * c, 256, 4, 2) if with_map else None)
         return iou, res
```
